# AgamChopra/TorchRegister

Measured on AMD Instinct MI355X. Metric: registration iterations/sec (3D 256^3 fp32, affine+NCC), higher is better.
Workload: dtype f32; 1 GPU; 3D 256^3 fp32 affine+NCC, 8 independent pairs per GPU (BASELINE.json configs[3] share of one GPU), ADAM on theta; pairs_per_gpu=8, pairs_total=8, loss=NCC(alpha=100), optimizer=adam, preconditioning=100 untimed iterations before the warm-up (clock settling); value_cold has none, parallelism=1 x independent shards, no collective

## Files before the change

torchregister_amd/csrc/affine.hip:

```cpp
#ifdef TRX_DEV
#include <cstdlib>
#endif
#include "trx_dev.h"

#include "trx_common.h"

namespace trx {

struct AffineGeom {
    int TX, TY, logTX, RPT, nxseg, nychunk, nblk;
};

static AffineGeom affine_geom(const trx_volumes &v, int target_blocks_total)
{
    AffineGeom g;
    int tx = 16, l = 4;
    while (tx < v.W && tx < TRX_BLOCK) { tx <<= 1; l++; }
    g.TX = tx; g.logTX = l; g.TY = TRX_BLOCK / tx;
    g.nxseg = (v.W + tx - 1) / tx;
    long rows = (long)v.D * v.H * g.nxseg * v.B;
    long rpt = rows / ((long)g.TY * target_blocks_total);
    if (rpt < 1) rpt = 1;
    if (rpt > 64) rpt = 64;
    g.RPT = (int)rpt;
    int rows_per_blk = g.TY * g.RPT;
    g.nychunk = (v.H + rows_per_blk - 1) / rows_per_blk;
    g.nblk = v.D * g.nychunk * g.nxseg;
    return g;
}

constexpr int np_full(int nd) { return 5 + 3 * nd * (nd + 1); }
constexpr int kRowsMask = 0xFFFFFF;
__host__ __device__ constexpr int rows_note(int rows, int body) { return rows > 0 ? (rows | (body << 24)) : 0; }
constexpr int kNpMse = 13;

template <int ND, int MODE>
__global__ __launch_bounds__(TRX_BLOCK) void affine_accum_kernel(trx_volumes vol, const float *__restrict__ theta,
                                                                 AffineGeom g, int channels, size_t chan_stride,
                                                                 float *__restrict__ partials)
{
    constexpr int NC = ND;
    constexpr int NQ = (MODE == 0) ? 3 : (MODE == 2 ? 1 : 0);
    constexpr int NP = (MODE == 0) ? np_full(ND) : (MODE == 1 ? 5 : ND * (ND + 1));
    const int b = blockIdx.y;
    int id = blockIdx.x;
    const int xs = id % g.nxseg; id /= g.nxseg;
    const int yc = id % g.nychunk;
    const int z = id / g.nychunk;
    const int tid = threadIdx.x;
    const int lx = tid & (g.TX - 1), ly = tid >> g.logTX;
    const int x = xs * g.TX + lx;
    const int D = vol.D, H = vol.H, W = vol.W;

    const float *__restrict__ th = theta + (size_t)b * TRX_PSTRIDE;
    const float *__restrict__ mov = vol.moving + (size_t)b * vol.moving_stride;
    const float *__restrict__ tgt = vol.target + (size_t)b * vol.target_stride;

    float A[NQ > 0 ? NQ : 1][NC], Bq[NQ > 0 ? NQ : 1][NC], m[5];
#pragma unroll
    for (int q = 0; q < (NQ > 0 ? NQ : 1); q++)
#pragma unroll
        for (int c = 0; c < NC; c++) A[q][c] = Bq[q][c] = 0.f;
#pragma unroll
    for (int i = 0; i < 5; i++) m[i] = 0.f;

    float xn = 0.f, zn = 0.f;
    if (x < W) {
        xn = base_coord(vol.xn, x, W);
        float bx, by, bz = 0.f, t_x1, t_y1, t_z1 = 0.f;
        if constexpr (ND == 3) {
            zn = base_coord(vol.zn, z, D);
            bx = fmaf(th[0], xn, fmaf(th[2], zn, th[3]));
            by = fmaf(th[4], xn, fmaf(th[6], zn, th[7]));
            bz = fmaf(th[8], xn, fmaf(th[10], zn, th[11]));
            t_x1 = th[1]; t_y1 = th[5]; t_z1 = th[9];
        } else {
            bx = fmaf(th[0], xn, th[2]);
            by = fmaf(th[3], xn, th[5]);
            t_x1 = th[1]; t_y1 = th[4];
        }
        const float fW = (float)W, fH = (float)H, fD = (float)D;
        const int y0 = yc * g.TY * g.RPT + ly;
        for (int j = 0; j < g.RPT; j++) {
            const int y = y0 + j * g.TY;
            if (y >= H) break;
            const float yn = base_coord(vol.yn, y, H);
            const float ix = unnorm<ND>(fmaf(t_x1, yn, bx), fW);
            const float iy = unnorm<ND>(fmaf(t_y1, yn, by), fH);
            const size_t vox = ((size_t)z * H + y) * W + x;
            float gq[NC];
            float w;
            if constexpr (MODE == 2) {
#pragma unroll
                for (int c = 0; c < NC; c++) gq[c] = 0.f;
                for (int ch = 0; ch < channels; ch++) {
                    const float go = tgt[ch * chan_stride + vox];
                    if constexpr (ND == 3) {
                        const float iz = unnorm<ND>(fmaf(t_z1, yn, bz), fD);
                        Samp3 s = sample3(mov + ch * chan_stride, D, H, W, ix, iy, iz);
                        gq[0] = fmaf(go, s.dx, gq[0]); gq[1] = fmaf(go, s.dy, gq[1]); gq[2] = fmaf(go, s.dz, gq[2]);
                    } else {
                        Samp2 s = sample2(mov + ch * chan_stride, H, W, ix, iy);
                        gq[0] = fmaf(go, s.dx, gq[0]); gq[1] = fmaf(go, s.dy, gq[1]);
                    }
                }
                w = 0.f;
            } else {
                if constexpr (ND == 3) {
                    const float iz = unnorm<ND>(fmaf(t_z1, yn, bz), fD);
                    Samp3 s = sample3(mov, D, H, W, ix, iy, iz);
                    w = s.v; gq[0] = s.dx; gq[1] = s.dy; gq[2] = s.dz;
                } else {
                    Samp2 s = sample2(mov, H, W, ix, iy);
                    w = s.v; gq[0] = s.dx; gq[1] = s.dy;
                }
            }
            if constexpr (MODE != 2) {
                const float yv = tgt[vox];
                m[0] += yv; m[1] += w;
                m[2] = fmaf(yv, yv, m[2]); m[3] = fmaf(w, w, m[3]); m[4] = fmaf(yv, w, m[4]);
                if constexpr (MODE == 0) {
#pragma unroll
                    for (int c = 0; c < NC; c++) {
                        const float u = yn * gq[c];
                        A[0][c] += gq[c];            Bq[0][c] += u;
                        A[1][c] = fmaf(yv, gq[c], A[1][c]); Bq[1][c] = fmaf(yv, u, Bq[1][c]);
                        A[2][c] = fmaf(w, gq[c], A[2][c]);  Bq[2][c] = fmaf(w, u, Bq[2][c]);
                    }
                }
            } else {
#pragma unroll
                for (int c = 0; c < NC; c++) { A[0][c] += gq[c]; Bq[0][c] = fmaf(yn, gq[c], Bq[0][c]); }
            }
        }
    }

    float vals[NP];
    int o = 0;
    if constexpr (MODE != 2) {
#pragma unroll
        for (int i = 0; i < 5; i++) vals[o++] = m[i];
    }
#pragma unroll
    for (int q = 0; q < NQ; q++)
#pragma unroll
        for (int c = 0; c < NC; c++) {
            vals[o++] = xn * A[q][c];
            vals[o++] = Bq[q][c];
            if constexpr (ND == 3) vals[o++] = zn * A[q][c];
            vals[o++] = A[q][c];
        }
    block_reduce_store<NP>(vals, partials + ((size_t)b * g.nblk + blockIdx.x) * NP);
}

template <int TX_, int TZ_, int THREADS_, int BW_, int BH_, int BD_, int PP_, int TY_ = 16>
struct TileCfg {
    static constexpr int TX = TX_, TY = TY_, TZ = TZ_, Threads = THREADS_;
    static constexpr int BW = BW_, BH = BH_, BD = BD_, PP = PP_;
    static constexpr int NH = Threads / (TX * TZ);
    static constexpr int Rows = TY / NH;
    static constexpr int Waves = Threads / 64;
    static constexpr int BW4 = BW / 4;
    static constexpr int PlaneSlots = BH * BW4;
    static constexpr int Pieces = (BD + PP - 1) / PP;
    static constexpr int PieceFloats = PP * BH * BW;
    static constexpr int BoxFloats = BW * BH * BD;
    static constexpr int ReduceScratch = Waves * 16 * 65 + Waves * 16;
    static constexpr int BoxAlloc = (BoxFloats > ReduceScratch) ? BoxFloats : ReduceScratch;
    static_assert(BW % 4 == 0 && PP * PlaneSlots <= Threads && (PP == 2 || PP == 4), "one DMA piece: at most one slot per thread");
};
using GeomA = TileCfg<32, 8, 512, 44, 23, TRX_GEOMA_BD, 2>;
#ifndef TRX_GEOMR_BH
#define TRX_GEOMR_BH 27
#define TRX_GEOMR_BD 26
#endif
using GeomR = TileCfg<16, 8, 512, 28, TRX_GEOMR_BH, TRX_GEOMR_BD, 2>;
using GeomD = TileCfg<32, 16, 512, 44, 23, 19, 2>;
using GeomRD = TileCfg<16, 16, 512, 28, TRX_GEOMR_BH, TRX_GEOMR_BD, 2>;

struct TileGeom {
    int ntx, nty, ntz, ntiles, blocks_per_pair, ysplit, tiles_per_seg;
};

template <class G = GeomA>
static TileGeom tile_geom(const trx_volumes &v)
{
    TileGeom t;
    t.ntx = (v.W + G::TX - 1) / G::TX; t.nty = (v.H + G::TY - 1) / G::TY; t.ntz = (v.D + G::TZ - 1) / G::TZ;
    t.ntiles = t.ntx * t.nty * t.ntz;
    const int ncol = t.ntx * t.ntz;
#ifdef TRX_DEV
    static const int target = [] { const char *e = getenv("TRX_TILE_TARGET_BLOCKS"); return e ? atoi(e) : 0; }();
#else
    constexpr int target = 0;
#endif
    const long cols = (long)v.B * ncol;
    int ys = 1;
    if (target > 0) {
        ys = (int)((target + cols - 1) / cols);
    } else if (cols * t.nty > 1024) {
        double best = 1e30;
        int last_tps = 0;
        const int cmax = cols > 512 ? (t.nty < 4 ? t.nty : 4) : t.nty;
        for (int c = 1; c <= cmax; c++) {
            const int tps = (t.nty + c - 1) / c, segs = (t.nty + tps - 1) / tps;
            if (tps == last_tps) continue;
            last_tps = tps;
            const long blocks = cols * segs, full = blocks / 512, rem = blocks % 512;
            double cost = (double)full * 1.6 * (tps + 1.5);
            if (rem > 0) cost += (rem <= 256 ? 1.0 : 1.6) * (tps + 1.5);
            if (cost < best - 1e-9) { best = cost; ys = c; }
        }
    } else if (cols <= 512) {
        ys = (int)((512 + cols - 1) / cols);
        const int cap = t.nty / 2 > 1 ? t.nty / 2 : 1;
        if (ys > cap && cols * cap >= 256) ys = cap;
    } else {
        double best = 1e30;
        for (int c = 1; c <= 4 && c <= t.nty; c++) {
            const int tps = (t.nty + c - 1) / c, segs = (t.nty + tps - 1) / tps;
            const double blocks = (double)cols * segs;
            const double rounds = (double)(((long)blocks + 511) / 512);
            const double waste = rounds * 512.0 / blocks * (1.0 + 1.5 / tps);
            if (waste < best - 1e-9) { best = waste; ys = c; }
        }
    }
    if (ys < 1) ys = 1;
    if (ys > t.nty) ys = t.nty;
    t.tiles_per_seg = (t.nty + ys - 1) / ys;
    t.ysplit = (t.nty + t.tiles_per_seg - 1) / t.tiles_per_seg;
    t.blocks_per_pair = ncol * t.ysplit;
    return t;
}

struct F1Acc {
    f2 AB[3][3], M01, M23;
    float M4;
};

template <int MODE>
__device__ __forceinline__ void f1_accumulate_pk(const Samp3 &sm, float yv, float yn, F1Acc &a)
{
    if constexpr (MODE == 2) {
        const float gq[3] = {sm.dx, sm.dy, sm.dz};
#pragma unroll
        for (int c = 0; c < 3; c++) {
            const f2 gu = {gq[c], yn * gq[c]};
            a.AB[0][c] = gu * yv + a.AB[0][c];
        }
        return;
    }
    if constexpr (MODE == 4) {
        const float d = sm.v - yv;
        a.M4 = fmaf(d, d, a.M4);
        const float gq[3] = {sm.dx, sm.dy, sm.dz};
#pragma unroll
        for (int c = 0; c < 3; c++) {
            const f2 gu = {gq[c], yn * gq[c]};
            a.AB[0][c] = gu * d + a.AB[0][c];
        }
        return;
    }
    const f2 yw = {yv, sm.v};
    a.M01 += yw;
    a.M23 = yw * yw + a.M23;
    a.M4 = fmaf(yv, sm.v, a.M4);
    if constexpr (MODE == 0) {
        const float gq[3] = {sm.dx, sm.dy, sm.dz};
#pragma unroll
        for (int c = 0; c < 3; c++) {
            const f2 gu = {gq[c], yn * gq[c]};
            a.AB[0][c] += gu;
            a.AB[1][c] = gu * yv + a.AB[1][c];
            a.AB[2][c] = gu * sm.v + a.AB[2][c];
        }
    }
}

constexpr int kTileThreads = GeomA::Threads;

__device__ __forceinline__ int trx_lane_id() { return (int)__builtin_amdgcn_mbcnt_hi(~0u, __builtin_amdgcn_mbcnt_lo(~0u, 0u)); }
__device__ __forceinline__ int trx_wave_index() { return __builtin_amdgcn_readfirstlane((int)threadIdx.x >> 6); }

template <int NV, int NW>
__device__ __forceinline__ void block_reduce_store_nw(const float (&vals)[NV], float *__restrict__ out, float *smem, int wave)
{
    constexpr int CH = 16;
    float(*red)[CH][65] = reinterpret_cast<float(*)[CH][65]>(smem);
    float(*wsum)[CH] = reinterpret_cast<float(*)[CH]>(smem + NW * CH * 65);
    const int lane = trx_lane_id(), tid = wave * 64 + lane;
#pragma unroll
    for (int c0 = 0; c0 < NV; c0 += CH) {
#pragma unroll
        for (int j = 0; j < CH; j++)
            if (c0 + j < NV) red[wave][j][lane] = vals[c0 + j];
        __syncthreads();
        if (lane < CH && c0 + lane < NV) {
            float s = 0.f;
#pragma unroll 16
            for (int i = 0; i < 64; i++) s += red[wave][lane][i];
            wsum[wave][lane] = s;
        }
        __syncthreads();
        if (tid < CH && c0 + tid < NV) {
            float s = 0.f;
#pragma unroll
            for (int w = 0; w < NW; w++) s += wsum[w][tid];
            out[c0 + tid] = s;
        }
        __syncthreads();
    }
}

__device__ __forceinline__ float uni(float v) { return __int_as_float(__builtin_amdgcn_readfirstlane(__float_as_int(v))); }
template <class T>
__device__ __forceinline__ T *uni_ptr(T *p)
{
    const unsigned long long v = (unsigned long long)p;
    const unsigned lo = __builtin_amdgcn_readfirstlane((unsigned)v), hi = __builtin_amdgcn_readfirstlane((unsigned)(v >> 32));
    return (T *)(((unsigned long long)hi << 32) | lo);
}
__device__ __forceinline__ float lane_bcast(float v, int lane) { return __int_as_float(__builtin_amdgcn_readlane(__float_as_int(v), lane)); }

#pragma clang diagnostic push
#pragma clang diagnostic ignored "-Winline-asm"
#pragma clang diagnostic ignored "-Wint-to-pointer-cast"
template <int MODE, class G, bool LTH = false>
__device__ __forceinline__ void tile_body(const trx_volumes &vol, const float *__restrict__ theta, const TileGeom &tg, int channels,
                                          float *__restrict__ partials, float *box, const int bx, const int by, const int rows_stride, const int wave_in)
{
    constexpr int kTX = G::TX, kTY = G::TY, kTZ = G::TZ, kBW = G::BW, kBH = G::BH, kBD = G::BD, kPP = G::PP;
    constexpr int kBufs = 1;
    constexpr int kNH = G::NH, kRows = G::Rows, kTileWaves = G::Waves, kBW4 = G::BW4, kPlaneSlots = G::PlaneSlots, kPieces = G::Pieces;
    constexpr int kPieceFloats = G::PieceFloats, kBoxFloats = G::BoxFloats;
    (void)kNH; (void)kBD; (void)kPlaneSlots;
    constexpr int NQ = (MODE == 0) ? 3 : ((MODE == 2 || MODE == 4) ? 1 : 0);
    constexpr int NP = (MODE == 0) ? np_full(3) : (MODE == 2 ? 12 : (MODE == 4 ? kNpMse : 5));
    constexpr bool kGrad = (MODE == 0) || (MODE == 2) || (MODE == 4);
    constexpr bool kPerChannel = (MODE == 2) || (MODE == 3);
    const int b = kPerChannel ? by / channels : by;
    const int ch = kPerChannel ? by - b * channels : 0;
    const int D = vol.D, H = vol.H, W = vol.W;
    const float *__restrict__ th = LTH ? theta : uni_ptr(theta + (size_t)b * TRX_PSTRIDE);
    const float *__restrict__ mov = uni_ptr(vol.moving + (size_t)b * vol.moving_stride + (size_t)ch * D * H * W);
    float *__restrict__ wout = uni_ptr(partials + (size_t)by * D * H * W);
    const float *__restrict__ tgt = (MODE == 3) ? wout : uni_ptr(vol.target + (size_t)b * vol.target_stride + (MODE == 2 ? (size_t)ch * D * H * W : 0));
    const float *__restrict__ xtab = uni_ptr(vol.xn), *__restrict__ ytab = uni_ptr(vol.yn), *__restrict__ ztab = uni_ptr(vol.zn);
    const int lane = trx_lane_id();
    const int wave = __builtin_amdgcn_readfirstlane(wave_in);
    const int tid = wave * 64 + lane;
    const int lx = tid & (kTX - 1), lz = (tid / kTX) & (kTZ - 1), lh = wave / (kTileWaves / kNH);
    const float fW = (float)W, fH = (float)H, fD = (float)D;
    const float hW = 0.5f * fW, hH = 0.5f * fH, hD = 0.5f * fD;
    auto thv = [&](int k) { return LTH ? uni(th[k]) : th[k]; };
    const float t00 = thv(0), t01 = thv(1), t02 = thv(2), t03 = thv(3);
    const float t10 = thv(4), t11 = thv(5), t12 = thv(6), t13 = thv(7);
    const float t20 = thv(8), t21 = thv(9), t22 = thv(10), t23 = thv(11);
    const float sx = uni(hW * t01), sy = uni(hH * (t11 - 1.0f)), sz = uni(hD * t21);

    const int ncol = tg.ntx * tg.ntz;
    const int yseg = bx / ncol, cb = bx - yseg * ncol;
    int col = cb;
    if ((ncol & 7) == 0) col = (cb & 7) * (ncol >> 3) + (cb >> 3);
    const int X0 = (col % tg.ntx) * kTX, Z0 = (col / tg.ntx) * kTZ;
    const int nx = min(kTX, W - X0), nz = min(kTZ, D - Z0);
    const bool act = (lx < nx) && (lz < nz);
    const int x = X0 + (act ? lx : 0), z = Z0 + (act ? lz : 0);
    const float xn = xtab[x], zn = ztab[z];
    const float base_x = unnorm<3>(xn, fW) + hW * fmaf(t00 - 1.0f, xn, fmaf(t02, zn, t03));
    const float base_y = hH * fmaf(t10, xn, fmaf(t12, zn, t13));
    const float base_z = unnorm<3>(zn, fD) + hD * fmaf(t20, xn, fmaf(t22 - 1.0f, zn, t23));

    float ext_lo[3], ext_hi[3];
    {
        const float ex[3] = {(float)(kTX - 1), (float)(kTY - 1), (float)(kTZ - 1)};
        const float slope[3][3] = {{t00, t01 * fW / fH, t02 * fW / fD}, {t10 * fH / fW, t11, t12 * fH / fD}, {t20 * fD / fW, t21 * fD / fH, t22}};
#pragma unroll
        for (int c = 0; c < 3; c++) {
            ext_lo[c] = ext_hi[c] = 0.f;
#pragma unroll
            for (int a = 0; a < 3; a++) {
                const float e = slope[c][a] * ex[a];
                ext_lo[c] += fminf(e, 0.f); ext_hi[c] += fmaxf(e, 0.f);
            }
            ext_lo[c] = uni(ext_lo[c]); ext_hi[c] = uni(ext_hi[c]);
        }
    }
    const float cxn = xtab[X0], czn = ztab[Z0];
    const float corner_x = uni(unnorm<3>(cxn, fW) + hW * fmaf(t00 - 1.0f, cxn, fmaf(t02, czn, t03)));
    const float corner_y = uni(hH * fmaf(t10, cxn, fmaf(t12, czn, t13)));
    const float corner_z = uni(unnorm<3>(czn, fD) + hD * fmaf(t20, cxn, fmaf(t22 - 1.0f, czn, t23)));

    auto slot_geom = [&](int ln, unsigned &rb0, int &d0) {
        const int q = wave * 64 + ln;
        const int pz = q / kPlaneSlots, r = q - pz * kPlaneSlots;
        const int dy = r / kBW4, dx4 = r - dy * kBW4;
        const bool valid = q < kPP * kPlaneSlots;
        rb0 = valid ? (unsigned)((pz * H + dy) * W + dx4 * 4) * 4u : 0u;
        d0 = valid ? ((pz << 16) | (dy << 8) | dx4) : (100 << 16);
    };
    const unsigned piece_stride = (unsigned)(kPP * H * W) * 4u;
    constexpr int kDShift = (kPP == 2) ? 17 : 18;
    auto fill_slot = [&](float *dst, int gz, int gy, int gx) {
        const bool rowin = ((unsigned)gz < (unsigned)D) && ((unsigned)gy < (unsigned)H);
        const float *row = mov + ((size_t)(rowin ? gz : 0) * H + (rowin ? gy : 0)) * W;
        float4 v;
        v.x = (rowin && (unsigned)(gx + 0) < (unsigned)W) ? row[gx + 0] : 0.f;
        v.y = (rowin && (unsigned)(gx + 1) < (unsigned)W) ? row[gx + 1] : 0.f;
        v.z = (rowin && (unsigned)(gx + 2) < (unsigned)W) ? row[gx + 2] : 0.f;
        v.w = (rowin && (unsigned)(gx + 3) < (unsigned)W) ? row[gx + 3] : 0.f;
        *reinterpret_cast<float4 *>(dst) = v;
    };
    static_assert(kPP == 2 || kPP == 4, "piece planes");

    F1Acc acc;
#pragma unroll
    for (int q = 0; q < 3; q++)
#pragma unroll
        for (int c = 0; c < 3; c++) acc.AB[q][c] = (f2)(0.f);
    acc.M01 = acc.M23 = (f2)(0.f);
    acc.M4 = 0.f;
    const int j0 = lh * kRows;
    const int toff = (z * H + j0) * W + x;

    const int ty_begin = yseg * tg.tiles_per_seg, ty_end = min((yseg + 1) * tg.tiles_per_seg, tg.nty);
    int g_ox = 0, g_oy = 0, g_oz = 0, g_pk = 0;
    auto lane_geometry = [&](int ty_first) {
        const int ty = min(ty_first + lane, tg.nty - 1);
        const float yn0 = ytab[ty * kTY], yid0 = unnorm<3>(yn0, fH);
        const float cx = fmaf(sx, yn0, corner_x), cy = yid0 + fmaf(sy, yn0, corner_y), cz = fmaf(sz, yn0, corner_z);
        const float slack = 0.05f;
        bool fits = (fabsf(cx) < 1.0e6f) && (fabsf(cy) < 1.0e6f) && (fabsf(cz) < 1.0e6f);
        int ox = 0, oy = 0, oz = 0, ex4 = 0, ey = 0, ez = 0;
        bool interior = false;
        if (fits) {
            const int lx0 = (int)floorf(cx + ext_lo[0] - slack), hx1 = (int)floorf(cx + ext_hi[0] + slack) + 1;
            oy = (int)floorf(cy + ext_lo[1] - slack); const int hy1 = (int)floorf(cy + ext_hi[1] + slack) + 1;
            oz = (int)floorf(cz + ext_lo[2] - slack); const int hz1 = (int)floorf(cz + ext_hi[2] + slack) + 1;
            ox = lx0 & ~3;
            ex4 = ((hx1 - ox) >> 2) + 1; ey = hy1 - oy + 1; ez = hz1 - oz + 1;
            fits = (ex4 <= kBW4) && (ey <= kBH) && (ez <= kBD);
            interior = (ox >= 0) && (oy >= 0) && (oz >= 0) && (ox + kBW <= W) && (oy + kBH <= H) && (oz + kBD <= D);
        }
        g_ox = ox; g_oy = oy; g_oz = oz;
        g_pk = fits ? ((ex4 - 1) | ((ey - 1) << 8) | ((ez - 1) << 16) | (1 << 24) | ((interior ? 1 : 0) << 25)) : 0;
    };
    int ty = ty_begin;
    {
        const unsigned toffb = (unsigned)toff * 4u;
        const unsigned lane7b = (unsigned)(lane & (kRows - 1)) * 4u;
        float sxv, syv, szv;
        asm("v_mov_b32 %0, %1" : "=v"(sxv) : "s"(sx));
        asm("v_mov_b32 %0, %1" : "=v"(syv) : "s"(sy));
        asm("v_mov_b32 %0, %1" : "=v"(szv) : "s"(sz));
        int ys_s, zs_s;
        asm("s_mov_b32 %0, %1" : "=s"(ys_s) : "i"(kBW * 4));
        asm("s_mov_b32 %0, %1" : "=s"(zs_s) : "i"(kBW * kBH * 4));
        const unsigned box_lds = (unsigned)(uintptr_t)box;
        unsigned rb0;
        {
            int d0;
            slot_geom(lane, rb0, d0);
        }
        constexpr bool kZMask = kPieces > 8;
        static_assert(!kZMask || (kPP == 2 && kBD <= 32), "plane-bit masks: pieces of two planes");
        constexpr int kNM = kZMask ? 1 : kPieces;
        unsigned long long m_ld[kNM];
#pragma unroll
        for (int k = 0; k < kNM; k++) m_ld[k] = 0;
        unsigned long long m_a0 = 0, m_a1 = 0;
        unsigned m_zb = 0;
        unsigned m_oob = 0;
        unsigned m_part = 0;
        int lim_blk;
        {
            const float slack2 = 0.1f;
            const int ex4m = (((int)floorf(ext_hi[0] - ext_lo[0] + slack2) + 5) >> 2) + 1;
            const int eym = (int)floorf(ext_hi[1] - ext_lo[1] + slack2) + 3, ezm = (int)floorf(ext_hi[2] - ext_lo[2] + slack2) + 3;
            lim_blk = __builtin_amdgcn_readfirstlane(((min(ezm, kBD) - 1) << 16) | ((min(eym, kBH) - 1) << 8) | (min(ex4m, kBW4) - 1));
        }
        int m_lim = -1, m_lo = -1, m_hi = -1, m_px = -2;
        TRX_TM_INIT();
        typedef const __attribute__((address_space(3))) f2u *lds_f2;
        while (ty < ty_end) {
          lane_geometry(ty);
          const int chunk = min(64, ty_end - ty);
          const bool xpart = ((W & 3) != 0) && (g_ox + 4 * ((lim_blk & 0xff) + 1) > W - (W & 3)) &&
                             (g_oy + ((lim_blk >> 8) & 0xff) >= H - 1) && (g_oz + (lim_blk >> 16) >= D - 1);
          const bool ok = (lane < chunk) && ((g_pk >> 24) & 1) && ((ty + lane + 1) * kTY <= H) && !xpart;
          const unsigned long long bad = ~__builtin_amdgcn_ballot_w64(ok);
          const int nf = bad ? __builtin_ctzll(bad) : 64;
          const char *dma_base = nullptr;
          unsigned dma_lds = 0;
          auto issue_box = [&](int g, int buf, bool spread) {
              const int ox = __builtin_amdgcn_readlane(g_ox, g), oy = __builtin_amdgcn_readlane(g_oy, g), oz = __builtin_amdgcn_readlane(g_oz, g);
              const int lim = lim_blk;
              const int loz = max(0, -oz), loy = max(0, -oy), lox = max(0, -(ox >> 2));
              const int hiz = min(lim >> 16, D - 1 - oz), hiy = min((lim >> 8) & 0xff, H - 1 - oy), hix = min(lim & 0xff, ((W - ox + 3) >> 2) - 1);
              const bool none = (hiz < loz) || (hiy < loy) || (hix < lox);
              const int lo = none ? 0x7f7f7f : ((loz << 16) | (loy << 8) | lox);
              const int hi = none ? 0 : ((hiz << 16) | (hiy << 8) | hix);
              const int part_x = ((W & 3) && !none && ((W - ox) >> 2) <= hix) ? ((W - ox) >> 2) : -1;
              if (lim != m_lim || lo != m_lo || hi != m_hi || part_x != m_px) {
                  m_lim = lim; m_lo = lo; m_hi = hi; m_px = part_x;
                  m_oob = 0;
                  m_part = 0;
                  int ln = lane;
                  asm volatile("" : "+v"(ln));
                  unsigned rbx;
                  int d0;
                  slot_geom(ln, rbx, d0);
#pragma unroll
                  for (int k = 0; k < kPieces; k++) {
                      const int d = d0 + (k << kDShift);
                      const bool need = (((lim - d) & 0x80808080) == 0);
                      const bool ld = need && (((hi - d) & 0x80808080) == 0) && (((d - lo) & 0x80808080) == 0);
                      if constexpr (!kZMask) m_ld[k] = __builtin_amdgcn_ballot_w64(ld);
                      if (need && !ld) m_oob |= 1u << k;
                      if (ld && (d & 0xff) == part_x) m_part |= 1u << k;
                  }
                  if constexpr (kZMask) {
                      const int dyx = d0 & 0xffff;
                      const bool xy = (((((lim & 0xffff) - dyx) | ((hi & 0xffff) - dyx) | (dyx - (lo & 0xffff))) & 0x8080) == 0);
                      m_a0 = __builtin_amdgcn_ballot_w64(xy && (d0 >> 16) == 0);
                      m_a1 = __builtin_amdgcn_ballot_w64(xy && (d0 >> 16) == 1);
                      m_zb = (unsigned)__builtin_amdgcn_readfirstlane((int)(none ? 0u : (((2u << hiz) - 1u) & ~((1u << loz) - 1u))));
                  }
              }
              dma_base = reinterpret_cast<const char *>(mov + (ptrdiff_t)((oz * H + oy) * W + ox));
              dma_lds = box_lds + (unsigned)buf * (kBoxFloats * 4u) + (unsigned)wave * 1024u;
              if (TRX_DBG_SKIP != 2 && !spread) {
                  const float *mbase = reinterpret_cast<const float *>(dma_base);
                  const unsigned lds0 = dma_lds;
                  unsigned long long sv;
                  unsigned m0s;
                  static_assert((kPieces >= 6 && kPieces <= 8) || (kPieces >= 9 && kPieces <= 13), "the DMA block below is written for 6, 7, 8 or 9..13 pieces");
#define TRX_DMA_SKIP "s_cbranch_execz 1f\n\t"
#define TRX_DMA_NEXT(K)                                  \
    "s_add_u32 s100, s100, %[vstr]\n\t"                  \
    "s_addc_u32 s101, s101, 0\n\t"                       \
    "s_add_u32 m0, m0, %[pstr]\n\t"                      \
    "s_mov_b64 exec, %[k" #K "]\n\t"                     \
    TRX_DMA_SKIP                                         \
    "global_load_lds_dwordx4 %[off], s[100:101]" TRX_BOX_POLICY "\n\t" \
    "1:\n\t"
#define TRX_DMA_HEAD                                     \
    "s_mov_b64 %[sv], exec\n\t"                          \
    "s_mov_b32 %[m0s], m0\n\t"                           \
    "s_mov_b64 s[100:101], %[base]\n\t"                  \
    "s_mov_b32 m0, %[lds]\n\t"                           \
    "s_mov_b64 exec, %[k0]\n\t"                          \
    TRX_DMA_SKIP                                         \
    "global_load_lds_dwordx4 %[off], s[100:101]" TRX_BOX_POLICY "\n\t"     \
    "1:\n\t"                                             \
    TRX_DMA_NEXT(1) TRX_DMA_NEXT(2) TRX_DMA_NEXT(3) TRX_DMA_NEXT(4) TRX_DMA_NEXT(5)
#define TRX_DMA_TAIL "s_mov_b64 exec, %[sv]\n\t" "s_mov_b32 m0, %[m0s]"
                  if constexpr (kZMask) {
                      static_assert(kPieces <= 13, "plane-bit DMA block: up to 13 pieces (the plane bits of pieces a shallower box lacks are never set)");
                      unsigned long long t0, t1;
#define TRX_DMA_ZSEL(B0, B1)                             \
    "s_bitcmp1_b32 %[zb], " #B0 "\n\t"                   \
    "s_cselect_b64 %[t0], %[a0], 0\n\t"                 \
    "s_bitcmp1_b32 %[zb], " #B1 "\n\t"                   \
    "s_cselect_b64 %[t1], %[a1], 0\n\t"                 \
    "s_or_b64 exec, %[t0], %[t1]\n\t"                   \
    "s_cbranch_execz 1f\n\t"                            \
    "global_load_lds_dwordx4 %[off], s[100:101]" TRX_BOX_POLICY "\n\t" \
    "1:\n\t"
#define TRX_DMA_ZNEXT(B0, B1)                            \
    "s_add_u32 s100, s100, %[vstr]\n\t"                 \
    "s_addc_u32 s101, s101, 0\n\t"                      \
    "s_add_u32 m0, m0, %[pstr]\n\t" TRX_DMA_ZSEL(B0, B1)
                      asm volatile("s_mov_b64 %[sv], exec\n\t"
                                   "s_mov_b32 %[m0s], m0\n\t"
                                   "s_mov_b64 s[100:101], %[base]\n\t"
                                   "s_mov_b32 m0, %[lds]\n\t" TRX_DMA_ZSEL(0, 1)
                                   TRX_DMA_ZNEXT(2, 3) TRX_DMA_ZNEXT(4, 5) TRX_DMA_ZNEXT(6, 7) TRX_DMA_ZNEXT(8, 9) TRX_DMA_ZNEXT(10, 11)
                                   TRX_DMA_ZNEXT(12, 13) TRX_DMA_ZNEXT(14, 15) TRX_DMA_ZNEXT(16, 17) TRX_DMA_ZNEXT(18, 19)
                                   TRX_DMA_ZNEXT(20, 21) TRX_DMA_ZNEXT(22, 23) TRX_DMA_ZNEXT(24, 25) TRX_DMA_TAIL
                                   : [sv] "=&s"(sv), [m0s] "=&s"(m0s), [t0] "=&s"(t0), [t1] "=&s"(t1)
                                   : [lds] "s"(lds0), [base] "s"(mbase), [pstr] "i"(kPieceFloats * 4), [vstr] "s"(piece_stride), [off] "v"(rb0),
                                     [a0] "s"(m_a0), [a1] "s"(m_a1), [zb] "s"(__builtin_amdgcn_readfirstlane((int)m_zb))
                                   : "memory", "scc", "s100", "s101");
#undef TRX_DMA_ZSEL
#undef TRX_DMA_ZNEXT
                  } else if constexpr (kPieces == 8) {
                      asm volatile(TRX_DMA_HEAD TRX_DMA_NEXT(6) TRX_DMA_NEXT(7) TRX_DMA_TAIL
                                   : [sv] "=&s"(sv), [m0s] "=&s"(m0s)
                                   : [lds] "s"(lds0), [base] "s"(mbase), [pstr] "i"(kPieceFloats * 4), [vstr] "s"(piece_stride), [off] "v"(rb0),
                                     [k0] "s"(m_ld[0]), [k1] "s"(m_ld[1]), [k2] "s"(m_ld[2]), [k3] "s"(m_ld[3]), [k4] "s"(m_ld[4]),
                                     [k5] "s"(m_ld[5]), [k6] "s"(m_ld[kPieces > 6 ? 6 : 0]), [k7] "s"(m_ld[kPieces - 1])
                                   : "memory", "scc", "s100", "s101");
                  } else if constexpr (kPieces == 7) {
                      asm volatile(TRX_DMA_HEAD TRX_DMA_NEXT(6) TRX_DMA_TAIL
                                   : [sv] "=&s"(sv), [m0s] "=&s"(m0s)
                                   : [lds] "s"(lds0), [base] "s"(mbase), [pstr] "i"(kPieceFloats * 4), [vstr] "s"(piece_stride), [off] "v"(rb0),
                                     [k0] "s"(m_ld[0]), [k1] "s"(m_ld[1]), [k2] "s"(m_ld[2]), [k3] "s"(m_ld[3]), [k4] "s"(m_ld[4]),
                                     [k5] "s"(m_ld[5]), [k6] "s"(m_ld[kPieces - 1])
                                   : "memory", "scc", "s100", "s101");
                  } else {
                      asm volatile(TRX_DMA_HEAD TRX_DMA_TAIL
                                   : [sv] "=&s"(sv), [m0s] "=&s"(m0s)
                                   : [lds] "s"(lds0), [base] "s"(mbase), [pstr] "i"(kPieceFloats * 4), [vstr] "s"(piece_stride), [off] "v"(rb0),
                                     [k0] "s"(m_ld[0]), [k1] "s"(m_ld[1]), [k2] "s"(m_ld[2]), [k3] "s"(m_ld[3]), [k4] "s"(m_ld[4]),
                                     [k5] "s"(m_ld[5])
                                   : "memory", "scc", "s100", "s101");
                  }
#undef TRX_DMA_NEXT
#undef TRX_DMA_SKIP
#undef TRX_DMA_HEAD
#undef TRX_DMA_TAIL
              }
              if (m_oob) {
                  float zero;
                  asm volatile("v_mov_b32 %0, 0" : "=v"(zero));
#pragma unroll
                  for (int k = 0; k < kPieces; k++)
                      if (m_oob & (1u << k))
                          *reinterpret_cast<float4 *>(box + buf * kBoxFloats + k * kPieceFloats + (wave * 64 + lane) * 4) = make_float4(zero, zero, zero, zero);
              }
          };
          auto zero_tails = [&](int buf) {
#pragma unroll
              for (int k = 0; k < kPieces; k++)
                  if (m_part & (1u << k)) {
                      float *sl = box + buf * kBoxFloats + k * kPieceFloats + (wave * 64 + lane) * 4;
                      for (int e = W & 3; e < 4; e++) sl[e] = 0.f;
                  }
          };
          auto issue_piece = [&](int k) {
              if (TRX_DBG_SKIP == 2) return;
              unsigned long long sv;
              unsigned m0s;
              asm volatile("s_mov_b64 %[sv], exec\n\t"
                           "s_mov_b32 %[m0s], m0\n\t"
                           "s_mov_b32 m0, %[lds]\n\t"
                           "s_mov_b64 exec, %[mk]\n\t"
                           "global_load_lds_dwordx4 %[off], %[base]\n\t"
                           "s_mov_b64 exec, %[sv]\n\t"
                           "s_mov_b32 m0, %[m0s]"
                           : [sv] "=&s"(sv), [m0s] "=&s"(m0s)
                           : [lds] "s"(dma_lds + (unsigned)k * (kPieceFloats * 4u)), [base] "s"(dma_base + (size_t)k * piece_stride), [off] "v"(rb0),
                             [mk] "s"(kZMask ? ((((m_zb >> (2 * k)) & 1u) ? m_a0 : 0ull) | (((m_zb >> (2 * k + 1)) & 1u) ? m_a1 : 0ull)) : m_ld[kZMask ? 0 : k])
                           : "memory");
          };
          auto gather_tile = [&](int g, int buf, float yn_l, float yid_l, float (&tv)[kRows], const float *tnext, bool dma_next) {
              const int Y0 = (ty + g) * kTY;
              const int ox = __builtin_amdgcn_readlane(g_ox, g), oy = __builtin_amdgcn_readlane(g_oy, g), oz = __builtin_amdgcn_readlane(g_oz, g);
              float yn_r[kRows], yid_r[kRows];
#pragma unroll
              for (int j = 0; j < kRows; j++) { yn_r[j] = lane_bcast(yn_l, j); yid_r[j] = lane_bcast(yid_l, j); }
              if (TRX_DBG_SKIP == 1) return;
              const int bpb = (int)box_lds + buf * (kBoxFloats * 4) - ((oz * kBH + oy) * kBW + ox) * 4;
              struct Fetch { f2 r00, r01, r10, r11; float fx, fy, fz; };
              auto fetch = [&](int j) -> Fetch {
                  const float yn = yn_r[j];
                  const float ix = fmaf(sxv, yn, base_x);
                  const float iy = yid_r[j] + fmaf(syv, yn, base_y);
                  const float iz = fmaf(szv, yn, base_z);
                  int a0, a1, a2, a3;
                  asm("v_lshl_add_u32 %0, %1, 2, %2" : "=v"(a0) : "v"(floor_to_int(ix)), "s"(bpb));
                  asm("v_mad_i32_i24 %0, %1, %2, %3" : "=v"(a1) : "v"(floor_to_int(iy)), "s"(ys_s), "v"(a0));
                  asm("v_mad_i32_i24 %0, %1, %2, %3" : "=v"(a2) : "v"(floor_to_int(iz)), "s"(zs_s), "v"(a1));
                  asm("v_add_u32 %0, %1, %2" : "=v"(a3) : "s"(zs_s), "v"(a2));
                  Fetch f;
                  f.r00 = *(lds_f2)(unsigned)a2; f.r01 = *(lds_f2)(unsigned)(a2 + kBW * 4);
                  f.r10 = *(lds_f2)(unsigned)a3; f.r11 = *(lds_f2)(unsigned)(a3 + kBW * 4);
                  f.fx = __builtin_amdgcn_fractf(ix); f.fy = __builtin_amdgcn_fractf(iy); f.fz = __builtin_amdgcn_fractf(iz);
                  return f;
              };
              Fetch cur = fetch(0);
#pragma unroll
              for (int j = 0; j < kRows; j++) {
                  Fetch nxt;
                  if (j + 1 < kRows) nxt = fetch(j + 1);
                  if (kBufs == 2 && j < kPieces && dma_next) issue_piece(j);
                  const Samp3 sm = lerp3_pairs<kGrad>(cur.r00, cur.r01, cur.r10, cur.r11, cur.fx, cur.fy, cur.fz);
                  if constexpr (MODE == 3) { if (act) wout[(size_t)Y0 * W + (unsigned)(toff + j * W)] = sm.v; }
                  else f1_accumulate_pk<MODE>(sm, tv[j], yn_r[j], acc);
                  if (kBufs == 2 && TRX_DBG_SKIP != 3 && MODE != 3)
                      asm volatile("global_load_dword %0, %1, %2" : "=v"(tv[j]) : "v"(toffb), "s"(tnext + (size_t)j * W));
                  if (j + 1 < kRows) cur = nxt;
              }
          };
          auto load_targets = [&](int g, float (&tv)[kRows]) {
              const float *trow = tgt + (size_t)(ty + g) * kTY * W;
#pragma unroll
              for (int j = 0; j < kRows; j++) {
                  if (TRX_DBG_SKIP == 3 || MODE == 3) tv[j] = 1.f;
                  else asm volatile("global_load_dword %0, %1, %2" TRX_TGT_POLICY : "=v"(tv[j]) : "v"(toffb), "s"(trow + (size_t)j * W) : "memory");
              }
          };
          float tv[kRows];
          if constexpr (kBufs == 1) {
            for (int gl = 0; gl < nf; gl++) {
              TRX_TM_STAMP(tm0);
              float yn_l;
              asm volatile("global_load_dword %0, %1, %2" : "=v"(yn_l) : "v"(lane7b), "s"(ytab + (ty + gl) * kTY + j0) : "memory");
              __builtin_amdgcn_s_setprio(TRX_STAGE_PRIO);
              load_targets(gl, tv);
              issue_box(gl, 0, false);
              __builtin_amdgcn_s_setprio(0);
              asm volatile("s_waitcnt vmcnt(0)" ::: "memory");
              if (m_part) zero_tails(0);
              {
#pragma unroll
                  for (int j = 0; j < kRows; j++) asm volatile("" : "+v"(tv[j]));
                  asm volatile("" : "+v"(yn_l));
              }
              const float yid_l = unnorm<3>(yn_l, fH);
              TRX_TM_STAMP(tm1);
              __syncthreads();
              TRX_TM_STAMP(tm2);
              gather_tile(gl, 0, yn_l, yid_l, tv, nullptr, false);
              TRX_TM_STAMP(tm3);
              __syncthreads();
              TRX_TM_TILE_DONE();
            }
          } else {
            if (nf > 0) {
                load_targets(0, tv);
                issue_box(0, 0, false);
            }
            for (int gl = 0; gl < nf; gl++) {
              TRX_TM_STAMP(tm0);
              float yn_l;
              asm volatile("global_load_dword %0, %1, %2" : "=v"(yn_l) : "v"(lane7b), "s"(ytab + (ty + gl) * kTY + j0) : "memory");
              asm volatile("s_waitcnt vmcnt(0)" ::: "memory");
              if (m_part) zero_tails(gl & 1);
              {
#pragma unroll
                  for (int j = 0; j < kRows; j++) asm volatile("" : "+v"(tv[j]));
                  asm volatile("" : "+v"(yn_l));
              }
              const float yid_l = unnorm<3>(yn_l, fH);
              TRX_TM_STAMP(tm1);
              __syncthreads();
              TRX_TM_STAMP(tm2);
              const int gn = (gl + 1 < nf) ? gl + 1 : gl;
              if (gl + 1 < nf) issue_box(gl + 1, (gl + 1) & 1, true);
              TRX_TM_STAMP(tm3);
              gather_tile(gl, gl & 1, yn_l, yid_l, tv, tgt + (size_t)(ty + gn) * kTY * W, gl + 1 < nf);
              TRX_TM_TILE_DONE();
            }
            asm volatile("s_waitcnt vmcnt(0)" ::: "memory");
#pragma unroll
            for (int j = 0; j < kRows; j++) asm volatile("" : "+v"(tv[j]));
            __syncthreads();
          }
          ty += nf;
          if (nf < chunk) break;
        }
        TRX_TM_STORE();
        if (!act) {
#pragma unroll
            for (int q = 0; q < 3; q++)
#pragma unroll
                for (int c = 0; c < 3; c++) acc.AB[q][c] = (f2)(0.f);
            acc.M01 = acc.M23 = (f2)(0.f);
            acc.M4 = 0.f;
        }
    }

    unsigned rb0;
    int d0;
    {
        int ln = lane;
        asm volatile("" : "+v"(ln));
        slot_geom(ln, rb0, d0);
    }
    int prev_lim = -1;
    unsigned needmask = 0;

    auto stage_box = [&](int pk, int ox, int oy, int oz) {
        const bool interior = (pk >> 25) & 1;
        const int lim = pk & 0xffffff;
        if (lim != prev_lim) {
            prev_lim = lim;
            needmask = 0;
#pragma unroll
            for (int k = 0; k < kPieces; k++)
                if (((lim - (d0 + (k << kDShift))) & 0x80808080) == 0) needmask |= 1u << k;
        }
        const int obase = (oz * H + oy) * W + ox;
        unsigned oob = 0;
        if (interior) {
            const char *__restrict__ mbase = reinterpret_cast<const char *>(mov + obase);
#pragma unroll
            for (int k = 0; k < kPieces; k++)
                if ((needmask & (1u << k)) && TRX_DBG_SKIP != 2)
                    __builtin_amdgcn_global_load_lds(reinterpret_cast<const float *>(mbase + (size_t)k * piece_stride + rb0),
                                                     box + k * kPieceFloats + wave * 256, 16, 0, 0);
        } else {
#pragma unroll
            for (int k = 0; k < kPieces; k++)
                if ((needmask & (1u << k)) && TRX_DBG_SKIP != 2) {
                    const int d = d0 + (k << kDShift);
                    const int gz = oz + (d >> 16), gy = oy + ((d >> 8) & 0xff), gx = ox + (d & 0xff) * 4;
                    const bool inb = ((unsigned)gz < (unsigned)D) && ((unsigned)gy < (unsigned)H) && (gx >= 0) && (gx + 4 <= W);
                    const unsigned idx = inb ? (unsigned)(obase + (int)((rb0 + k * piece_stride) >> 2)) : 0u;
                    if (!inb) oob |= 1u << k;
                    __builtin_amdgcn_global_load_lds(mov + idx, box + k * kPieceFloats + wave * 256, 16, 0, 0);
                }
        }
        __builtin_amdgcn_s_setprio(0);
        asm volatile("s_waitcnt vmcnt(0)" ::: "memory");
        if (oob) {
#pragma unroll
            for (int k = 0; k < kPieces; k++)
                if (oob & (1u << k)) {
                    const int d = d0 + (k << kDShift);
                    fill_slot(box + k * kPieceFloats + (wave * 64 + lane) * 4, oz + (d >> 16), oy + ((d >> 8) & 0xff), ox + (d & 0xff) * 4);
                }
        }
    };
    auto gather = [&](const float *bp, float yn, float yid) -> Samp3 {
        const float ix = fmaf(sx, yn, base_x);
        const float iy = yid + fmaf(sy, yn, base_y);
        const float iz = fmaf(sz, yn, base_z);
        const int a = __mul24(floor_to_int(iz), kBH * kBW) + __mul24(floor_to_int(iy), kBW) + floor_to_int(ix);
        const float *p = bp + a;
        const f2 r00 = *reinterpret_cast<const f2u *>(p), r01 = *reinterpret_cast<const f2u *>(p + kBW);
        const f2 r10 = *reinterpret_cast<const f2u *>(p + kBW * kBH), r11 = *reinterpret_cast<const f2u *>(p + kBW * kBH + kBW);
        return lerp3_pairs<kGrad>(r00, r01, r10, r11, __builtin_amdgcn_fractf(ix), __builtin_amdgcn_fractf(iy), __builtin_amdgcn_fractf(iz));
    };

    for (; ty < ty_end; ty++) {
        const int gl = (ty - ty_begin) & 63;
        if (gl == 0) lane_geometry(ty);
        const int Y0 = ty * kTY;
        const int ny = min(kTY, H - Y0);
        const float yn_l = ytab[Y0 + min(lane & (kTY - 1), ny - 1)];
        const float yid_l = unnorm<3>(yn_l, fH);
        const int pk = __builtin_amdgcn_readlane(g_pk, gl);
        const int ox = __builtin_amdgcn_readlane(g_ox, gl), oy = __builtin_amdgcn_readlane(g_oy, gl), oz = __builtin_amdgcn_readlane(g_oz, gl);
        const bool fits = (pk >> 24) & 1;
        const float *__restrict__ trow = tgt + (size_t)Y0 * W;

        if (fits) {
            __builtin_amdgcn_s_setprio(TRX_STAGE_PRIO);
            float tv[kRows];
#pragma unroll
            for (int j = 0; j < kRows; j++)
                tv[j] = (TRX_DBG_SKIP == 3 || MODE == 3) ? 1.f : trow[(unsigned)(toff + (min(j0 + j, ny - 1) - j0) * W)];
            stage_box(pk, ox, oy, oz);
            __syncthreads();
            float yn_r[kRows], yid_r[kRows];
#pragma unroll
            for (int j = 0; j < kRows; j++) { yn_r[j] = lane_bcast(yn_l, j0 + j); yid_r[j] = lane_bcast(yid_l, j0 + j); }
            if (act && TRX_DBG_SKIP != 1) {
                const float *bp = box - ((oz * kBH + oy) * kBW + ox);
#pragma unroll
                for (int j = 0; j < kRows; j++)
                    if (j0 + j < ny) {
                        const Samp3 sm = gather(bp, yn_r[j], yid_r[j]);
                        if constexpr (MODE == 3) wout[(size_t)Y0 * W + (unsigned)(toff + j * W)] = sm.v;
                        else f1_accumulate_pk<MODE>(sm, tv[j], yn_r[j], acc);
                    }
            }
            __syncthreads();
        } else if (act) {
            struct GFetch { f2 r00, r01, r10, r11; float fx, fy, fz, yn, yv; };
            auto gfetch = [&](int j) -> GFetch {
                GFetch g;
                g.yn = ytab[Y0 + j];
                const float ix = fmaf(sx, g.yn, base_x);
                const float iy = unnorm<3>(g.yn, fH) + fmaf(sy, g.yn, base_y);
                const float iz = fmaf(sz, g.yn, base_z);
                const float flx = floorf(ix), fly = floorf(iy), flz = floorf(iz);
                g.fx = ix - flx; g.fy = iy - fly; g.fz = iz - flz;
                const int x0 = (int)flx, y0 = (int)fly, z0 = (int)flz;
                const bool interior = ((unsigned)x0 < (unsigned)(W - 1)) & ((unsigned)y0 < (unsigned)(H - 1)) & ((unsigned)z0 < (unsigned)(D - 1));
                if (__all(interior)) {
                    const float *p = mov + ((size_t)z0 * H + y0) * W + x0, *q = p + (size_t)H * W;
                    g.r00 = *reinterpret_cast<const f2u *>(p); g.r01 = *reinterpret_cast<const f2u *>(p + W);
                    g.r10 = *reinterpret_cast<const f2u *>(q); g.r11 = *reinterpret_cast<const f2u *>(q + W);
                } else {
                    const int x1 = x0 + 1, y1 = y0 + 1, z1 = z0 + 1;
                    const bool bx0 = (unsigned)x0 < (unsigned)W, bx1 = (unsigned)x1 < (unsigned)W;
                    const bool by0 = (unsigned)y0 < (unsigned)H, by1 = (unsigned)y1 < (unsigned)H;
                    const bool bz0 = (unsigned)z0 < (unsigned)D, bz1 = (unsigned)z1 < (unsigned)D;
                    const int cx0 = min(max(x0, 0), W - 1), cx1 = min(max(x1, 0), W - 1);
                    const int cy0 = min(max(y0, 0), H - 1), cy1 = min(max(y1, 0), H - 1);
                    const int cz0 = min(max(z0, 0), D - 1), cz1 = min(max(z1, 0), D - 1);
                    const float *a00 = mov + ((size_t)cz0 * H + cy0) * W, *a01 = mov + ((size_t)cz0 * H + cy1) * W;
                    const float *a10 = mov + ((size_t)cz1 * H + cy0) * W, *a11 = mov + ((size_t)cz1 * H + cy1) * W;
                    g.r00 = f2{(bz0 & by0 & bx0) ? a00[cx0] : 0.f, (bz0 & by0 & bx1) ? a00[cx1] : 0.f};
                    g.r01 = f2{(bz0 & by1 & bx0) ? a01[cx0] : 0.f, (bz0 & by1 & bx1) ? a01[cx1] : 0.f};
                    g.r10 = f2{(bz1 & by0 & bx0) ? a10[cx0] : 0.f, (bz1 & by0 & bx1) ? a10[cx1] : 0.f};
                    g.r11 = f2{(bz1 & by1 & bx0) ? a11[cx0] : 0.f, (bz1 & by1 & bx1) ? a11[cx1] : 0.f};
                }
                g.yv = (MODE == 3) ? 0.f : trow[(unsigned)(toff + (j - j0) * W)];
                return g;
            };
            const int jend = min(j0 + kRows, ny);
            if (j0 < jend) {
                GFetch cur = gfetch(j0);
#pragma unroll 1
                for (int j = j0; j < jend; j++) {
                    GFetch nxt = cur;
                    if (j + 1 < jend) nxt = gfetch(j + 1);
                    const Samp3 sm = lerp3_pairs<kGrad>(cur.r00, cur.r01, cur.r10, cur.r11, cur.fx, cur.fy, cur.fz);
                    if constexpr (MODE == 3) wout[(size_t)Y0 * W + (unsigned)(toff + (j - j0) * W)] = sm.v;
                    else f1_accumulate_pk<MODE>(sm, cur.yv, cur.yn, acc);
                    cur = nxt;
                }
            }
        }
    }

    if constexpr (MODE == 3) return;
    float vals[NP];
    int o = 0;
    if constexpr (MODE == 4) {
        vals[0] = acc.M4;
        o = 1;
    } else if constexpr (MODE != 2) {
        vals[0] = acc.M01.x; vals[1] = acc.M01.y; vals[2] = acc.M23.x; vals[3] = acc.M23.y; vals[4] = acc.M4;
        o = 5;
    }
#pragma unroll
    for (int q = 0; q < NQ; q++)
#pragma unroll
        for (int c = 0; c < 3; c++) {
            const float a = acc.AB[q][c].x;
            vals[o++] = xn * a; vals[o++] = acc.AB[q][c].y; vals[o++] = zn * a; vals[o++] = a;
        }
    block_reduce_store_nw<NP, kTileWaves>(vals, partials + ((size_t)by * rows_stride + bx) * NP, box, wave);
}

template <int MODE>
__global__ __launch_bounds__(GeomA::Threads, TRX_TILE_MIN_WAVES) void affine_tile_kernel(trx_volumes vol, const float *__restrict__ theta,
                                                                                          TileGeom tg, int channels, float *__restrict__ partials)
{
    __shared__ __attribute__((aligned(16))) float box[GeomA::BoxAlloc + TRX_DEV_LDS_PAD];
    tile_body<MODE, GeomA>(vol, theta, tg, channels, partials, box, blockIdx.x, blockIdx.y, gridDim.x, trx_wave_index());
}

#pragma clang diagnostic pop
#include "affine_zstream.h"
#include "affine_eft.h"
#pragma clang diagnostic push
#pragma clang diagnostic ignored "-Winline-asm"
#pragma clang diagnostic ignored "-Wint-to-pointer-cast"

template <class G>
__device__ __forceinline__ bool dual_fits(const float *__restrict__ th, float fD, float fH, float fW)
{
    const float slope[3][3] = {{th[0], th[1] * fW / fH, th[2] * fW / fD}, {th[4] * fH / fW, th[5], th[6] * fH / fD}, {th[8] * fD / fW, th[9] * fD / fH, th[10]}};
    const float ex[3] = {(float)(G::TX - 1), (float)(G::TY - 1), (float)(G::TZ - 1)};
    float span[3];
#pragma unroll
    for (int c = 0; c < 3; c++) span[c] = fabsf(slope[c][0]) * ex[0] + fabsf(slope[c][1]) * ex[1] + fabsf(slope[c][2]) * ex[2];
    return (span[0] < 1.0e6f) && (span[1] < 1.0e6f) && (span[2] < 1.0e6f) &&
           ((((int)floorf(span[0] + 0.1f) + 5) >> 2) + 1 <= G::BW4) && ((int)floorf(span[1] + 0.1f) + 3 <= G::BH) &&
           ((int)floorf(span[2] + 0.1f) + 3 <= G::BD);
}
__device__ __forceinline__ int dual_choice(const float *__restrict__ th, float fD, float fH, float fW, bool with_deep, bool with_rd = false, int zs_planes = 0)
{
    if (zs_planes > 0 && zs_nsub<ZS64>(th, fD, fH, fW, zs_planes) > 0) return 4;
    if (with_deep && dual_fits<GeomD>(th, fD, fH, fW)) return 0;
    if (dual_fits<GeomA>(th, fD, fH, fW)) return 1;
    return (with_rd && dual_fits<GeomRD>(th, fD, fH, fW)) ? 3 : 2;
}

__device__ __forceinline__ bool eft_wants(int choice, const float *__restrict__ th, float fD, float fH, float fW)
{
    if (choice == 2) return true;
    if (choice != 3) return false;
    const float tilt = fabsf(th[8] * fD / fW) + fabsf(th[9] * fD / fH);
    const float zspan = (tilt + fabsf(th[10])) * (float)(ECfg::TZ - 1);
    if (zspan > 17.0f || tilt > 0.07f) return true;
    const float s = fmaxf(fabsf(th[1] * fW / fH), fabsf(th[4] * fH / fW));
    return s > 0.15f && s < 0.37f;
}

struct CarryKArgs {
    const float *prev_partials;
    const int *prev_rows_used;
    int prev_nblk;
    int mse_rows;
    const float *state_prev;
    float *state_next;
    double nvox;
    trx_loss_cfg lc;
    trx_opt_cfg oc;
    trx_affine_state st;
};
typedef const __attribute__((address_space(4))) CarryKArgs *CarryKPtr;
template <int MODE>
__device__ __forceinline__ void carry_prologue(CarryKPtr c, int b, bool designated, int D, int H, int W, float *scratch, float *s_th, int wave, int lane);

struct DualKArgs {
    trx_volumes vol;
    const float *theta;
    TileGeom tgA, tgR;
    int channels;
    float *partials;
    int zero_surplus;
    TileGeom tgD, tgRD;
    ZGeom zg;
    int *rows_used;
    int rows_stride;
    int eft;
    CarryKArgs carry;
};

template <int MODE, int WHICH = 0>
__global__ __launch_bounds__(512, TRX_DUAL_MIN_WAVES) void affine_tile_dual_kernel(trx_volumes vol_, const float *__restrict__ theta_, TileGeom tgA_,
                                                                                   TileGeom tgR_, int channels_, float *__restrict__ partials_,
                                                                                   int zero_surplus_ = 1, TileGeom tgD_ = TileGeom{}, TileGeom tgRD_ = TileGeom{},
                                                                                   ZGeom zg_ = ZGeom{}, int *__restrict__ rows_used_ = nullptr, int rows_stride_ = 0,
                                                                                   int eft_ = 0, CarryKArgs carry_ = CarryKArgs{})
{
    static_assert(GeomA::Threads == 512 && GeomR::Threads == 512 && GeomD::Threads == 512 && GeomRD::Threads == 512, "every geometry runs 512-thread blocks");
    static_assert(GeomRD::BoxAlloc <= GeomR::BoxAlloc, "GeomRD lives in GeomR's box");
    constexpr bool kCarry = WHICH == 6;
    static_assert(!kCarry || MODE == 0 || MODE == 4, "the carry form exists for the step kernels");
    constexpr bool kDeep = (WHICH == 0 || WHICH == 4) && (MODE == 0 || MODE == 4);
    constexpr bool kZs = kDeep && WHICH == 0;
    constexpr int kAllocAR = GeomA::BoxAlloc > GeomR::BoxAlloc ? GeomA::BoxAlloc : GeomR::BoxAlloc;
    constexpr int kAllocD = (kDeep && GeomD::BoxAlloc > kAllocAR) ? GeomD::BoxAlloc : kAllocAR;
    constexpr int kAlloc = (kZs && ZS64::Alloc > kAllocD) ? ZS64::Alloc : kAllocD;
    __shared__ __attribute__((aligned(16))) float box[kAlloc];
    constexpr bool kPerChannel = (MODE == 2) || (MODE == 3);
    constexpr int NP = (MODE == 0) ? np_full(3) : (MODE == 2 ? 12 : (MODE == 4 ? kNpMse : 5));
    typedef const __attribute__((address_space(4))) DualKArgs *KArgs;
    auto args = [&]() {
        KArgs p = (KArgs)__builtin_amdgcn_kernarg_segment_ptr();
        asm volatile("" : "+s"(p));
        return p;
    };
    typedef const __attribute__((address_space(4))) TileGeom *KTile;
    auto tile_of = [](KTile t) { return TileGeom{t->ntx, t->nty, t->ntz, t->ntiles, t->blocks_per_pair, t->ysplit, t->tiles_per_seg}; };
    float fD, fH, fW;
    bool with_d, with_rd;
    int zs_planes, rows_stride, nA, nR, nD, nRD, nZ;
    bool with_ef;
    const float *theta;
    {
        KArgs a = args();
        fD = (float)a->vol.D; fH = (float)a->vol.H; fW = (float)a->vol.W;
        nA = a->tgA.blocks_per_pair; nR = a->tgR.blocks_per_pair; nD = a->tgD.blocks_per_pair; nRD = a->tgRD.blocks_per_pair; nZ = a->zg.blocks_per_pair;
        with_d = kDeep && nD > 0; with_rd = kDeep && nRD > 0;
        zs_planes = kZs && nZ > 0 ? a->zg.planes_per_seg : 0;
        rows_stride = a->rows_stride;
        theta = a->theta;
        with_ef = kDeep && a->rows_used != nullptr && (a->eft != 0 || WHICH == 4);
        if constexpr (WHICH == 4) {
            const int *plan = a->rows_used + a->vol.B;
            if (__builtin_amdgcn_readfirstlane(*plan) == 0) return;
        }
    }
    auto blocks_of = [&](int choice) { return choice == 6 ? 0 : (choice == 7 ? nRD : (choice == 4 ? nZ : (choice == 0 ? nD : (choice == 3 ? nRD : (choice == 1 ? nA : nR))))); };
    const bool flat = kDeep && rows_stride > 0;
    const int wave_idx = trx_wave_index();
    const int lane = trx_lane_id();
    const int tid_ = wave_idx * 64 + lane;
    __shared__ int s_choice[64], s_pre[64];
    __shared__ float s_th[16];
    if constexpr (kCarry) {
        carry_prologue<MODE>(&args()->carry, (int)blockIdx.y, blockIdx.x == 0, args()->vol.D, args()->vol.H, args()->vol.W, box, s_th, wave_idx, lane);
        theta = s_th - (size_t)blockIdx.y * TRX_PSTRIDE;
    }
    int my_choice = 2, total = 1;
    if (flat) {
        KArgs a = args();
        const int B = a->vol.B;
        int *rows_used = a->rows_used;
        int cnt = 0, ch = 2;
        if (lane < B) ch = dual_choice(theta + (size_t)lane * TRX_PSTRIDE, fD, fH, fW, with_d, with_rd, zs_planes);
        if (with_ef && lane < B && rows_used[lane] < 0) ch = 6;
        if (lane < B) {
            cnt = blocks_of(ch);
            if (rows_used && blockIdx.x == 0 && wave_idx == 0 && ch != 6) rows_used[lane] = ch == 7 ? -rows_note(cnt, 7) : rows_note(cnt, 1 + ch);
        }
        int pre = cnt;
#pragma unroll
        for (int d = 1; d < 64; d <<= 1) {
            const int t = __shfl_up(pre, d, 64);
            if (lane >= d) pre += t;
        }
        total = __builtin_amdgcn_readlane(pre, 63);
        if (wave_idx == 0) { s_choice[lane] = ch; s_pre[lane] = pre; }
        __syncthreads();
    } else {
        KArgs a = args();
        const int channels = a->channels;
        const int b = kPerChannel ? blockIdx.y / channels : blockIdx.y;
        my_choice = __builtin_amdgcn_readfirstlane(dual_choice(theta + (size_t)b * TRX_PSTRIDE, fD, fH, fW, with_d, with_rd, zs_planes));
        if (with_ef && a->rows_used[b] < 0) my_choice = 6;
        const int mine = blocks_of(my_choice);
        int *rows_used = a->rows_used;
        if (rows_used && blockIdx.x == 0 && tid_ == 0 && my_choice != 6) rows_used[blockIdx.y] = rows_note(mine, 1 + my_choice);
        if ((int)blockIdx.x >= mine) {
            if (MODE != 3 && a->zero_surplus && tid_ < NP) a->partials[((size_t)blockIdx.y * gridDim.x + blockIdx.x) * NP + tid_] = 0.f;
            return;
        }
    }
    total = __builtin_amdgcn_readfirstlane(total);
    const int it0 = flat ? (int)blockIdx.x : 0, it_step = flat ? (int)gridDim.x : 1;
    for (int item = __builtin_amdgcn_readfirstlane(it0); item < total; item += it_step) {
        int choice, v, by, stride;
        if (flat) {
            const int pre = *(volatile int *)&s_pre[lane];
            const int it = (WHICH == 4 && (args()->vol.flags & TRX_FLAG_WALK_DOWN) && (total & 7) == 0) ? total - 8 - (item & ~7) + (item & 7) : item;
            const int pair = __builtin_amdgcn_readfirstlane(__builtin_popcountll(__builtin_amdgcn_ballot_w64(pre <= it)));
            const int off = pair > 0 ? __builtin_amdgcn_readlane(pre, pair - 1) : 0;
            choice = *(volatile int *)&s_choice[pair];
            v = __builtin_amdgcn_readfirstlane(it - off); by = pair; stride = rows_stride;
            if (item != it0) __syncthreads();
        } else {
            choice = __builtin_amdgcn_readfirstlane(my_choice); v = blockIdx.x; by = blockIdx.y; stride = gridDim.x;
        }
        choice = __builtin_amdgcn_readfirstlane(choice); v = __builtin_amdgcn_readfirstlane(v);
        by = __builtin_amdgcn_readfirstlane(by); stride = __builtin_amdgcn_readfirstlane(stride);
        KArgs a = args();
        const trx_volumes vol = {a->vol.moving, a->vol.target, a->vol.moving_stride, a->vol.target_stride, a->vol.ndim, a->vol.B, a->vol.D, a->vol.H, a->vol.W,
                                 a->vol.xn, a->vol.yn, a->vol.zn, a->vol.flags};
        float *partials = a->partials;
        const int channels = a->channels;
        if constexpr (kZs) {
            if (choice == 4) {
                const ZGeom zg = {a->zg.ntx, a->zg.nty, a->zg.nzseg, a->zg.planes_per_seg, a->zg.blocks_per_pair};
                zstream_body<MODE, ZS64>(vol, theta, zg, partials, box, v, by, stride, wave_idx,
                                         (int)((blockIdx.y * gridDim.x + blockIdx.x) * 2 >= gridDim.x * gridDim.y));
                continue;
            }
        }
        if constexpr (kDeep) {
            if (choice == 0) {
                const TileGeom t = tile_of(&a->tgD);
                tile_body<MODE, GeomD>(vol, theta, t, channels, partials, box, v, by, stride, wave_idx);
                continue;
            }
            if (choice == 3) {
                const TileGeom t = tile_of(&a->tgRD);
                tile_body<MODE, GeomRD>(vol, theta, t, channels, partials, box, v, by, stride, wave_idx);
                continue;
            }
        }
        if (choice != 1) {
            const TileGeom t = tile_of(&a->tgR);
            if constexpr (kCarry) tile_body<MODE, GeomR, true>(vol, s_th, t, channels, partials, box, v, by, stride, wave_idx);
            else tile_body<MODE, GeomR>(vol, theta, t, channels, partials, box, v, by, stride, wave_idx);
            continue;
        }
        const TileGeom t = tile_of(&a->tgA);
        if constexpr (kCarry) tile_body<MODE, GeomA, true>(vol, s_th, t, channels, partials, box, v, by, stride, wave_idx);
        else tile_body<MODE, GeomA>(vol, theta, t, channels, partials, box, v, by, stride, wave_idx);
    }
}

struct ZsOneKArgs {
    trx_volumes vol;
    const float *theta;
    ZGeom zg, zgf;
    float *partials;
    int *rows_used;
    int stride;
    TileGeom tgR;
};
template <int MODE, int FB>
__device__ __forceinline__ void zs_step_main(const trx_volumes &vol, const float *__restrict__ theta, const ZGeom &zg, const ZGeom &zgf, float *__restrict__ partials,
                                             int *__restrict__ rows_used, int stride, const int fb_blocks, float *ring)
{
    const int wave = trx_wave_index(), lane = trx_lane_id();
    const float fD = (float)vol.D, fH = (float)vol.H, fW = (float)vol.W;
    int which = 0;
    if (lane < vol.B) {
        if (zs_nsub<ZS64>(theta + (size_t)lane * TRX_PSTRIDE, fD, fH, fW, zg.planes_per_seg) > 0) which = 1;
        else if (zgf.blocks_per_pair > 0 && zs_nsub<ZSF>(theta + (size_t)lane * TRX_PSTRIDE, fD, fH, fW, zgf.planes_per_seg) > 0) which = 2;
        else if (FB) which = 3;
    }
    const unsigned long long take = __builtin_amdgcn_ballot_w64(which != 0), take1 = __builtin_amdgcn_ballot_w64(which == 1);
    const int mine = which == 1 ? zg.blocks_per_pair : (which == 2 ? zgf.blocks_per_pair : ((FB && which == 3) ? fb_blocks : 0));
    if (blockIdx.x == 0 && wave == 0) {
        if (lane < vol.B) rows_used[lane] = -rows_note(mine, which == 3 ? 3 : (which == 2 ? 8 : 6));
        if (lane == 0) {
            rows_used[vol.B] = vol.B - __builtin_popcountll(take);
            rows_used[vol.B + 1] = (int)(unsigned)take; rows_used[vol.B + 2] = (int)(unsigned)(take >> 32);
        }
        if (lane < 8) rows_used[vol.B + 3 + lane] = 0;
    }
    if (take == 0) return;
    int pre = mine;
#pragma unroll
    for (int d = 1; d < 64; d <<= 1) {
        const int t = __shfl_up(pre, d, 64);
        if (lane >= d) pre += t;
    }
    const int total = __builtin_amdgcn_readlane(pre, 63);
    const int second = (int)(blockIdx.x * 2 >= gridDim.x);
    if constexpr (FB != 0) {
        const int prew = (pre << 2) | which;
        for (int item = blockIdx.x; item < total; item += gridDim.x) {
            const int pair = __builtin_amdgcn_readfirstlane(__builtin_popcountll(__builtin_amdgcn_ballot_w64((prew >> 2) <= item)));
            const int off = pair > 0 ? (__builtin_amdgcn_readlane(prew, pair - 1) >> 2) : 0;
            const int w = __builtin_amdgcn_readlane(prew, pair) & 3;
            const int v = __builtin_amdgcn_readfirstlane(item - off);
            if (item != (int)blockIdx.x) __syncthreads();
            if (__builtin_expect(w == 3, 0)) {
                typedef const __attribute__((address_space(4))) ZsOneKArgs *KArgs;
                KArgs a = (KArgs)__builtin_amdgcn_kernarg_segment_ptr();
                asm volatile("" : "+s"(a));
                const TileGeom t = {a->tgR.ntx, a->tgR.nty, a->tgR.ntz, a->tgR.ntiles, a->tgR.blocks_per_pair, a->tgR.ysplit, a->tgR.tiles_per_seg};
                tile_body<MODE, GeomR>(vol, theta, t, 1, partials, ring, v, pair, stride, wave);
            } else if (w == 1) zstream_body<MODE, ZS64>(vol, theta, zg, partials, ring, v, pair, stride, wave, second);
            else zstream_body<MODE, ZSF>(vol, theta, zgf, partials, ring, v, pair, stride, wave, second);
        }
        return;
    }
    for (int item = blockIdx.x; item < total; item += gridDim.x) {
        const int pair = __builtin_amdgcn_readfirstlane(__builtin_popcountll(__builtin_amdgcn_ballot_w64(pre <= item)));
        const int off = pair > 0 ? __builtin_amdgcn_readlane(pre, pair - 1) : 0;
        const int v = __builtin_amdgcn_readfirstlane(item - off);
        if (item != (int)blockIdx.x) __syncthreads();
        if ((take1 >> pair) & 1ull) zstream_body<MODE, ZS64>(vol, theta, zg, partials, ring, v, pair, stride, wave, second);
        else zstream_body<MODE, ZSF>(vol, theta, zgf, partials, ring, v, pair, stride, wave, second);
    }
}

template <int MODE>
__global__ __launch_bounds__(ZS64::Threads, TRX_ZS_MIN_WAVES) void affine_zs_step_kernel(trx_volumes vol, const float *__restrict__ theta, ZGeom zg, ZGeom zgf, float *__restrict__ partials,
                                                                                         int *__restrict__ rows_used, int stride)
{
    constexpr int kAlloc = ZSF::Alloc > ZS64::Alloc ? ZSF::Alloc : ZS64::Alloc;
    __shared__ __attribute__((aligned(16))) float ring[kAlloc];
    zs_step_main<MODE, 0>(vol, theta, zg, zgf, partials, rows_used, stride, 0, ring);
}

template <int MODE>
__global__ __launch_bounds__(ZS64::Threads, TRX_ZS_MIN_WAVES) void affine_zs_one_kernel(trx_volumes vol, const float *__restrict__ theta, ZGeom zg, ZGeom zgf, float *__restrict__ partials,
                                                                                        int *__restrict__ rows_used, int stride, TileGeom tgR)
{
    constexpr int kAllocZ = ZSF::Alloc > ZS64::Alloc ? ZSF::Alloc : ZS64::Alloc;
    constexpr int kAlloc = GeomR::BoxAlloc > kAllocZ ? GeomR::BoxAlloc : kAllocZ;
    __shared__ __attribute__((aligned(16))) float ring[kAlloc];
    zs_step_main<MODE, 1>(vol, theta, zg, zgf, partials, rows_used, stride, tgR.blocks_per_pair, ring);
}

template <int MODE>
__global__ __launch_bounds__(ECfg::Threads, 4) void affine_eft_step_kernel(trx_volumes vol, const float *__restrict__ theta, TileGeom tg, float *__restrict__ partials,
                                                                           int *__restrict__ rows_used, int stride, int with_d, int with_rd, int zs_planes_)
{
    const bool zs_first = zs_planes_ < 0;
    const int zs_planes = zs_first ? 0 : zs_planes_;
    __shared__ __attribute__((aligned(16))) float lds[ECfg::Alloc];
    __shared__ int s_ef[64];
    const int wave = trx_wave_index(), lane = trx_lane_id();
    const float fD = (float)vol.D, fH = (float)vol.H, fW = (float)vol.W;
    if (stride < 0) {
        if ((int)blockIdx.x >= tg.blocks_per_pair) return;
        const int b = blockIdx.y;
        const float *th = theta + (size_t)b * TRX_PSTRIDE;
        bool take = __builtin_amdgcn_readfirstlane((int)eft_wants(dual_choice(th, fD, fH, fW, with_d != 0, with_rd != 0, zs_planes), th, fD, fH, fW)) &&
                    __builtin_amdgcn_readfirstlane((int)ef_candidate(th, fD, fH, fW));
        if (take) {
            const EfMap m = ef_map(th, fD, fH, fW);
            const EfDims d = ef_dims(m);
            int cnt = 0;
#pragma unroll
            for (int h = 0; h < (ECfg::NY * ECfg::NZ) / ECfg::Threads; h++) {
                const int r = wave * 64 + lane + h * ECfg::Threads, iy = r & (ECfg::NY - 1), iz = r >> 5;
                int wlo;
                if (iy < d.ny && iz < d.nz) cnt += ef_row_window(m, d.dy0 + iy, d.dz0 + iz, wlo);
            }
#pragma unroll
            for (int o = 32; o > 0; o >>= 1) cnt += __shfl_xor(cnt, o, 64);
            if (lane == 0) s_ef[wave] = cnt;
            __syncthreads();
            int g = 0;
#pragma unroll
            for (int w = 0; w < ECfg::Waves; w++) g += s_ef[w];
            g = __builtin_amdgcn_readfirstlane(g);
            take = d.ok && g > 0 && g <= ECfg::GCap;
            __syncthreads();
        }
        if (blockIdx.x == 0 && wave == 0 && lane == 0) rows_used[b] = take ? -rows_note(tg.blocks_per_pair, 7) : 0;
        if (!take) return;
    }
    const bool flat = stride >= 0;
#if TRX_EF_STAMP
    if (flat && wave == 0 && lane == 0) { for (int k = 1; k < 8; k++) trx_ef_blocks[blockIdx.x * 8 + k] = 0; trx_ef_blocks[blockIdx.x * 8] = __builtin_amdgcn_s_memrealtime(); }
#endif
    int pre = 0, total = 1;
    if (flat) {
    if (zs_first && __builtin_amdgcn_readfirstlane(rows_used[vol.B]) == 0) return;
    unsigned long long zs_mask = 0;
    if (zs_first) zs_mask = (unsigned long long)(unsigned)__builtin_amdgcn_readfirstlane(rows_used[vol.B + 1]) | ((unsigned long long)(unsigned)__builtin_amdgcn_readfirstlane(rows_used[vol.B + 2]) << 32);
    const bool free_l = lane < vol.B && !((zs_mask >> lane) & 1ull);
    const bool cand_l = free_l && eft_wants(dual_choice(theta + (size_t)lane * TRX_PSTRIDE, fD, fH, fW, with_d != 0, with_rd != 0, zs_planes),
                                                  theta + (size_t)lane * TRX_PSTRIDE, fD, fH, fW) &&
                        ef_candidate(theta + (size_t)lane * TRX_PSTRIDE, fD, fH, fW);
    const unsigned long long cand = __builtin_amdgcn_ballot_w64(cand_l);
    unsigned long long fit = 0;
    if (cand) {
        if (wave == 0) s_ef[lane] = 0;
        __syncthreads();
        unsigned long long rest = cand;
        for (int k = 0; rest; k++) {
            const int pb = __builtin_ctzll(rest);
            rest &= rest - 1;
            if ((k & (ECfg::Waves - 1)) != wave) continue;
            const EfMap m = ef_map(theta + (size_t)pb * TRX_PSTRIDE, fD, fH, fW);
            const EfDims d = ef_dims(m);
            const int g = ef_plan_granules_wave(m, d, lane);
            if (lane == 0) s_ef[pb] = (d.ok && g > 0 && g <= ECfg::GCap) ? 1 : 0;
        }
        __syncthreads();
        fit = __builtin_amdgcn_ballot_w64(s_ef[lane] != 0) & cand;
    }
    const int mine = ((fit >> lane) & 1ull) ? tg.blocks_per_pair : 0;
    if (blockIdx.x == 0 && wave == 0 && free_l) rows_used[lane] = -rows_note(mine, 7);
    if (fit == 0) return;
    pre = mine;
#pragma unroll
    for (int d = 1; d < 64; d <<= 1) {
        const int t = __shfl_up(pre, d, 64);
        if (lane >= d) pre += t;
    }
    total = __builtin_amdgcn_readlane(pre, 63);
    }
    total = __builtin_amdgcn_readfirstlane(total);
    const int rows_stride = __builtin_amdgcn_readfirstlane(flat ? stride : -stride);
    const bool tickets = flat && zs_first && (tg.blocks_per_pair & 7) == 0 && (gridDim.x & 7) == 0 && (total % tg.blocks_per_pair) == 0;
    const int it0 = flat ? (int)blockIdx.x : 0, it_step = flat ? (int)gridDim.x : 1;
    const int it_end = flat ? total : 1;
    EfPlanRegs pr;
    int planned = -1;
    int q = blockIdx.x & 7;
    const int qlen = total >> 3, per_pair_q = tg.blocks_per_pair >> 3;
    int qk = (int)blockIdx.x >> 3;
    for (int item = __builtin_amdgcn_readfirstlane(it0); tickets ? (qk < qlen) : (item < it_end); item += it_step) {
        int v = blockIdx.x, pair = blockIdx.y;
        if (flat) {
            if (tickets) {
                int ord = qk / per_pair_q;
                const int j = qk - ord * per_pair_q;
                if (vol.flags & TRX_FLAG_WALK_DOWN) ord = total / tg.blocks_per_pair - 1 - ord;
                pair = __builtin_popcountll(__builtin_amdgcn_ballot_w64(pre <= ord * tg.blocks_per_pair));
                v = q + 8 * j;
            } else {
                pair = __builtin_popcountll(__builtin_amdgcn_ballot_w64(pre <= item));
                const int off = pair > 0 ? __builtin_amdgcn_readlane(pre, pair - 1) : 0;
                v = (item - off + 104 * pair) % tg.blocks_per_pair;
            }
        }
        v = __builtin_amdgcn_readfirstlane(v); pair = __builtin_amdgcn_readfirstlane(pair);
        if (item != it0) __syncthreads();
        eft_body<MODE>(vol, theta, tg, partials, lds, v, pair, rows_stride, wave, pr, pair != planned);
        planned = pair;
#if TRX_EF_STAMP
        if (flat && wave == 0 && lane == 0) { trx_ef_blocks[blockIdx.x * 8 + 1 + min((item - it0) / it_step, 5)] = __builtin_amdgcn_s_memrealtime(); }
#endif
        if (tickets) {
            if (wave == 0 && lane == 0) {
                const int first = (int)gridDim.x >> 3;
                int nq = blockIdx.x & 7, k = qlen;
                for (int t = 0; t < 8 && k >= qlen; t++) {
                    nq = ((int)blockIdx.x + t) & 7;
                    k = __hip_atomic_fetch_add(rows_used + vol.B + 3 + nq, 1, __ATOMIC_RELAXED, __HIP_MEMORY_SCOPE_AGENT) + first;
                }
                s_ef[63] = k < qlen ? ((nq << 24) | k) : -1;
            }
            __syncthreads();
            const int nx = __builtin_amdgcn_readfirstlane(s_ef[63]);
            if (nx < 0) break;
            q = nx >> 24; qk = nx & 0xffffff;
        }
    }
}

template <int MODE>
static void launch_dual(dim3 grid, hipStream_t s, const trx_volumes &v, const float *theta, const TileGeom &ta, const TileGeom &tr, int channels, float *out,
                        int zero_surplus = 1, TileGeom td = TileGeom{}, TileGeom trd = TileGeom{}, ZGeom zg = ZGeom{}, int *rows_used = nullptr, int rows_stride = 0,
                        int eft = 0, const CarryKArgs *carry = nullptr, bool *carry_used = nullptr)
{
    if (td.blocks_per_pair == 0 && trd.blocks_per_pair == 0 && zg.blocks_per_pair == 0 && rows_stride == 0 && eft == 0) {
        if constexpr (MODE == 0 || MODE == 4) {
            if (carry != nullptr && rows_used != nullptr && zero_surplus == 0) {
                hipLaunchKernelGGL((affine_tile_dual_kernel<MODE, 6>), grid, dim3(512), 0, s, v, theta, ta, tr, channels, out, zero_surplus, td, trd, zg, rows_used, rows_stride, 0, *carry);
                *carry_used = true;
                return;
            }
        }
        hipLaunchKernelGGL((affine_tile_dual_kernel<MODE, 3>), grid, dim3(512), 0, s, v, theta, ta, tr, channels, out, zero_surplus, td, trd, zg, rows_used, rows_stride);
    }
    else
        hipLaunchKernelGGL((affine_tile_dual_kernel<MODE, 0>), grid, dim3(512), 0, s, v, theta, ta, tr, channels, out, zero_surplus, td, trd, zg, rows_used, rows_stride, eft);
}

#pragma clang diagnostic pop


__global__ void fill_tables_kernel(float *__restrict__ tab, int W, int H, int D)
{
    const int i = blockIdx.x * blockDim.x + threadIdx.x;
    if (i < W) tab[i] = (float)(2 * i + 1) / (float)W - 1.0f;
    if (i < H) tab[W + i] = (float)(2 * i + 1) / (float)H - 1.0f;
    if (i < D) tab[W + H + i] = (float)(2 * i + 1) / (float)D - 1.0f;
}

struct LossCoef {
    double total, mse, ncc, ssd, cy, cw, c0;
};

__device__ __forceinline__ LossCoef loss_from_moments(const double *S, double n, const trx_loss_cfg &lc)
{
    const double Sy = S[0], Sw = S[1], Syy = S[2], Sww = S[3], Syw = S[4];
    const double my = Sy / n, mw = Sw / n;
    const double Saa = Syy - Sy * my, Sbb = Sww - Sw * mw, Sab = Syw - Sy * mw;
    const double s = sqrt(Saa * Sbb + 1e-10);
    const double alpha = lc.ncc_alpha;
    const double sq = Syy - 2.0 * Syw + Sww;
    LossCoef r;
    r.mse = sq / n;
    r.ncc = alpha * (1.0 - Sab / s);
    r.ssd = (double)lc.ssd_alpha * sq;
    r.total = (double)lc.w_mse * r.mse + (double)lc.w_ncc * r.ncc + (double)lc.w_ssd * r.ssd;
    const double k1 = -alpha / s, k2 = alpha * Sab * Saa / (s * s * s);
    const double q = (double)lc.w_mse * 2.0 / n + (double)lc.w_ssd * (double)lc.ssd_alpha * 2.0;
    r.cy = (double)lc.w_ncc * k1 - q;
    r.cw = (double)lc.w_ncc * k2 + q;
    r.c0 = (double)lc.w_ncc * (-k1 * my - k2 * mw);
    return r;
}

template <int ND>
__device__ void theta_from_pose(const float *p, double *th)
{
    if constexpr (ND == 3) {
        double cps, sps;
        sincos((double)p[0], &sps, &cps);
        double cth, sth;
        sincos((double)p[1], &sth, &cth);
        double cph, sph;
        sincos((double)p[2], &sph, &cph);
        th[0] = cps * cth; th[1] = sph * sps * cth - cph * sth; th[2] = cph * sps * cth + sph * sth; th[3] = 0.25 * tanh((double)p[3]);
        th[4] = cps * sth; th[5] = sph * sps * sth + cph * cth; th[6] = cph * sps * sth - sph * cth; th[7] = 0.25 * tanh((double)p[4]);
        th[8] = -sps;      th[9] = sph * cps;                   th[10] = cph * cps;                  th[11] = 0.25 * tanh((double)p[5]);
    } else {
        double c, s;
        sincos((double)p[0], &s, &c);
        th[0] = c; th[1] = -s; th[2] = p[1];
        th[3] = s; th[4] = c;  th[5] = p[2];
    }
}

template <int ND>
__device__ void pose_vjp(const float *p, const double *g, double *dx)
{
    if constexpr (ND == 3) {
        double cps, sps;
        sincos((double)p[0], &sps, &cps);
        double cth, sth;
        sincos((double)p[1], &sth, &cth);
        double cph, sph;
        sincos((double)p[2], &sph, &cph);
        dx[0] = g[0] * (-sps * cth) + g[1] * (sph * cps * cth) + g[2] * (cph * cps * cth) + g[4] * (-sps * sth) +
                g[5] * (sph * cps * sth) + g[6] * (cph * cps * sth) + g[8] * (-cps) + g[9] * (-sph * sps) + g[10] * (-cph * sps);
        dx[1] = g[0] * (-cps * sth) + g[1] * (-sph * sps * sth - cph * cth) + g[2] * (-cph * sps * sth + sph * cth) +
                g[4] * (cps * cth) + g[5] * (sph * sps * cth - cph * sth) + g[6] * (cph * sps * cth + sph * sth);
        dx[2] = g[1] * (cph * sps * cth + sph * sth) + g[2] * (-sph * sps * cth + cph * sth) +
                g[5] * (cph * sps * sth - sph * cth) + g[6] * (-sph * sps * sth - cph * cth) + g[9] * (cph * cps) + g[10] * (-sph * cps);
        for (int i = 0; i < 3; i++) {
            const double t = tanh((double)p[3 + i]);
            dx[3 + i] = g[3 + 4 * i] * 0.25 * (1.0 - t * t);
        }
    } else {
        double c, s;
        sincos((double)p[0], &s, &c);
        dx[0] = g[0] * (-s) + g[1] * (-c) + g[3] * c + g[4] * (-s);
        dx[1] = g[2];
        dx[2] = g[5];
    }
}

#define TRX_FIN_THREADS 1024

template <int NP>
__device__ __forceinline__ void reduce_partials(const float *__restrict__ part, int nblk, double *S )
{
    __shared__ double acc[TRX_FIN_THREADS / 64][64];
    const int tid = threadIdx.x, k = tid & 63, grp = tid >> 6;
    constexpr int NG = TRX_FIN_THREADS / 64;
    double s = 0.0;
    if (k < NP) {
        for (int blk0 = grp; blk0 < nblk; blk0 += 16 * NG) {
            float a[16];
#pragma unroll
            for (int i = 0; i < 16; i++) {
                const int blk = blk0 + i * NG;
                const float v = part[(size_t)min(blk, nblk - 1) * NP + k];
                a[i] = (blk < nblk) ? v : 0.f;
            }
            s += ((((double)a[0] + (double)a[1]) + ((double)a[2] + (double)a[3])) + (((double)a[4] + (double)a[5]) + ((double)a[6] + (double)a[7]))) +
                 ((((double)a[8] + (double)a[9]) + ((double)a[10] + (double)a[11])) + (((double)a[12] + (double)a[13]) + ((double)a[14] + (double)a[15])));
        }
    }
    acc[grp][k] = s;
    __syncthreads();
    if (tid < 64) {
        double t = 0.0;
#pragma unroll
        for (int i = 0; i < NG; i++) t += acc[i][tid];
        S[tid] = t;
    }
    __syncthreads();
}

template <int ND>
struct FinRegs {
    int t;
    float best_prev, theta_old, p_old, m_old, v_old;
    float pose_old[(ND == 3) ? 6 : 3];
};
template <int ND>
__device__ __forceinline__ FinRegs<ND> fin_load(const float *param, const float *theta, const float *am, const float *av, const int *step, const float *best_loss,
                                                bool adam, bool rigid, int i)
{
    constexpr int NT = ND * (ND + 1), NPOSE = (ND == 3) ? 6 : 3;
    FinRegs<ND> r;
    const int ic = min(i, NT - 1);
    r.t = *step;
    r.best_prev = best_loss ? *best_loss : 0.f;
    r.theta_old = theta[ic]; r.p_old = param[ic];
    r.m_old = r.v_old = 0.f;
    if (adam) { r.m_old = am[ic]; r.v_old = av[ic]; }
#pragma unroll
    for (int k = 0; k < NPOSE; k++) r.pose_old[k] = rigid ? param[k] : 0.f;
    return r;
}
template <int ND>
__device__ __forceinline__ void fin_apply(const double *S, const FinRegs<ND> &r, int b, int i, double nvox, int D, int H, int W, const trx_loss_cfg &lc, const trx_opt_cfg &oc,
                                          const trx_affine_state &st, int mse_rows, float *param_out, float *theta_out, float *m_out, float *v_out, int *step_out, bool user,
                                          float *theta_lds, double *sh_dth, float *sh_pose)
{
    constexpr int NT = ND * (ND + 1);
    constexpr int NPOSE = (ND == 3) ? 6 : 3;
    const bool rigid = st.mode == TRX_PARAM_RIGID;
    const int np = rigid ? NPOSE : NT;
    const int ic = min(i, NT - 1);
    const int t = r.t;
    double bc1 = 1.0, rsbc2 = 1.0;
    if (oc.kind == TRX_OPT_ADAM) {
        bc1 = 1.0 - ipow((double)oc.beta1, t + 1);
        rsbc2 = 1.0 / sqrt(1.0 - ipow((double)oc.beta2, t + 1));
    }
    const double scale[3] = {0.5 * W, 0.5 * H, 0.5 * D};
    double dth_i, total;
    if (ND == 3 && mse_rows) {
        const double q = (double)lc.w_mse * 2.0 / nvox + (double)lc.w_ssd * (double)lc.ssd_alpha * 2.0;
        total = 0.5 * q * S[0];
        dth_i = scale[ic / (ND + 1)] * q * S[1 + ic];
    } else {
        const LossCoef L = loss_from_moments(S, nvox, lc);
        total = L.total;
        dth_i = scale[ic / (ND + 1)] * (L.c0 * S[5 + ic] + L.cy * S[5 + NT + ic] + L.cw * S[5 + 2 * NT + ic]);
    }
    const float lossf = (float)total;
    const bool is_best = (t == 0) || (lossf < r.best_prev);
    if (user) {
        if (is_best && i < NT) st.best_theta[(size_t)b * TRX_PSTRIDE + i] = r.theta_old;
        if (i == 0) {
            if (st.losses && t < st.losses_capacity) st.losses[(size_t)b * st.losses_capacity + t] = lossf;
            if (is_best) { st.best_loss[b] = lossf; st.best_idx[b] = t; }
        }
    }
    if (i == 0 && step_out) *step_out = t + 1;

    double g_i = dth_i;
    if (rigid) {
        if (i < NT) sh_dth[i] = dth_i;
        __builtin_amdgcn_wave_barrier();
        __threadfence_block();
        double dth[NT], g[NT];
#pragma unroll
        for (int k = 0; k < NT; k++) dth[k] = sh_dth[k];
        pose_vjp<ND>(r.pose_old, dth, g);
        g_i = 0.0;
#pragma unroll
        for (int k = 0; k < NPOSE; k++) g_i = (k == i) ? g[k] : g_i;
    }
    float p_new = r.p_old;
    if (i < np) {
        const float gf = (float)g_i;
        if (user && st.grad) st.grad[(size_t)b * TRX_PSTRIDE + i] = gf;
        if (oc.kind == TRX_OPT_ADAM) {
            const float mi = r.m_old + (gf - r.m_old) * (1.0f - oc.beta1);
            const float vi = oc.beta2 * r.v_old + (1.0f - oc.beta2) * gf * gf;
            if (m_out) { m_out[i] = mi; v_out[i] = vi; }
            const float denom = (float)(sqrt((double)vi) * rsbc2) + oc.eps;
            p_new = r.p_old - (float)((double)oc.lr / bc1) * (mi / denom);
        } else {
            p_new = r.p_old - oc.lr * gf;
        }
        if (param_out) param_out[i] = p_new;
    }
    float th_new = p_new;
    if (rigid) {
        if (i < NPOSE) sh_pose[i] = p_new;
        __builtin_amdgcn_wave_barrier();
        __threadfence_block();
        float pose_new[NPOSE];
#pragma unroll
        for (int k = 0; k < NPOSE; k++) pose_new[k] = sh_pose[k];
        double thd[NT];
        theta_from_pose<ND>(pose_new, thd);
        double th_i = 0.0;
#pragma unroll
        for (int k = 0; k < NT; k++) th_i = (k == i) ? thd[k] : th_i;
        th_new = (float)th_i;
    }
    if (i < NT) {
        if (theta_out) theta_out[i] = th_new;
        if (theta_lds) theta_lds[i] = th_new;
    }
}

constexpr int kCarryStride = 64;
constexpr int kCarryTheta = 0, kCarryParam = 12, kCarryM = 24, kCarryV = 36, kCarryStep = 48;

template <int ND>
__global__ __launch_bounds__(TRX_FIN_THREADS) void affine_finalize_kernel(const float *__restrict__ partials, int nblk,
                                                                          double nvox, int D, int H, int W,
                                                                          trx_loss_cfg lc, trx_opt_cfg oc,
                                                                          trx_affine_state st, const int *__restrict__ rows_used = nullptr, int mse_rows = 0,
                                                                          const float *__restrict__ state_in = nullptr)
{
    constexpr int NP = np_full(ND);
    constexpr int NT = ND * (ND + 1);
    constexpr int NPOSE = (ND == 3) ? 6 : 3;
    __shared__ double S[64];
    const int b = blockIdx.x;
    __shared__ double sh_dth[NT];
    __shared__ float sh_pose[NPOSE];
    const int i = threadIdx.x;
    const bool rigid = st.mode == TRX_PARAM_RIGID;
    float *param = st.param + (size_t)b * TRX_PSTRIDE;
    float *theta = st.theta + (size_t)b * TRX_PSTRIDE;
    FinRegs<ND> r;
    if (i < 64) {
        if (state_in) {
            const float *sb = state_in + (size_t)b * kCarryStride;
            r = fin_load<ND>(sb + kCarryParam, sb + kCarryTheta, sb + kCarryM, sb + kCarryV, reinterpret_cast<const int *>(sb + kCarryStep), st.best_loss + b,
                             oc.kind == TRX_OPT_ADAM, rigid, i);
        } else {
            r = fin_load<ND>(param, theta, st.adam_m ? st.adam_m + (size_t)b * TRX_PSTRIDE : nullptr, st.adam_v ? st.adam_v + (size_t)b * TRX_PSTRIDE : nullptr, st.step + b,
                             st.best_loss + b, oc.kind == TRX_OPT_ADAM, rigid, i);
        }
    }
    {
        int rows = nblk;
        if (rows_used) rows = min(abs(rows_used[b]) & kRowsMask, nblk);
        if (ND == 3 && mse_rows) reduce_partials<kNpMse>(partials + (size_t)b * nblk * kNpMse, rows, S);
        else reduce_partials<NP>(partials + (size_t)b * nblk * NP, rows, S);
    }
    if (i >= 64) return;
    fin_apply<ND>(S, r, b, i, nvox, D, H, W, lc, oc, st, mse_rows, param, theta, st.adam_m ? st.adam_m + (size_t)b * TRX_PSTRIDE : nullptr,
                  st.adam_v ? st.adam_v + (size_t)b * TRX_PSTRIDE : nullptr, st.step + b, true, nullptr, sh_dth, sh_pose);
}

template <int MODE>
__device__ __forceinline__ void carry_prologue(CarryKPtr c, int b, bool designated, int D, int H, int W, float *scratch, float *s_th, int wave, int lane)
{
    constexpr int NP = (MODE == 4) ? kNpMse : np_full(3);
    constexpr int NT = 12;
    const float *prev = c->prev_partials;
    const float *sp = c->state_prev;
    float *sn = c->state_next;
    const trx_affine_state st = {c->st.mode, c->st.param, c->st.theta, c->st.adam_m, c->st.adam_v, c->st.best_theta, c->st.best_loss, c->st.best_idx, c->st.losses,
                                 c->st.losses_capacity, c->st.step, c->st.grad};
    const trx_opt_cfg oc = {c->oc.kind, c->oc.lr, c->oc.beta1, c->oc.beta2, c->oc.eps};
    const bool adam = oc.kind == TRX_OPT_ADAM, rigid = st.mode == TRX_PARAM_RIGID;
    const float *src_theta = sp ? sp + (size_t)b * kCarryStride + kCarryTheta : st.theta + (size_t)b * TRX_PSTRIDE;
    const float *src_param = sp ? sp + (size_t)b * kCarryStride + kCarryParam : st.param + (size_t)b * TRX_PSTRIDE;
    const float *src_m = sp ? sp + (size_t)b * kCarryStride + kCarryM : (st.adam_m ? st.adam_m + (size_t)b * TRX_PSTRIDE : nullptr);
    const float *src_v = sp ? sp + (size_t)b * kCarryStride + kCarryV : (st.adam_v ? st.adam_v + (size_t)b * TRX_PSTRIDE : nullptr);
    const int *src_step = sp ? reinterpret_cast<const int *>(sp + (size_t)b * kCarryStride + kCarryStep) : st.step + b;
    float *nxt = (designated && sn) ? sn + (size_t)b * kCarryStride : nullptr;
    if (prev == nullptr) {
        if (wave == 0) {
            const int ic = min(lane, NT - 1);
            const float th = src_theta[ic], pa = src_param[ic];
            const float m0 = (adam && src_m) ? src_m[ic] : 0.f, v0 = (adam && src_v) ? src_v[ic] : 0.f;
            const int t = *src_step;
            if (lane < NT) {
                s_th[lane] = th;
                if (nxt) { nxt[kCarryTheta + lane] = th; nxt[kCarryParam + lane] = pa; nxt[kCarryM + lane] = m0; nxt[kCarryV + lane] = v0; }
            }
            if (lane == 0 && nxt) *reinterpret_cast<int *>(nxt + kCarryStep) = t;
        }
        __syncthreads();
        return;
    }
    double *acc = reinterpret_cast<double *>(scratch);
    double *S = acc + 8 * 64, *sh_dth = S + 64;
    float *sh_pose = reinterpret_cast<float *>(sh_dth + NT);
    FinRegs<3> r;
    if (wave == 0) r = fin_load<3>(src_param, src_theta, src_m, src_v, src_step, designated ? st.best_loss + b : nullptr, adam, rigid, lane);
    {
        const int nblk = c->prev_nblk;
        const int rows = min(abs(c->prev_rows_used[b]) & kRowsMask, nblk);
        const float *part = prev + (size_t)b * nblk * NP;
        double s = 0.0;
        if (lane < NP) {
            constexpr int NB = TRX_CARRY_BATCH;
            for (int r0 = wave; r0 < rows; r0 += NB * 8) {
                float a[NB];
#pragma unroll
                for (int i = 0; i < NB; i++) {
                    const int row = r0 + i * 8;
                    const float v = part[(size_t)min(row, rows - 1) * NP + lane];
                    a[i] = (row < rows) ? v : 0.f;
                }
                double d[NB];
#pragma unroll
                for (int i = 0; i < NB; i++) d[i] = (double)a[i];
#pragma unroll
                for (int w = 1; w < NB; w <<= 1)
#pragma unroll
                    for (int i = 0; i + w < NB; i += 2 * w) d[i] += d[i + w];
                s += d[0];
            }
        }
        acc[wave * 64 + lane] = s;
    }
    __syncthreads();
    if (wave == 0) {
        double t = 0.0;
#pragma unroll
        for (int w = 0; w < 8; w++) t += acc[w * 64 + lane];
        S[lane] = t;
    }
    __syncthreads();
    if (wave == 0) {
        const trx_loss_cfg lc = {c->lc.w_mse, c->lc.w_ncc, c->lc.ncc_alpha, c->lc.w_ssd, c->lc.ssd_alpha};
        fin_apply<3>(S, r, b, lane, c->nvox, D, H, W, lc, oc, st, c->mse_rows, nxt ? nxt + kCarryParam : nullptr, nxt ? nxt + kCarryTheta : nullptr,
                     nxt ? nxt + kCarryM : nullptr, nxt ? nxt + kCarryV : nullptr, nxt ? reinterpret_cast<int *>(nxt + kCarryStep) : nullptr, designated, s_th, sh_dth, sh_pose);
    }
    __syncthreads();
}

__global__ __launch_bounds__(TRX_FIN_THREADS) void affine_loss_finalize_kernel(const float *__restrict__ partials, int nblk,
                                                                               double nvox, trx_loss_cfg lc,
                                                                               float *__restrict__ terms)
{
    __shared__ double S[64];
    const int b = blockIdx.x;
    reduce_partials<5>(partials + (size_t)b * nblk * 5, nblk, S);
    if (threadIdx.x != 0) return;
    const LossCoef L = loss_from_moments(S, nvox, lc);
    terms[b * 4 + 0] = (float)L.total; terms[b * 4 + 1] = (float)L.mse;
    terms[b * 4 + 2] = (float)L.ncc;   terms[b * 4 + 3] = (float)L.ssd;
}

template <int ND>
__global__ __launch_bounds__(TRX_FIN_THREADS) void affine_bwd_finalize_kernel(const float *__restrict__ partials, int nblk,
                                                                              int D, int H, int W, float *__restrict__ dtheta)
{
    constexpr int NT = ND * (ND + 1);
    __shared__ double S[64];
    const int b = blockIdx.x;
    reduce_partials<NT>(partials + (size_t)b * nblk * NT, nblk, S);
    if (threadIdx.x >= NT) return;
    const double scale[3] = {0.5 * W, 0.5 * H, 0.5 * D};
    dtheta[(size_t)b * TRX_PSTRIDE + threadIdx.x] = (float)(scale[threadIdx.x / (ND + 1)] * S[threadIdx.x]);
}

template <int ND>
__global__ __launch_bounds__(TRX_BLOCK) void affine_warp_kernel(trx_volumes vol, const float *__restrict__ theta,
                                                                int channels, size_t chan_stride,
                                                                float *__restrict__ out)
{
    const int b = blockIdx.y;
    const int D = vol.D, H = vol.H, W = vol.W;
    const size_t nvox = (size_t)D * H * W;
    const float *__restrict__ th = theta + (size_t)b * TRX_PSTRIDE;
    const float *__restrict__ mov = vol.moving + (size_t)b * vol.moving_stride;
    float *__restrict__ o = out + (size_t)b * channels * nvox;
    const float fW = (float)W, fH = (float)H, fD = (float)D;
    for (VoxelWalk vw(blockIdx.x * TRX_BLOCK + threadIdx.x, gridDim.x * TRX_BLOCK, H, W); vw.i < nvox; vw.next(H, W)) {
        const size_t i = vw.i;
        const int x = vw.x, y = vw.y, z = vw.z;
        const float xn = base_coord(vol.xn, x, W), yn = base_coord(vol.yn, y, H);
        if constexpr (ND == 3) {
            const float zn = base_coord(vol.zn, z, D);
            const float ix = unnorm<3>(fmaf(th[1], yn, fmaf(th[0], xn, fmaf(th[2], zn, th[3]))), fW);
            const float iy = unnorm<3>(fmaf(th[5], yn, fmaf(th[4], xn, fmaf(th[6], zn, th[7]))), fH);
            const float iz = unnorm<3>(fmaf(th[9], yn, fmaf(th[8], xn, fmaf(th[10], zn, th[11]))), fD);
            for (int ch = 0; ch < channels; ch++) o[ch * nvox + i] = sample3(mov + ch * chan_stride, D, H, W, ix, iy, iz).v;
        } else {
            const float ix = unnorm<2>(fmaf(th[1], yn, fmaf(th[0], xn, th[2])), fW);
            const float iy = unnorm<2>(fmaf(th[4], yn, fmaf(th[3], xn, th[5])), fH);
            for (int ch = 0; ch < channels; ch++) o[ch * nvox + i] = sample2(mov + ch * chan_stride, H, W, ix, iy).v;
        }
    }
}

struct LatticeIdx {
    const int *iz, *iy, *ix;
    int nz, ny, nx;
};

template <int ND>
__device__ __forceinline__ void lattice_coords(const trx_volumes &vol, const float *__restrict__ th, int x, int y, int z, float &xn, float &yn,
                                               float &zn, float &ix, float &iy, float &iz)
{
    xn = base_coord(vol.xn, x, vol.W); yn = base_coord(vol.yn, y, vol.H); zn = 0.f; iz = 0.f;
    if constexpr (ND == 3) {
        zn = base_coord(vol.zn, z, vol.D);
        ix = unnorm<3>(fmaf(th[1], yn, fmaf(th[0], xn, fmaf(th[2], zn, th[3]))), (float)vol.W);
        iy = unnorm<3>(fmaf(th[5], yn, fmaf(th[4], xn, fmaf(th[6], zn, th[7]))), (float)vol.H);
        iz = unnorm<3>(fmaf(th[9], yn, fmaf(th[8], xn, fmaf(th[10], zn, th[11]))), (float)vol.D);
    } else {
        ix = unnorm<2>(fmaf(th[1], yn, fmaf(th[0], xn, th[2])), (float)vol.W);
        iy = unnorm<2>(fmaf(th[4], yn, fmaf(th[3], xn, th[5])), (float)vol.H);
    }
}

template <int ND, bool BWD>
__device__ __forceinline__ void lattice_pass(const trx_volumes &vol, const float *__restrict__ th, const float *__restrict__ mov, const LatticeIdx &L,
                                             const float *__restrict__ go, float *__restrict__ out, float (&acc)[ND * (ND + 1)], float &vmin, float &vmax)
{
    constexpr int U = 4;
    const unsigned n = (unsigned)L.nz * L.ny * L.nx;
    const unsigned stride = gridDim.x * TRX_BLOCK;
    for (unsigned i0 = blockIdx.x * TRX_BLOCK + threadIdx.x; i0 < n; i0 += U * stride) {
        unsigned idx[U];
        bool ok[U];
        int x[U], y[U], z[U];
        float g[U];
#pragma unroll
        for (int u = 0; u < U; u++) {
            const unsigned i = i0 + u * stride;
            ok[u] = i < n;
            idx[u] = ok[u] ? i : i0;
            const unsigned r = idx[u] / (unsigned)L.nx, kx = idx[u] - r * L.nx, kz = r / (unsigned)L.ny, ky = r - kz * L.ny;
            x[u] = L.ix[kx]; y[u] = L.iy[ky]; z[u] = (ND == 3) ? L.iz[kz] : 0;
            g[u] = BWD ? go[idx[u]] : 0.f;
        }
        float xn[U], yn[U], zn[U], ix[U], iy[U], iz[U];
#pragma unroll
        for (int u = 0; u < U; u++) lattice_coords<ND>(vol, th, x[u], y[u], z[u], xn[u], yn[u], zn[u], ix[u], iy[u], iz[u]);
        float v[U], gq[U][ND];
#pragma unroll
        for (int u = 0; u < U; u++) {
            if constexpr (ND == 3) {
                const Samp3 sm = sample3_padded(mov, vol.D, vol.H, vol.W, ix[u], iy[u], iz[u]);
                v[u] = sm.v; gq[u][0] = sm.dx; gq[u][1] = sm.dy; gq[u][2] = sm.dz;
            } else {
                const Samp2 sm = sample2(mov, vol.H, vol.W, ix[u], iy[u]);
                v[u] = sm.v; gq[u][0] = sm.dx; gq[u][1] = sm.dy;
            }
        }
#pragma unroll
        for (int u = 0; u < U; u++) {
            if constexpr (!BWD) {
                if (ok[u]) { out[idx[u]] = v[u]; vmin = fminf(vmin, v[u]); vmax = fmaxf(vmax, v[u]); }
            } else {
                const float w = ok[u] ? g[u] : 0.f;
#pragma unroll
                for (int c = 0; c < ND; c++) {
                    const float q = w * gq[u][c];
                    acc[c * (ND + 1) + 0] = fmaf(q, xn[u], acc[c * (ND + 1) + 0]);
                    acc[c * (ND + 1) + 1] = fmaf(q, yn[u], acc[c * (ND + 1) + 1]);
                    if constexpr (ND == 3) acc[c * (ND + 1) + 2] = fmaf(q, zn[u], acc[c * (ND + 1) + 2]);
                    acc[c * (ND + 1) + ND] += q;
                }
            }
        }
    }
}

template <int ND>
__global__ __launch_bounds__(TRX_BLOCK) void affine_warp_lattice_kernel(trx_volumes vol, const float *__restrict__ theta, LatticeIdx L,
                                                                        float *__restrict__ out, float *__restrict__ block_minmax)
{
    const int b = blockIdx.y;
    const size_t n = (size_t)L.nz * L.ny * L.nx;
    float acc[ND * (ND + 1)];
    float vmin = INFINITY, vmax = -INFINITY;
    lattice_pass<ND, false>(vol, theta + (size_t)b * TRX_PSTRIDE, vol.moving + (size_t)b * vol.moving_stride, L, nullptr, out + (size_t)b * n, acc, vmin, vmax);
    if (block_minmax) {
        __shared__ float red[2][TRX_WAVES];
#pragma unroll
        for (int m = 32; m >= 1; m >>= 1) { vmin = fminf(vmin, __shfl_xor(vmin, m, 64)); vmax = fmaxf(vmax, __shfl_xor(vmax, m, 64)); }
        if ((threadIdx.x & 63) == 0) { red[0][threadIdx.x >> 6] = vmin; red[1][threadIdx.x >> 6] = vmax; }
        __syncthreads();
        if (threadIdx.x == 0) {
#pragma unroll
            for (int w = 1; w < TRX_WAVES; w++) { vmin = fminf(vmin, red[0][w]); vmax = fmaxf(vmax, red[1][w]); }
            block_minmax[((size_t)b * gridDim.x + blockIdx.x) * 2 + 0] = vmin;
            block_minmax[((size_t)b * gridDim.x + blockIdx.x) * 2 + 1] = vmax;
        }
    }
}

__global__ __launch_bounds__(1024) void nmi_lines_kernel(const float *__restrict__ block_minmax, int nblk, const float *__restrict__ mm_target, int P, int bins,
                                                         float *__restrict__ xis, float *__restrict__ mm_out)
{
    __shared__ float red[2][16];
    const int b = blockIdx.x, tid = threadIdx.x;
    float vmin = INFINITY, vmax = -INFINITY;
    for (int i = tid; i < nblk; i += 1024) {
        vmin = fminf(vmin, block_minmax[((size_t)b * nblk + i) * 2 + 0]);
        vmax = fmaxf(vmax, block_minmax[((size_t)b * nblk + i) * 2 + 1]);
    }
#pragma unroll
    for (int m = 32; m >= 1; m >>= 1) { vmin = fminf(vmin, __shfl_xor(vmin, m, 64)); vmax = fmaxf(vmax, __shfl_xor(vmax, m, 64)); }
    if ((tid & 63) == 0) { red[0][tid >> 6] = vmin; red[1][tid >> 6] = vmax; }
    __syncthreads();
    vmin = red[0][0]; vmax = red[1][0];
#pragma unroll
    for (int w = 1; w < 16; w++) { vmin = fminf(vmin, red[0][w]); vmax = fmaxf(vmax, red[1][w]); }
    const float tlo = mm_target[b * 2 + 0], thi = mm_target[b * 2 + 1];
    const float lo2 = fminf(vmin, tlo), hi2 = fmaxf(vmax, thi);
    if (tid == 0 && mm_out) { mm_out[b * 2 + 0] = vmin; mm_out[b * 2 + 1] = vmax; }
    auto lerp = [](float start, float end, float w) { const float d = end - start; return (fabsf(w) < 0.5f) ? start + w * d : end - d * (1.0f - w); };
    for (int i = tid; i < P * 2 * bins; i += 1024) {
        const int p = i / (2 * bins), k = i - p * 2 * bins;
        const bool second = k >= bins;
        const float w = (float)(second ? k - bins : k) / (float)(bins - 1);
        xis[((size_t)b * P + p) * 2 * bins + k] = second ? lerp(hi2, lo2, w) : lerp(vmax, vmin, w);
    }
}

template <int ND>
__global__ __launch_bounds__(64) void nmi_loop_update_kernel(float *__restrict__ theta, float *__restrict__ pose, const float *__restrict__ g_a,
                                                             const float *__restrict__ g_b, float lr, const float *__restrict__ loss_terms, int n_terms,
                                                             const float *__restrict__ loss_b, float *__restrict__ hist_loss_t,
                                                             float *__restrict__ hist_theta_t, float *__restrict__ param_copy)
{
    constexpr int NT = ND * (ND + 1), NPOSE = (ND == 3) ? 6 : 3;
    const int i = threadIdx.x;
    if (i == 0) {
        float tot = 0.f;
        for (int k = 0; k < n_terms; k++) tot += loss_terms[k];
        if (loss_b) tot += *loss_b;
        *hist_loss_t = tot;
    }
    const float th_i = (i < TRX_PSTRIDE) ? theta[i] : 0.f;
    if (i < TRX_PSTRIDE) hist_theta_t[i] = th_i;
    float gi = 0.f;
    if (i < TRX_PSTRIDE) gi = g_a[i] + (g_b ? g_b[i] : 0.f);
    float th_new = th_i;
    if (pose) {
        float p[NPOSE];
        double g[NT], dx[NPOSE];
#pragma unroll
        for (int k = 0; k < NPOSE; k++) p[k] = pose[k];
#pragma unroll
        for (int k = 0; k < NT; k++) g[k] = (double)(g_a[k] + (g_b ? g_b[k] : 0.f));
        pose_vjp<ND>(p, g, dx);
#pragma unroll
        for (int k = 0; k < NPOSE; k++) p[k] = p[k] - lr * (float)dx[k];
        double th[NT];
        theta_from_pose<ND>(p, th);
        double v = 0.0, pv = 0.0;
#pragma unroll
        for (int k = 0; k < NT; k++) v = (k == i) ? th[k] : v;
#pragma unroll
        for (int k = 0; k < NPOSE; k++) pv = (k == i) ? (double)p[k] : pv;
        if (i < NT) th_new = (float)v;
        __syncthreads();
        if (i < NPOSE) pose[i] = (float)pv;
    } else if (i < NT) {
        th_new = th_i - lr * gi;
    }
    if (i < TRX_PSTRIDE) { theta[i] = th_new; if (param_copy) param_copy[i] = th_new; }
}

template <int ND>
__global__ __launch_bounds__(TRX_BLOCK) void affine_lattice_bwd_kernel(trx_volumes vol, const float *__restrict__ theta, LatticeIdx L,
                                                                       const float *__restrict__ grad_out, float *__restrict__ partials)
{
    constexpr int NT = ND * (ND + 1);
    const int b = blockIdx.y;
    const size_t n = (size_t)L.nz * L.ny * L.nx;
    float acc[NT];
#pragma unroll
    for (int t = 0; t < NT; t++) acc[t] = 0.f;
    float vmin = 0.f, vmax = 0.f;
    lattice_pass<ND, true>(vol, theta + (size_t)b * TRX_PSTRIDE, vol.moving + (size_t)b * vol.moving_stride, L, grad_out + (size_t)b * n, nullptr, acc, vmin, vmax);
    block_reduce_store<NT>(acc, partials + ((size_t)b * gridDim.x + blockIdx.x) * NT);
}

template <int ND>
__global__ __launch_bounds__(64) void theta_chain_kernel(const float *__restrict__ pose, const float *__restrict__ dtheta, float *__restrict__ theta_out,
                                                         float *__restrict__ dpose_out)
{
    constexpr int NT = ND * (ND + 1), NPOSE = (ND == 3) ? 6 : 3;
    const int b = blockIdx.x, i = threadIdx.x;
    float p[NPOSE];
#pragma unroll
    for (int k = 0; k < NPOSE; k++) p[k] = pose[(size_t)b * TRX_PSTRIDE + k];
    if (theta_out) {
        double th[NT];
        theta_from_pose<ND>(p, th);
        double v = 0.0;
#pragma unroll
        for (int k = 0; k < NT; k++) v = (k == i) ? th[k] : v;
        if (i < NT) theta_out[(size_t)b * TRX_PSTRIDE + i] = (float)v;
    }
    if (dtheta && dpose_out) {
        double g[NT], dx[NPOSE];
#pragma unroll
        for (int k = 0; k < NT; k++) g[k] = (double)dtheta[(size_t)b * TRX_PSTRIDE + k];
        pose_vjp<ND>(p, g, dx);
        double v = 0.0;
#pragma unroll
        for (int k = 0; k < NPOSE; k++) v = (k == i) ? dx[k] : v;
        if (i < NPOSE) dpose_out[(size_t)b * TRX_PSTRIDE + i] = (float)v;
    }
}

static int check_vol(const trx_volumes *v, bool need_target)
{
    if (!v || !v->moving || (need_target && !v->target)) return TRX_ERR_ARG;
    if (v->ndim != 2 && v->ndim != 3) return TRX_ERR_NDIM;
    if (v->B < 1 || v->D < 1 || v->H < 1 || v->W < 1) return TRX_ERR_ARG;
    if (v->ndim == 2 && v->D != 1) return TRX_ERR_NDIM;
    if (v->B > 65535) return TRX_ERR_ARG;
    if ((size_t)v->D * v->H * v->W >= ((size_t)1 << 31)) return TRX_ERR_ARG;
    return TRX_OK;
}

constexpr int kTargetBlocks = 2048;

}

using namespace trx;

static bool use_dual(const trx_volumes *vol)
{
    return !(vol->flags & TRX_FLAG_SINGLE_GEOM);
}

static int persistent_blocks()
{
    int dev = 0, cus = 0;
    if (hipGetDevice(&dev) != hipSuccess || hipDeviceGetAttribute(&cus, hipDeviceAttributeMultiprocessorCount, dev) != hipSuccess || cus <= 0)
        return TRX_PERSISTENT_BLOCKS;
    return 2 * cus;
}

static ZGeom zs_launch_geom(const trx_volumes &v)
{
    ZGeom none = ZGeom{};
    if ((v.flags & TRX_FLAG_NO_ZSTREAM) || !zs_shape_ok<ZS64>(v)) return none;
    const ZGeom g = zs_geom<ZS64>(v);
    if (v.flags & TRX_FLAG_ZSTREAM) return g;
    const long zb = (long)g.blocks_per_pair * v.B;
    if (zb < TRX_ZS_MIN_BLOCKS || g.planes_per_seg < TRX_ZS_MIN_PLANES) return none;
    const int slots = persistent_blocks();
    if (zb > slots / 2 && zb < slots && (long)tile_geom<GeomA>(v).blocks_per_pair * v.B <= slots) return none;
    return g;
}

static size_t tile_rows_per_pair(const trx_volumes &v)
{
    size_t n = (size_t)tile_geom<GeomA>(v).blocks_per_pair;
    const size_t r = (size_t)tile_geom<GeomR>(v).blocks_per_pair;
    const size_t d = (size_t)tile_geom<GeomD>(v).blocks_per_pair, rd = (size_t)tile_geom<GeomRD>(v).blocks_per_pair;
    size_t z = zs_shape_ok<ZS64>(v) ? (size_t)zs_geom<ZS64>(v).blocks_per_pair : 0;
    if (zs_shape_ok<ZSF>(v) && (size_t)zs_geom<ZSF>(v).blocks_per_pair > z) z = (size_t)zs_geom<ZSF>(v).blocks_per_pair;
    if (r > n) n = r;
    if (d > n) n = d;
    if (rd > n) n = rd;
    if (z > n) n = z;
    return n;
}

struct AffineWs {
    size_t rows, off_tab, off_rows_used, off_part2, off_rows_used2, off_carry, bytes;
};
static AffineWs affine_ws(const trx_volumes &v)
{
    AffineWs w;
    AffineGeom g = affine_geom(v, kTargetBlocks);
    w.rows = (size_t)g.nblk;
    if (v.ndim == 3) {
        const size_t t = tile_rows_per_pair(v);
        if (t > w.rows) w.rows = t;
    }
    w.off_tab = ((size_t)v.B * w.rows * np_full(3) * sizeof(float) + 255) & ~(size_t)255;
    w.off_rows_used = w.off_tab + (((size_t)(v.W + v.H + v.D) * sizeof(float) + 255) & ~(size_t)255);
    const size_t notes = ((size_t)(v.B + 11) * sizeof(int) + 255) & ~(size_t)255;
    w.off_part2 = w.off_rows_used + notes;
    w.off_rows_used2 = w.off_part2 + (v.ndim == 3 ? w.off_tab : 0);
    w.off_carry = w.off_rows_used2 + (v.ndim == 3 ? notes : 0);
    w.bytes = w.off_carry + (v.ndim == 3 ? (((size_t)2 * v.B * kCarryStride * sizeof(float) + 255) & ~(size_t)255) : 0);
    return w;
}

extern "C" size_t trx_affine_workspace_bytes(const trx_volumes *vol)
{
    if (check_vol(vol, false) != TRX_OK) return 0;
    return affine_ws(*vol).bytes;
}

extern "C" size_t trx_affine_workspace_rows_offset(const trx_volumes *vol)
{
    if (check_vol(vol, false) != TRX_OK) return 0;
    return affine_ws(*vol).off_rows_used;
}

extern "C" int trx_affine_near_identity(const trx_volumes *vol, const float *theta_host)
{
    if (check_vol(vol, false) != TRX_OK || !theta_host || vol->ndim != 3) return 0;
    const ZGeom zg = zs_launch_geom(*vol);
    if (zg.blocks_per_pair == 0) return 0;
    const bool flat_ok = zs_shape_ok<ZSF>(*vol) && !(vol->flags & TRX_FLAG_NO_ZS_FLAT);
    const ZGeom zgf = flat_ok ? zs_geom<ZSF>(*vol) : ZGeom{};
    const float fD = (float)vol->D, fH = (float)vol->H, fW = (float)vol->W;
    for (int b = 0; b < vol->B; b++) {
        const float *th = theta_host + (size_t)b * TRX_PSTRIDE;
        if (zs_nsub<ZS64>(th, fD, fH, fW, zg.planes_per_seg) > 0) continue;
        if (flat_ok && zs_nsub<ZSF>(th, fD, fH, fW, zgf.planes_per_seg) > 0) continue;
        return 0;
    }
    return 1;
}

static bool use_tile_path(const trx_volumes *vol)
{
    if (vol->ndim != 3) return false;
    return !(vol->flags & TRX_FLAG_GATHER_PATH);
}

struct CarryLaunch {
    int parity;
    CarryKArgs args;
    bool used;
    float *partials_out;
};
template <int MODE>
static int launch_f1(const trx_volumes *vol, const float *theta, float *partials, int *nblk, hipStream_t s, bool dual, const int **rows_used = nullptr, CarryLaunch *cl = nullptr);

template <int MODE>
static int launch_accum(const trx_volumes *vol, const float *theta, const AffineGeom &g, int channels, size_t chan_stride,
                        float *partials, hipStream_t s)
{
    dim3 grid(g.nblk, vol->B), block(TRX_BLOCK);
    if (vol->ndim == 3)
        hipLaunchKernelGGL((affine_accum_kernel<3, MODE>), grid, block, 0, s, *vol, theta, g, channels, chan_stride, partials);
    else
        hipLaunchKernelGGL((affine_accum_kernel<2, MODE>), grid, block, 0, s, *vol, theta, g, channels, chan_stride, partials);
    TRX_CHECK_LAUNCH();
    return TRX_OK;
}

template <int MODE>
static int launch_f1(const trx_volumes *vol, const float *theta, float *partials, int *nblk, hipStream_t s, bool dual, const int **rows_used, CarryLaunch *cl)
{
    if (rows_used) *rows_used = nullptr;
    if (cl) cl->used = false;
    if (use_tile_path(vol)) {
        TileGeom t = tile_geom(*vol);
        trx_volumes v = *vol;
        const AffineWs ws = affine_ws(*vol);
        float *const ws_base = partials;
        const bool odd = cl != nullptr && cl->parity != 0;
        if (odd) partials = (float *)((char *)ws_base + ws.off_part2);
        if (cl) cl->partials_out = partials;
        if (!v.xn || !v.yn || !v.zn) {
            float *tab = (float *)((char *)ws_base + ws.off_tab);
            const int n = max(v.W, max(v.H, v.D));
            hipLaunchKernelGGL(fill_tables_kernel, dim3((n + 255) / 256), dim3(256), 0, s, tab, v.W, v.H, v.D);
            TRX_CHECK_LAUNCH();
            v.xn = tab; v.yn = tab + v.W; v.zn = tab + v.W + v.H;
        }
        if (dual && use_dual(vol)) {
            const TileGeom ta = tile_geom<GeomA>(*vol), tr = tile_geom<GeomR>(*vol);
            const int gx = ta.blocks_per_pair > tr.blocks_per_pair ? ta.blocks_per_pair : tr.blocks_per_pair;
            const bool aware = rows_used != nullptr;
            const bool step_kernel = aware && (MODE == 0 || MODE == 4);
            TileGeom td = TileGeom{};
            if (step_kernel) {
                const TileGeom cand = tile_geom<GeomD>(*vol);
                const long blocks_d = (long)cand.blocks_per_pair * vol->B;
                const long slots_d = persistent_blocks();
                const long rem_d = blocks_d % slots_d;
                const bool small_ok = blocks_d >= slots_d && cand.tiles_per_seg >= 4 && (rem_d == 0 || rem_d >= slots_d * 5 / 8);
                if (blocks_d >= 2 * slots_d || small_ok || (vol->flags & TRX_FLAG_DEEP_TILE)) td = cand;
            }
            TileGeom trd = TileGeom{};
            if (step_kernel && !(vol->flags & TRX_FLAG_NO_ROT_DEEP_TILE)) {
                const TileGeom cand = tile_geom<GeomRD>(*vol);
                if ((cand.ntiles >= 128 && (long)cand.ntiles * vol->B >= 2l * persistent_blocks()) || (vol->flags & TRX_FLAG_DEEP_TILE)) trd = cand;
            }
            ZGeom zg = ZGeom{};
            if (step_kernel) zg = zs_launch_geom(*vol);
            int gxx = gx;
            if (td.blocks_per_pair > gxx) gxx = td.blocks_per_pair;
            if (trd.blocks_per_pair > gxx) gxx = trd.blocks_per_pair;
            if (zg.blocks_per_pair > gxx) gxx = zg.blocks_per_pair;
            if (zg.blocks_per_pair > 0 && zs_shape_ok<ZSF>(*vol) && zs_geom<ZSF>(*vol).blocks_per_pair > gxx) gxx = zs_geom<ZSF>(*vol).blocks_per_pair;
            int *ru = aware ? (int *)((char *)ws_base + (odd ? ws.off_rows_used2 : ws.off_rows_used)) : nullptr;
            const int slots = persistent_blocks();
            const bool flat = step_kernel && vol->B <= 64 && (long)gxx * vol->B >= 2 * slots;
            const TileGeom tef = tile_geom<GeomRD>(*vol);
            const bool eft_sizes = (long)vol->H * vol->W * 4 < (1l << 24) && (size_t)vol->D * vol->H * vol->W < ((size_t)1 << 29);
            const int eft = (step_kernel && ru && tef.tiles_per_seg <= 64 && eft_sizes && !(vol->flags & TRX_FLAG_NO_EFT) &&
                             (flat || (vol->flags & TRX_FLAG_EFT))) ? tef.blocks_per_pair : 0;
            if (eft && tef.blocks_per_pair > gxx) gxx = tef.blocks_per_pair;
            const bool zs_first = flat && zg.blocks_per_pair > 0 && ru != nullptr && !(vol->flags & TRX_FLAG_ZS_FUSED);
            if constexpr (MODE == 0 || MODE == 4) {
                if (zs_first) {
                    const ZGeom zgf = (zs_shape_ok<ZSF>(*vol) && !(vol->flags & TRX_FLAG_NO_ZS_FLAT)) ? zs_geom<ZSF>(*vol) : ZGeom{};
                    if (vol->flags & TRX_FLAG_ONE_KERNEL) {
                        hipLaunchKernelGGL((affine_zs_one_kernel<MODE>), dim3(slots, 1), dim3(ZS64::Threads), 0, s, v, theta, zg, zgf, partials, ru, gxx, tr);
                        TRX_CHECK_LAUNCH();
                        *nblk = gxx;
                        *rows_used = ru;
                        return TRX_OK;
                    }
                    hipLaunchKernelGGL((affine_zs_step_kernel<MODE>), dim3(slots, 1), dim3(ZS64::Threads), 0, s, v, theta, zg, zgf, partials, ru, gxx);
                    TRX_CHECK_LAUNCH();
                }
                if (eft) {
                    const int wd = td.blocks_per_pair > 0, wrd = trd.blocks_per_pair > 0, zp = zs_first ? -1 : (zg.blocks_per_pair > 0 ? zg.planes_per_seg : 0);
                    if (flat) hipLaunchKernelGGL((affine_eft_step_kernel<MODE>), dim3(slots, 1), dim3(ECfg::Threads), 0, s, v, theta, tef, partials, ru, gxx, wd, wrd, zp);
                    else hipLaunchKernelGGL((affine_eft_step_kernel<MODE>), dim3(tef.blocks_per_pair, vol->B), dim3(ECfg::Threads), 0, s, v, theta, tef, partials, ru, -gxx, wd, wrd, zp);
                    TRX_CHECK_LAUNCH();
                }
            }
            if (zs_first) hipLaunchKernelGGL((affine_tile_dual_kernel<MODE, 4>), dim3(slots, 1), dim3(512), 0, s, v, theta, ta, tr, 1, partials, 0, td, trd, zg, ru, gxx, eft);
            else if (flat) launch_dual<MODE>(dim3(slots, 1), s, v, theta, ta, tr, 1, partials, 0, td, trd, zg, ru, gxx, eft);
            else launch_dual<MODE>(dim3(gxx, vol->B), s, v, theta, ta, tr, 1, partials, aware ? 0 : 1, td, trd, zg, ru, 0, eft, cl ? &cl->args : nullptr, cl ? &cl->used : nullptr);
            TRX_CHECK_LAUNCH();
            *nblk = gxx;
            if (aware) *rows_used = ru;
            return TRX_OK;
        }
        hipLaunchKernelGGL((affine_tile_kernel<MODE>), dim3(t.blocks_per_pair, vol->B), dim3(kTileThreads), 0, s, v, theta, t, 1, partials);
        TRX_CHECK_LAUNCH();
        *nblk = t.blocks_per_pair;
        return TRX_OK;
    }
    if constexpr (MODE == 4) {
        return TRX_ERR_ARG;
    } else {
        AffineGeom g = affine_geom(*vol, kTargetBlocks);
        *nblk = g.nblk;
        return launch_accum<MODE>(vol, theta, g, 1, 0, partials, s);
    }
}

static int launch_finalize(const trx_volumes *vol, const trx_loss_cfg *loss, const trx_opt_cfg *opt, const trx_affine_state *st, const float *partials, int nblk,
                           const int *rows_used, bool mse_only, const float *state_in, hipStream_t s);

extern "C" int trx_affine_step(const trx_volumes *vol, const trx_loss_cfg *loss, const trx_opt_cfg *opt,
                               const trx_affine_state *st, void *workspace, size_t workspace_bytes, void *stream)
{
    int rc = check_vol(vol, true);
    if (rc) return rc;
    if (!loss || !opt || !st || !workspace) return TRX_ERR_ARG;
    if (!st->param || !st->theta || !st->best_theta || !st->best_loss || !st->best_idx || !st->step) return TRX_ERR_ARG;
    if (opt->kind != TRX_OPT_SGD && opt->kind != TRX_OPT_ADAM) return TRX_ERR_ARG;
    if (opt->kind == TRX_OPT_ADAM && (!st->adam_m || !st->adam_v)) return TRX_ERR_ARG;
    if (st->mode != TRX_PARAM_AFFINE && st->mode != TRX_PARAM_RIGID) return TRX_ERR_ARG;
    if (workspace_bytes < trx_affine_workspace_bytes(vol)) return TRX_ERR_WORKSPACE;
    hipStream_t s = (hipStream_t)stream;
    float *partials = (float *)workspace;
    int nblk = 0;
    const int *rows_used = nullptr;
    const bool mse_only = (loss->w_ncc == 0.f) && use_tile_path(vol);
    rc = mse_only ? launch_f1<4>(vol, st->theta, partials, &nblk, s, true, &rows_used) : launch_f1<0>(vol, st->theta, partials, &nblk, s, true, &rows_used);
    if (rc) return rc;
    return launch_finalize(vol, loss, opt, st, partials, nblk, rows_used, mse_only, nullptr, s);
}

extern "C" int trx_affine_accumulate(const trx_volumes *vol, const float *theta, void *workspace, size_t workspace_bytes, void *stream)
{
    int rc = check_vol(vol, true);
    if (rc) return rc;
    if (!theta || !workspace) return TRX_ERR_ARG;
    if (workspace_bytes < trx_affine_workspace_bytes(vol)) return TRX_ERR_WORKSPACE;
    int nblk = 0;
    const int *rows_used = nullptr;
    return launch_f1<0>(vol, theta, (float *)workspace, &nblk, (hipStream_t)stream, true, &rows_used);
}

static int launch_finalize(const trx_volumes *vol, const trx_loss_cfg *loss, const trx_opt_cfg *opt, const trx_affine_state *st, const float *partials, int nblk,
                           const int *rows_used, bool mse_only, const float *state_in, hipStream_t s)
{
    const double nvox = (double)vol->D * vol->H * vol->W;
    if (vol->ndim == 3)
        hipLaunchKernelGGL((affine_finalize_kernel<3>), dim3(vol->B), dim3(TRX_FIN_THREADS), 0, s, partials, nblk, nvox,
                           vol->D, vol->H, vol->W, *loss, *opt, *st, rows_used, mse_only ? 1 : 0, state_in);
    else
        hipLaunchKernelGGL((affine_finalize_kernel<2>), dim3(vol->B), dim3(TRX_FIN_THREADS), 0, s, partials, nblk, nvox,
                           vol->D, vol->H, vol->W, *loss, *opt, *st);
    TRX_CHECK_LAUNCH();
    return TRX_OK;
}

extern "C" int trx_affine_run(const trx_volumes *vol, const trx_loss_cfg *loss, const trx_opt_cfg *opt,
                              const trx_affine_state *st, int iters, void *workspace, size_t workspace_bytes, void *stream)
{
    if (iters < 0 || !st) return TRX_ERR_ARG;
    if (st->losses && iters > st->losses_capacity) return TRX_ERR_CAPACITY;
    if (!vol) return TRX_ERR_ARG;
    trx_volumes v = *vol;
    int first = 0;
    if (iters >= 2 && !(vol->flags & TRX_FLAG_NO_CARRY) && check_vol(vol, true) == TRX_OK && vol->ndim == 3 && use_tile_path(vol) && loss && opt && workspace &&
        st->param && st->theta && st->best_theta && st->best_loss && st->best_idx && st->step && (opt->kind == TRX_OPT_SGD || (opt->kind == TRX_OPT_ADAM && st->adam_m && st->adam_v)) &&
        (st->mode == TRX_PARAM_AFFINE || st->mode == TRX_PARAM_RIGID) && workspace_bytes >= trx_affine_workspace_bytes(vol)) {
        hipStream_t s = (hipStream_t)stream;
        const AffineWs ws = affine_ws(*vol);
        const bool mse_only = loss->w_ncc == 0.f;
        float *const base = (float *)workspace;
        float *const carry_buf = (float *)((char *)workspace + ws.off_carry);
        const float *prev_partials = nullptr;
        const int *prev_notes = nullptr;
        int prev_nblk = 0;
        for (int k = 0; k < iters; k++) {
            CarryLaunch cl;
            cl.parity = (iters - 1 - k) & 1;
            cl.used = false;
            cl.partials_out = nullptr;
            cl.args = CarryKArgs{prev_partials, prev_notes, prev_nblk, mse_only ? 1 : 0, k > 0 ? carry_buf + (size_t)(cl.parity ^ 1) * vol->B * kCarryStride : nullptr,
                                 carry_buf + (size_t)cl.parity * vol->B * kCarryStride, (double)vol->D * vol->H * vol->W, *loss, *opt, *st};
            v.flags = vol->flags;
            if ((k & 1) && !(vol->flags & TRX_FLAG_NO_PINGPONG)) v.flags ^= TRX_FLAG_WALK_DOWN;
            int nblk = 0;
            const int *notes = nullptr;
            int rc = mse_only ? launch_f1<4>(&v, st->theta, base, &nblk, s, true, &notes, &cl) : launch_f1<0>(&v, st->theta, base, &nblk, s, true, &notes, &cl);
            if (rc) return rc;
            if (!cl.used) {
                rc = launch_finalize(vol, loss, opt, st, cl.partials_out, nblk, notes, mse_only, nullptr, s);
                if (rc) return rc;
                first = 1;
                prev_partials = nullptr;
                break;
            }
            prev_partials = cl.partials_out; prev_notes = notes; prev_nblk = nblk;
        }
        if (prev_partials != nullptr)
            return launch_finalize(vol, loss, opt, st, prev_partials, prev_nblk, prev_notes, mse_only, carry_buf, s);
    }
    for (int i = first; i < iters; i++) {
        v.flags = vol->flags;
        if ((i & 1) && !(vol->flags & TRX_FLAG_NO_PINGPONG)) v.flags ^= TRX_FLAG_WALK_DOWN;
        int rc = trx_affine_step(&v, loss, opt, st, workspace, workspace_bytes, stream);
        if (rc) return rc;
    }
    return TRX_OK;
}

extern "C" int trx_affine_loss(const trx_volumes *vol, const trx_loss_cfg *loss, const float *theta, float *terms,
                               void *workspace, size_t workspace_bytes, void *stream)
{
    int rc = check_vol(vol, true);
    if (rc) return rc;
    if (!loss || !theta || !terms || !workspace) return TRX_ERR_ARG;
    if (workspace_bytes < trx_affine_workspace_bytes(vol)) return TRX_ERR_WORKSPACE;
    hipStream_t s = (hipStream_t)stream;
    float *partials = (float *)workspace;
    int nblk = 0;
    rc = launch_f1<1>(vol, theta, partials, &nblk, s, true);
    if (rc) return rc;
    const double nvox = (double)vol->D * vol->H * vol->W;
    hipLaunchKernelGGL(affine_loss_finalize_kernel, dim3(vol->B), dim3(TRX_FIN_THREADS), 0, s, partials, nblk, nvox, *loss, terms);
    TRX_CHECK_LAUNCH();
    return TRX_OK;
}

extern "C" int trx_affine_warp(const trx_volumes *vol, const float *theta, int channels, float *out, void *stream)
{
    int rc = check_vol(vol, false);
    if (rc) return rc;
    if (!theta || !out || channels < 1) return TRX_ERR_ARG;
    if ((long)vol->B * channels > 65535) return TRX_ERR_ARG;
    hipStream_t s = (hipStream_t)stream;
    const size_t nvox = (size_t)vol->D * vol->H * vol->W;
    if (use_tile_path(vol) && vol->xn && vol->yn && vol->zn) {
        trx_volumes v = *vol;
        v.B = vol->B * channels;
        TileGeom t = tile_geom(v);
        if (use_dual(vol)) {
            const TileGeom ta = tile_geom<GeomA>(v), tr = tile_geom<GeomR>(v);
            v.B = vol->B;
            const int gx = ta.blocks_per_pair > tr.blocks_per_pair ? ta.blocks_per_pair : tr.blocks_per_pair;
            launch_dual<3>(dim3(gx, vol->B * channels), s, v, theta, ta, tr, channels, out);
            TRX_CHECK_LAUNCH();
            return TRX_OK;
        }
        v.B = vol->B;
        hipLaunchKernelGGL((affine_tile_kernel<3>), dim3(t.blocks_per_pair, vol->B * channels), dim3(kTileThreads), 0, s, v, theta, t, channels, out);
        TRX_CHECK_LAUNCH();
        return TRX_OK;
    }
    size_t nb = (nvox + TRX_BLOCK - 1) / TRX_BLOCK;
    if (nb > 8192) nb = 8192;
    dim3 grid((unsigned)nb, vol->B), block(TRX_BLOCK);
    if (vol->ndim == 3)
        hipLaunchKernelGGL((affine_warp_kernel<3>), grid, block, 0, s, *vol, theta, channels, nvox, out);
    else
        hipLaunchKernelGGL((affine_warp_kernel<2>), grid, block, 0, s, *vol, theta, channels, nvox, out);
    TRX_CHECK_LAUNCH();
    return TRX_OK;
}

extern "C" int trx_affine_warp_backward(const trx_volumes *vol, const float *theta, int channels, const float *grad_out,
                                        float *dtheta, void *workspace, size_t workspace_bytes, void *stream)
{
    int rc = check_vol(vol, false);
    if (rc) return rc;
    if (!theta || !grad_out || !dtheta || !workspace || channels < 1) return TRX_ERR_ARG;
    if (workspace_bytes < trx_affine_workspace_bytes(vol)) return TRX_ERR_WORKSPACE;
    hipStream_t s = (hipStream_t)stream;
    AffineGeom g = affine_geom(*vol, kTargetBlocks);
    float *partials = (float *)workspace;
    const size_t nvox = (size_t)vol->D * vol->H * vol->W;
    trx_volumes v = *vol;
    v.target = grad_out;
    v.target_stride = (size_t)channels * nvox;
    if (use_tile_path(vol) && vol->xn && vol->yn && vol->zn && channels == 1) {
        TileGeom t = tile_geom(*vol);
        int rows = t.blocks_per_pair;
        if (use_dual(vol)) {
            const TileGeom ta = tile_geom<GeomA>(*vol), tr = tile_geom<GeomR>(*vol);
            rows = ta.blocks_per_pair > tr.blocks_per_pair ? ta.blocks_per_pair : tr.blocks_per_pair;
            launch_dual<2>(dim3(rows, vol->B), s, v, theta, ta, tr, 1, partials);
        } else {
            hipLaunchKernelGGL((affine_tile_kernel<2>), dim3(t.blocks_per_pair, vol->B), dim3(kTileThreads), 0, s, v, theta, t, 1, partials);
        }
        TRX_CHECK_LAUNCH();
        hipLaunchKernelGGL((affine_bwd_finalize_kernel<3>), dim3(vol->B), dim3(TRX_FIN_THREADS), 0, s, partials, rows, vol->D, vol->H,
                           vol->W, dtheta);
        TRX_CHECK_LAUNCH();
        return TRX_OK;
    }
    rc = launch_accum<2>(&v, theta, g, channels, nvox, partials, s);
    if (rc) return rc;
    if (vol->ndim == 3)
        hipLaunchKernelGGL((affine_bwd_finalize_kernel<3>), dim3(vol->B), dim3(TRX_FIN_THREADS), 0, s, partials, g.nblk, vol->D, vol->H, vol->W, dtheta);
    else
        hipLaunchKernelGGL((affine_bwd_finalize_kernel<2>), dim3(vol->B), dim3(TRX_FIN_THREADS), 0, s, partials, g.nblk, vol->D, vol->H, vol->W, dtheta);
    TRX_CHECK_LAUNCH();
    return TRX_OK;
}

static int check_lattice(const trx_volumes *vol, const int *iz, int nz, const int *iy, int ny, const int *ix, int nx)
{
    if (!iy || !ix || ny < 1 || nx < 1) return TRX_ERR_ARG;
    if (vol->ndim == 3 ? (!iz || nz < 1) : (nz != 1)) return TRX_ERR_ARG;
    if ((double)nz * ny * nx >= 2147483648.0) return TRX_ERR_ARG;
    return TRX_OK;
}

static int lattice_blocks(size_t n)
{
    size_t nb = (n + (size_t)TRX_BLOCK * 4 - 1) / ((size_t)TRX_BLOCK * 4);
    return (int)(nb < 1 ? 1 : (nb > 1024 ? 1024 : nb));
}

static unsigned lattice_fwd_blocks(size_t n)
{
    size_t nb = (n + (size_t)TRX_BLOCK * 4 - 1) / ((size_t)TRX_BLOCK * 4);
    return (unsigned)(nb > 8192 ? 8192 : nb);
}

static int launch_lattice_fwd(const trx_volumes *vol, const float *theta, const LatticeIdx &L, float *out, float *block_minmax, hipStream_t s)
{
    dim3 grid(lattice_fwd_blocks((size_t)L.nz * L.ny * L.nx), vol->B), block(TRX_BLOCK);
    if (vol->ndim == 3) hipLaunchKernelGGL((affine_warp_lattice_kernel<3>), grid, block, 0, s, *vol, theta, L, out, block_minmax);
    else hipLaunchKernelGGL((affine_warp_lattice_kernel<2>), grid, block, 0, s, *vol, theta, L, out, block_minmax);
    TRX_CHECK_LAUNCH();
    return TRX_OK;
}

extern "C" int trx_affine_warp_lattice(const trx_volumes *vol, const float *theta, const int *iz, int nz, const int *iy, int ny, const int *ix,
                                       int nx, float *out, void *stream)
{
    int rc = check_vol(vol, false);
    if (rc) return rc;
    if (!theta || !out) return TRX_ERR_ARG;
    if ((rc = check_lattice(vol, iz, nz, iy, ny, ix, nx)) != TRX_OK) return rc;
    const LatticeIdx L = {iz, iy, ix, nz, ny, nx};
    return launch_lattice_fwd(vol, theta, L, out, nullptr, (hipStream_t)stream);
}

extern "C" int trx_nmi_lattice_lines(const trx_volumes *vol, const float *theta, const int *iz, int nz, const int *iy, int ny, const int *ix, int nx,
                                     float *out, const float *minmax_target, int patches, int bins, float *xis, float *minmax_warped, void *workspace,
                                     size_t workspace_bytes, void *stream)
{
    int rc = check_vol(vol, false);
    if (rc) return rc;
    if (!theta || !out || !minmax_target || !xis || !workspace || patches < 1 || bins < 2 || bins > 1024) return TRX_ERR_ARG;
    if ((rc = check_lattice(vol, iz, nz, iy, ny, ix, nx)) != TRX_OK) return rc;
    const LatticeIdx L = {iz, iy, ix, nz, ny, nx};
    const unsigned nblk = lattice_fwd_blocks((size_t)nz * ny * nx);
    if (workspace_bytes < (size_t)vol->B * nblk * 2 * sizeof(float)) return TRX_ERR_WORKSPACE;
    hipStream_t s = (hipStream_t)stream;
    if ((rc = launch_lattice_fwd(vol, theta, L, out, (float *)workspace, s)) != TRX_OK) return rc;
    hipLaunchKernelGGL(nmi_lines_kernel, dim3(vol->B), dim3(1024), 0, s, (const float *)workspace, (int)nblk, minmax_target, patches, bins, xis, minmax_warped);
    TRX_CHECK_LAUNCH();
    return TRX_OK;
}

extern "C" int trx_nmi_loop_update(int ndim, float *theta, float *pose, const float *grad_a, const float *grad_b, float lr, const float *loss_terms,
                                   int n_terms, const float *loss_b, float *hist_loss_t, float *hist_theta_t, float *param_copy, void *stream)
{
    if ((ndim != 2 && ndim != 3)) return TRX_ERR_NDIM;
    if (!theta || !grad_a || !loss_terms || n_terms < 1 || !hist_loss_t || !hist_theta_t) return TRX_ERR_ARG;
    hipStream_t s = (hipStream_t)stream;
    if (ndim == 3) hipLaunchKernelGGL((nmi_loop_update_kernel<3>), dim3(1), dim3(64), 0, s, theta, pose, grad_a, grad_b, lr, loss_terms, n_terms, loss_b,
                                      hist_loss_t, hist_theta_t, param_copy);
    else hipLaunchKernelGGL((nmi_loop_update_kernel<2>), dim3(1), dim3(64), 0, s, theta, pose, grad_a, grad_b, lr, loss_terms, n_terms, loss_b, hist_loss_t,
                            hist_theta_t, param_copy);
    TRX_CHECK_LAUNCH();
    return TRX_OK;
}

extern "C" int trx_affine_warp_lattice_backward(const trx_volumes *vol, const float *theta, const int *iz, int nz, const int *iy, int ny,
                                                const int *ix, int nx, const float *grad_out, float *dtheta, void *workspace,
                                                size_t workspace_bytes, void *stream)
{
    int rc = check_vol(vol, false);
    if (rc) return rc;
    if (!theta || !grad_out || !dtheta || !workspace) return TRX_ERR_ARG;
    if ((rc = check_lattice(vol, iz, nz, iy, ny, ix, nx)) != TRX_OK) return rc;
    const int nblk = lattice_blocks((size_t)nz * ny * nx);
    if (workspace_bytes < trx_affine_workspace_bytes(vol) || workspace_bytes < (size_t)vol->B * nblk * 12 * sizeof(float)) return TRX_ERR_WORKSPACE;
    hipStream_t s = (hipStream_t)stream;
    float *partials = (float *)workspace;
    const LatticeIdx L = {iz, iy, ix, nz, ny, nx};
    dim3 grid((unsigned)nblk, vol->B), block(TRX_BLOCK);
    if (vol->ndim == 3) {
        hipLaunchKernelGGL((affine_lattice_bwd_kernel<3>), grid, block, 0, s, *vol, theta, L, grad_out, partials);
        TRX_CHECK_LAUNCH();
        hipLaunchKernelGGL((affine_bwd_finalize_kernel<3>), dim3(vol->B), dim3(TRX_FIN_THREADS), 0, s, partials, nblk, vol->D, vol->H, vol->W, dtheta);
    } else {
        hipLaunchKernelGGL((affine_lattice_bwd_kernel<2>), grid, block, 0, s, *vol, theta, L, grad_out, partials);
        TRX_CHECK_LAUNCH();
        hipLaunchKernelGGL((affine_bwd_finalize_kernel<2>), dim3(vol->B), dim3(TRX_FIN_THREADS), 0, s, partials, nblk, vol->D, vol->H, vol->W, dtheta);
    }
    TRX_CHECK_LAUNCH();
    return TRX_OK;
}

extern "C" int trx_theta_chain(const float *pose, const float *dtheta, int ndim, int B, float *theta_out, float *dpose_out, void *stream)
{
    if (!pose || B < 1 || (!theta_out && !(dtheta && dpose_out))) return TRX_ERR_ARG;
    if (ndim != 2 && ndim != 3) return TRX_ERR_NDIM;
    hipStream_t s = (hipStream_t)stream;
    if (ndim == 3) hipLaunchKernelGGL((theta_chain_kernel<3>), dim3(B), dim3(64), 0, s, pose, dtheta, theta_out, dpose_out);
    else hipLaunchKernelGGL((theta_chain_kernel<2>), dim3(B), dim3(64), 0, s, pose, dtheta, theta_out, dpose_out);
    TRX_CHECK_LAUNCH();
    return TRX_OK;
}
```

torchregister_amd/csrc/affine_eft.h:

```cpp

#ifndef TRX_EF_DBG
#define TRX_EF_DBG 0
#endif
#ifndef TRX_EF_STAMP
#define TRX_EF_STAMP 0
#endif
#if TRX_EF_STAMP
__device__ unsigned long long trx_ef_stamps2[1024 * 8 * 8];
#define TRX_EF_ST2(k) do { if (trx_lane_id() == 0) trx_ef_stamps2[((size_t)((by * rows_stride + bx) & 1023) * 8 + wave) * 8 + (k)] = __builtin_amdgcn_s_memtime() - ef_t0; } while (0)
__device__ unsigned long long trx_ef_blocks[1024 * 8];
__device__ unsigned long long trx_ef_stamps[1024 * 8 * 8];
#endif
#if !TRX_EF_STAMP
#define TRX_EF_ST2(k) do { } while (0)
#endif
#ifndef TRX_EF_EPS
#define TRX_EF_EPS 0.05f
#endif

struct ECfg {
    static constexpr int TX = 16, TY = 16, TZ = 16, Threads = 512, Waves = 8, NH = 2, Rows = 8;
    static constexpr int K = 5;
    static constexpr int NY = 32, NZ = 32;
    static constexpr int TP = 40;
    static constexpr int GCap = 2304;
    static constexpr int BufFloats = GCap * 4, TabInts = TP * NZ;
    static constexpr int ReduceScratch = Waves * 16 * 65 + Waves * 16;
    static constexpr int OrgInts = 64 * 8;
    static constexpr int Alloc = 2 * BufFloats + TabInts + OrgInts;
    static_assert(Alloc >= ReduceScratch && K * Threads >= GCap && NY * NZ == 2 * Threads && TabInts + 2 * Waves <= BufFloats, "geometry");
};

struct EfMap {
    float A[3][3], N[3][3], ext_lo[3], ext_hi[3];
    bool ok;
};
__device__ __forceinline__ EfMap ef_map(const float *__restrict__ th, float fD, float fH, float fW)
{
    EfMap m;
    const float A[3][3] = {{th[0], th[1] * fW / fH, th[2] * fW / fD}, {th[4] * fH / fW, th[5], th[6] * fH / fD}, {th[8] * fD / fW, th[9] * fD / fH, th[10]}};
    const float c00 = A[1][1] * A[2][2] - A[1][2] * A[2][1], c01 = A[1][2] * A[2][0] - A[1][0] * A[2][2], c02 = A[1][0] * A[2][1] - A[1][1] * A[2][0];
    const float det = A[0][0] * c00 + A[0][1] * c01 + A[0][2] * c02;
    float amax = 0.f;
#pragma unroll
    for (int c = 0; c < 3; c++)
#pragma unroll
        for (int a = 0; a < 3; a++) { m.A[c][a] = A[c][a]; amax = fmaxf(amax, fabsf(A[c][a])); }
    m.ok = (fabsf(det) > 0.05f) && (amax < 4.0f);
    const float r = 1.0f / det;
    m.N[0][0] = c00 * r; m.N[0][1] = (A[0][2] * A[2][1] - A[0][1] * A[2][2]) * r; m.N[0][2] = (A[0][1] * A[1][2] - A[0][2] * A[1][1]) * r;
    m.N[1][0] = c01 * r; m.N[1][1] = (A[0][0] * A[2][2] - A[0][2] * A[2][0]) * r; m.N[1][2] = (A[0][2] * A[1][0] - A[0][0] * A[1][2]) * r;
    m.N[2][0] = c02 * r; m.N[2][1] = (A[0][1] * A[2][0] - A[0][0] * A[2][1]) * r; m.N[2][2] = (A[0][0] * A[1][1] - A[0][1] * A[1][0]) * r;
    const float ex = (float)(ECfg::TX - 1);
#pragma unroll
    for (int c = 0; c < 3; c++) {
        m.ext_lo[c] = m.ext_hi[c] = 0.f;
#pragma unroll
        for (int a = 0; a < 3; a++) { const float e = A[c][a] * ex; m.ext_lo[c] += fminf(e, 0.f); m.ext_hi[c] += fmaxf(e, 0.f); }
    }
    return m;
}
struct EfDims {
    int dy0, dz0, ny, nz, xmin, xmax;
    bool ok;
};
__device__ __forceinline__ EfDims ef_dims(const EfMap &m)
{
    EfDims d;
    const float e = TRX_EF_EPS;
    d.dy0 = (int)floorf(m.ext_lo[1] - e); d.ny = (int)floorf(m.ext_hi[1] + e) + 3 - d.dy0;
    d.dz0 = (int)floorf(m.ext_lo[2] - e); d.nz = (int)floorf(m.ext_hi[2] + e) + 3 - d.dz0;
    d.xmin = (int)floorf(m.ext_lo[0] - 2.f * e); d.xmax = (int)floorf(m.ext_hi[0] + 2.f * e) + 2;
    d.ok = m.ok && d.ny <= ECfg::NY && d.nz <= ECfg::NZ && d.ny > 0 && d.nz > 0 && (d.xmax - d.xmin) < 120;
    return d;
}
__device__ __forceinline__ int ef_row_window(const EfMap &m, int dy, int dz, int &wlo)
{
    const float e = TRX_EF_EPS, hw = 1.5f + e, yc = (float)dy - 0.5f, zc = (float)dz - 0.5f, ex = (float)(ECfg::TX - 1);
    float lo = m.ext_lo[0] - e, hi = m.ext_hi[0] + e;
    bool feasible = true;
#pragma unroll
    for (int a = 0; a < 3; a++) {
        const float gc = m.N[a][1] * yc + m.N[a][2] * zc, gh = (fabsf(m.N[a][1]) + fabsf(m.N[a][2])) * hw;
        const float l = -gc - gh, h = ex - gc + gh, n = m.N[a][0];
        if (fabsf(n) < 1.0e-6f) {
            feasible = feasible && (l <= 1.0e-3f) && (h >= -1.0e-3f);
        } else {
            const float r = 1.0f / n;
            const float a0 = l * r, a1 = h * r;
            lo = fmaxf(lo, fminf(a0, a1)); hi = fminf(hi, fmaxf(a0, a1));
        }
    }
    if (!feasible || !(lo <= hi)) { wlo = 0; return 0; }
    wlo = (int)floorf(lo - e);
    const int whi = (int)floorf(hi + e) + 2;
    return (whi - wlo + 4) >> 2;
}

__device__ __forceinline__ int ef_plan_granules_wave(const EfMap &m, const EfDims &d, int lane)
{
    int cnt = 0;
    for (int h = 0; h < (ECfg::NY * ECfg::NZ) / 64; h++) {
        const int r = lane + h * 64, iy = r & (ECfg::NY - 1), iz = r >> 5;
        int wlo;
        if (iy < d.ny && iz < d.nz) cnt += ef_row_window(m, d.dy0 + iy, d.dz0 + iz, wlo);
    }
#pragma unroll
    for (int o = 32; o > 0; o >>= 1) cnt += __shfl_xor(cnt, o, 64);
    return __builtin_amdgcn_readfirstlane(cnt);
}
__device__ __forceinline__ bool ef_candidate(const float *__restrict__ th, float fD, float fH, float fW)
{
    const EfMap m = ef_map(th, fD, fH, fW);
    return ef_dims(m).ok;
}

typedef float f4 __attribute__((ext_vector_type(4)));
typedef int i2u __attribute__((ext_vector_type(2), aligned(4)));

#pragma clang diagnostic push
#pragma clang diagnostic ignored "-Winline-asm"
#pragma clang diagnostic ignored "-Wint-to-pointer-cast"
__device__ __forceinline__ int wave_scan_incl(int v)
{
    v += __builtin_amdgcn_update_dpp(0, v, 0x111, 0xf, 0xf, false);
    v += __builtin_amdgcn_update_dpp(0, v, 0x112, 0xf, 0xf, false);
    v += __builtin_amdgcn_update_dpp(0, v, 0x114, 0xf, 0xf, false);
    v += __builtin_amdgcn_update_dpp(0, v, 0x118, 0xf, 0xf, false);
    v += __builtin_amdgcn_update_dpp(0, v, 0x142, 0xa, 0xf, false);
    v += __builtin_amdgcn_update_dpp(0, v, 0x143, 0xc, 0xf, false);
    return v;
}

struct EfPlanRegs {
    int G, ok;
    int geo[ECfg::K];
    unsigned goff[ECfg::K];
};
template <int MODE>
__device__ __forceinline__ void eft_body(const trx_volumes &vol, const float *__restrict__ theta, const TileGeom &tg, float *__restrict__ partials,
                                         float *lds, const int bx, const int by, const int rows_stride, const int wave_in, EfPlanRegs &pr, const bool replan)
{
    static_assert(MODE == 0 || MODE == 1 || MODE == 4, "step kernels and the moments pass");
    using C = ECfg;
    constexpr int NQ = (MODE == 0) ? 3 : (MODE == 4 ? 1 : 0);
    constexpr int NP = (MODE == 0) ? np_full(3) : (MODE == 4 ? kNpMse : 5);
    constexpr bool kGrad = MODE != 1;
    constexpr int kRows = C::Rows, K = C::K;
    const int b = by;
    const int D = vol.D, H = vol.H, W = vol.W;
    const float *__restrict__ th = uni_ptr(theta + (size_t)b * TRX_PSTRIDE);
    const float *__restrict__ mov = uni_ptr(vol.moving + (size_t)b * vol.moving_stride);
    const float *__restrict__ tgt = uni_ptr(vol.target + (size_t)b * vol.target_stride);
    const float *__restrict__ xtab = uni_ptr(vol.xn), *__restrict__ ytab = uni_ptr(vol.yn), *__restrict__ ztab = uni_ptr(vol.zn);
    const int lane = trx_lane_id();
    const int wave = __builtin_amdgcn_readfirstlane(wave_in);
    const int tid = wave * 64 + lane;
    const int lx = tid & (C::TX - 1), lz = (tid / C::TX) & (C::TZ - 1), lh = wave / (C::Waves / C::NH);
    const float fW = (float)W, fH = (float)H, fD = (float)D;
    const float hW = 0.5f * fW, hH = 0.5f * fH, hD = 0.5f * fD;
    const float t00 = th[0], t01 = th[1], t02 = th[2], t03 = th[3];
    const float t10 = th[4], t11 = th[5], t12 = th[6], t13 = th[7];
    const float t20 = th[8], t21 = th[9], t22 = th[10], t23 = th[11];
    const float sx = uni(hW * t01), sy = uni(hH * (t11 - 1.0f)), sz = uni(hD * t21);

    const int ncol = tg.ntx * tg.ntz;
    const int yseg = bx / ncol, cb = bx - yseg * ncol;
    int col = cb;
    if ((ncol & 7) == 0) col = (cb & 7) * (ncol >> 3) + (cb >> 3);
    const int colx = col % tg.ntx, colz = col / tg.ntx;
    const int X0 = colx * C::TX, Z0 = colz * C::TZ;
    const int nx = min(C::TX, W - X0), nz = min(C::TZ, D - Z0);
    const bool act = (lx < nx) && (lz < nz);
    const int x = X0 + (act ? lx : 0), z = Z0 + (act ? lz : 0);
    const float xn = xtab[x], zn = ztab[z];
    const float base_x = unnorm<3>(xn, fW) + hW * fmaf(t00 - 1.0f, xn, fmaf(t02, zn, t03));
    const float base_y = hH * fmaf(t10, xn, fmaf(t12, zn, t13));
    const float base_z = unnorm<3>(zn, fD) + hD * fmaf(t20, xn, fmaf(t22 - 1.0f, zn, t23));
    const float cxn = xtab[X0], czn = ztab[Z0];
    const float corner_x = uni(unnorm<3>(cxn, fW) + hW * fmaf(t00 - 1.0f, cxn, fmaf(t02, czn, t03)));
    const float corner_y = uni(hH * fmaf(t10, cxn, fmaf(t12, czn, t13)));
    const float corner_z = uni(unnorm<3>(czn, fD) + hD * fmaf(t20, cxn, fmaf(t22 - 1.0f, czn, t23)));
    const int ty_begin = yseg * tg.tiles_per_seg, ty_end = min((yseg + 1) * tg.tiles_per_seg, tg.nty);

    const EfMap mp = ef_map(th, fD, fH, fW);
    const EfDims dm = ef_dims(mp);
    int *ilds = reinterpret_cast<int *>(lds);
    int *tab = ilds + 2 * C::BufFloats;
    int *desc = ilds + C::BufFloats;
    int *wtot = ilds;
    const unsigned lds0 = (unsigned)(uintptr_t)lds;
#if TRX_EF_STAMP
    unsigned long long ef_stamp[6] = {0, 0, 0, 0, 0, 0}, ef_issue[2] = {0, 0};
    const unsigned long long ef_t0 = __builtin_amdgcn_s_memtime();
#endif
    int w4_s, hw4_s;
    asm("s_mov_b32 %0, %1" : "=s"(w4_s) : "s"(W * 4));
    asm("s_mov_b32 %0, %1" : "=s"(hw4_s) : "s"(H * W * 4));
    int *org = ilds + 2 * C::BufFloats + C::TabInts;
    auto lane_origins = [&](int ty_first) {
        if (wave != 0) return;
        const int ty = min(ty_first + lane, tg.nty - 1);
        const float yn0 = ytab[ty * C::TY], yid0 = unnorm<3>(yn0, fH);
        const float cx = fmaf(sx, yn0, corner_x), cy = yid0 + fmaf(sy, yn0, corner_y), cz = fmaf(sz, yn0, corner_z);
        const bool sane = (fabsf(cx) < 1.0e6f) && (fabsf(cy) < 1.0e6f) && (fabsf(cz) < 1.0e6f);
        const int rx = sane ? (int)floorf(cx) : -100000, ry = sane ? (int)floorf(cy) : -100000, rz = sane ? (int)floorf(cz) : -100000;
        const int x0 = rx + dm.xmin, y0 = ry + dm.dy0, z0 = rz + dm.dz0;
        const bool interior = (x0 >= 0) && (rx + dm.xmax + 3 < W) && (y0 >= 0) && (y0 + dm.ny <= H) && (z0 >= 0) && (z0 + dm.nz <= D);
        const bool outside = (rx + dm.xmax < 0) || (x0 >= W) || (y0 + dm.ny <= 0) || (y0 >= H) || (z0 + dm.nz <= 0) || (z0 >= D);
        int4 v;
        v.x = rx; v.y = ry; v.z = rz;
        v.w = outside ? 0 : (int)((((long long)z0 * H + y0) * W + x0) * 4);
        *reinterpret_cast<int4 *>(org + lane * 8) = v;
        org[lane * 8 + 4] = (interior ? 1 : 0) | (outside ? 2 : 0);
    };
    if (dm.ok) lane_origins(ty_begin);
    if (replan) {
    int cnt_r[2], wlo_r[2], pre_r[2];
#pragma unroll
    for (int h = 0; h < 2; h++) {
        const int r = tid + h * C::Threads, iy = r & (C::NY - 1), iz = r >> 5;
        cnt_r[h] = 0; wlo_r[h] = 0;
        if (dm.ok && iy < dm.ny && iz < dm.nz) cnt_r[h] = ef_row_window(mp, dm.dy0 + iy, dm.dz0 + iz, wlo_r[h]);
        const int p = wave_scan_incl(cnt_r[h]);
        pre_r[h] = p;
        if (lane == 63) wtot[h * C::Waves + wave] = p;
    }
    TRX_EF_ST2(0);
    __syncthreads();
    TRX_EF_ST2(1);
    int G = 0;
    {
        int before[2] = {0, 0};
#pragma unroll
        for (int c = 0; c < 2 * C::Waves; c++) {
            const int t = wtot[c];
            if (c < wave) before[0] += t;
            if (c < C::Waves + wave) before[1] += t;
            G += t;
        }
        pre_r[0] += before[0] - cnt_r[0];
        pre_r[1] += before[1] - cnt_r[1];
    }
    G = __builtin_amdgcn_readfirstlane(G);
    const bool plan_ok = dm.ok && G <= C::GCap && G > 0;
    __syncthreads();
    TRX_EF_ST2(2);
    if (plan_ok) {
#pragma unroll
        for (int h = 0; h < 2; h++) {
            const int r = tid + h * C::Threads, iy = r & (C::NY - 1), iz = r >> 5;
            tab[iz * C::TP + iy] = (pre_r[h] * 4 - wlo_r[h]) * 4;
            for (int k = 0; k < cnt_r[h]; k++) desc[pre_r[h] + k] = (iz << 20) | (iy << 12) | ((wlo_r[h] + 4 * k - dm.xmin) << 2);
        }
    }
    __syncthreads();
    TRX_EF_ST2(3);
#pragma unroll
    for (int k = 0; k < K; k++) {
        const int g = tid + k * C::Threads;
        pr.geo[k] = (plan_ok && g < G) ? desc[g] : 0;
    }
    auto goff_of = [&](int pk) -> unsigned {
        unsigned t0, t1, t2;
        asm("v_and_b32 %0, 0xffc, %1" : "=v"(t0) : "v"(pk));
        asm("v_bfe_u32 %0, %1, 12, 8" : "=v"(t1) : "v"(pk));
        asm("v_mad_u32_u24 %0, %1, %2, %3" : "=v"(t2) : "v"(t1), "s"(w4_s), "v"(t0));
        asm("v_lshrrev_b32 %0, 20, %1" : "=v"(t1) : "v"(pk));
        asm("v_mad_u32_u24 %0, %1, %2, %3" : "=v"(t0) : "v"(t1), "s"(hw4_s), "v"(t2));
        return t0;
    };
#pragma unroll
    for (int k = 0; k < K; k++) pr.goff[k] = goff_of(pr.geo[k]);
    pr.G = G; pr.ok = plan_ok ? 1 : 0;
    __syncthreads();
    TRX_EF_ST2(4);
    }
    const int G = __builtin_amdgcn_readfirstlane(pr.G);
    const bool plan_ok = __builtin_amdgcn_readfirstlane(pr.ok) != 0;
    const int (&geo)[K] = pr.geo;
    const unsigned (&goff)[K] = pr.goff;
#if TRX_EF_STAMP
    ef_stamp[3] = __builtin_amdgcn_s_memtime() - ef_t0;
#endif

    F1Acc acc;
#pragma unroll
    for (int q = 0; q < 3; q++)
#pragma unroll
        for (int c = 0; c < 3; c++) acc.AB[q][c] = (f2)(0.f);
    acc.M01 = acc.M23 = (f2)(0.f);
    acc.M4 = 0.f;
    const int j0 = lh * kRows;
    const unsigned toffb = (unsigned)((z * H + j0) * W + x) * 4u;
    const unsigned lane7b = (unsigned)(lane & (kRows - 1)) * 4u;

    if (plan_ok) {
        typedef const __attribute__((address_space(3))) f2u *lds_f2;
        typedef const __attribute__((address_space(3))) i2u *lds_i2;
        struct TileOrg { int rx, ry, rz; bool interior, outside; const char *base; int dP; };
        auto tile_org = [&](int ty) -> TileOrg {
            const int g = (ty - ty_begin) & 63;
            const int4 v = *reinterpret_cast<const int4 *>(org + g * 8);
            const int fl = org[g * 8 + 4];
            TileOrg o;
            o.rx = __builtin_amdgcn_readfirstlane(v.x); o.ry = __builtin_amdgcn_readfirstlane(v.y); o.rz = __builtin_amdgcn_readfirstlane(v.z);
            o.dP = __builtin_amdgcn_readfirstlane(v.w);
            const int f = __builtin_amdgcn_readfirstlane(fl);
            o.interior = f & 1; o.outside = (f >> 1) & 1;
            o.base = reinterpret_cast<const char *>(mov) + (o.interior ? (long long)o.dP : 0ll);
            return o;
        };
        auto issue_tile = [&](const TileOrg &o, int buf) {
            const char *bs = uni_ptr(o.base);
#pragma unroll
            for (int k = 0; k < K; k++) {
                int pk = geo[k], tt = tid;
                asm volatile("" : "+v"(pk), "+v"(tt));
                const int g = tt + k * C::Threads;
                unsigned off = goff[k];
                bool fetch = g < G;
                if (!o.interior) {
                    const int gz = o.rz + dm.dz0 + (pk >> 20), gy = o.ry + dm.dy0 + ((pk >> 12) & 0xff), gx = o.rx + dm.xmin + ((pk & 0xfff) >> 2);
                    const bool rowin = ((unsigned)gz < (unsigned)D) && ((unsigned)gy < (unsigned)H);
                    const bool full = rowin && (gx >= 0) && (gx + 3 < W);
                    const bool part = rowin && !full && (gx + 3 >= 0) && (gx < W);
                    off = (unsigned)((int)off + o.dP);
                    if (fetch && !full) {
                        f4 v = (f4)(0.f);
                        if (part) {
                            const float *row = mov + ((size_t)gz * H + gy) * W;
                            v.x = ((unsigned)(gx + 0) < (unsigned)W) ? row[gx + 0] : 0.f;
                            v.y = ((unsigned)(gx + 1) < (unsigned)W) ? row[gx + 1] : 0.f;
                            v.z = ((unsigned)(gx + 2) < (unsigned)W) ? row[gx + 2] : 0.f;
                            v.w = ((unsigned)(gx + 3) < (unsigned)W) ? row[gx + 3] : 0.f;
                        }
                        *reinterpret_cast<f4 *>(lds + buf * C::BufFloats + g * 4) = v;
                    }
                    fetch = fetch && full;
                }
                if (TRX_EF_DBG & 1) continue;
                const unsigned long long mk = __builtin_amdgcn_ballot_w64(fetch);
                const unsigned ldsa = lds0 + (unsigned)(buf * C::BufFloats * 4) + (unsigned)((wave * 64 + k * C::Threads) * 16);
                unsigned long long sv;
                unsigned m0s;
                asm volatile("s_mov_b64 %[sv], exec\n\t"
                             "s_mov_b32 %[m0s], m0\n\t"
                             "s_mov_b32 m0, %[l0]\n\t"
                             "s_mov_b64 exec, %[k0]\n\t"
                             "s_cbranch_execz 1f\n\t"
                             "global_load_lds_dwordx4 %[o0], %[b0]" TRX_EF_DMA_POLICY "\n\t"
                             "1:\n\t"
                             "s_mov_b64 exec, %[sv]\n\t"
                             "s_mov_b32 m0, %[m0s]"
                             : [sv] "=&s"(sv), [m0s] "=&s"(m0s)
                             : [l0] "s"(ldsa), [b0] "s"(bs), [o0] "v"(off), [k0] "s"(mk)
                             : "memory");
            }
        };
        auto issue_yn = [&](int ty, float &yn_l) {
            const unsigned yoff = (unsigned)min(ty * C::TY + j0 + (int)(lane7b >> 2), H - 1) * 4u;
            asm volatile("global_load_dword %0, %1, %2" : "=v"(yn_l) : "v"(yoff), "s"(ytab) : "memory");
        };
        auto issue_target = [&](int ty, int j, float &tvj) {
            const int Y0 = ty * C::TY;
            const float *trow = tgt + (size_t)min(Y0 + j, H - 1 - j0) * W;
            if (TRX_EF_DBG & 2) { tvj = 1.f; return; }
            asm volatile("global_load_dword %0, %1, %2" TRX_TGT_POLICY : "=v"(tvj) : "v"(toffb), "s"(trow) : "memory");
        };
        const float dyn_s = uni(H > 1 ? ytab[1] - ytab[0] : 0.f);
        const float dpx_s = uni(sx * dyn_s), dpy_s = uni((hH + sy) * dyn_s), dpz_s = uni(sz * dyn_s);
        const unsigned long long dxy2 = sgpr_pair(dpx_s, dpy_s);
        auto gather_rows = [&](int ty, const TileOrg &o, int buf, float yn_l, float (&tv)[kRows], int ja, int jb, bool more) {
            if (TRX_EF_DBG & 4) {
                if (more) for (int j = ja; j < jb; j++) issue_target(ty + 1, j, tv[j]);
                return;
            }
            const int Y0 = ty * C::TY, ny = min(C::TY, H - Y0);
            const float px_l = sx * yn_l, py_l = unnorm<3>(yn_l, fH) + sy * yn_l, pz_l = sz * yn_l;
            const float bxt = base_x - (float)o.rx, byt = base_y - (float)(o.ry + dm.dy0), bzt = base_z - (float)(o.rz + dm.dz0);
            const int tab_s = (int)lds0 + 2 * C::BufFloats * 4;
            int tp_s, bufb_s;
            asm("s_mov_b32 %0, %1" : "=s"(tp_s) : "i"(C::TP));
            asm("s_mov_b32 %0, %1" : "=s"(bufb_s) : "s"((int)lds0 + buf * C::BufFloats * 4));
            struct S1 { int e00, e01, e10, e11, xi; float fx, fy, fz; };
            struct S2 { f2 r00, r01, r10, r11; float fx, fy, fz; };
            const float ixr = bxt + lane_bcast(px_l, ja), iyr = byt + lane_bcast(py_l, ja);
            float izr = bzt + lane_bcast(pz_l, ja);
            float ynr = lane_bcast(yn_l, ja);
            f2 xyr = {ixr, iyr};
            auto stage1 = [&]() -> S1 {
                const float ix = xyr.x, iy = xyr.y, iz = izr;
                asm("v_pk_add_f32 %0, %1, %2" : "=v"(xyr) : "v"(xyr), "s"(dxy2));
                izr += dpz_s;
                int t, ta;
                asm("v_mad_u32_u24 %0, %1, %2, %3" : "=v"(t) : "v"(floor_to_int(iz)), "s"(tp_s), "v"(floor_to_int(iy)));
                asm("v_lshl_add_u32 %0, %1, 2, %2" : "=v"(ta) : "v"(t), "s"(tab_s));
                S1 s;
                const i2u ea = *(lds_i2)(unsigned)ta, eb = *(lds_i2)(unsigned)(ta + C::TP * 4);
                s.e00 = ea.x; s.e01 = ea.y; s.e10 = eb.x; s.e11 = eb.y;
                asm("v_lshl_add_u32 %0, %1, 2, %2" : "=v"(s.xi) : "v"(floor_to_int(ix)), "s"(bufb_s));
                s.fx = __builtin_amdgcn_fractf(ix); s.fy = __builtin_amdgcn_fractf(iy); s.fz = __builtin_amdgcn_fractf(iz);
                return s;
            };
            auto stage2 = [&](const S1 &s) -> S2 {
                int a00, a01, a10, a11;
                asm("v_add_u32 %0, %1, %2" : "=v"(a00) : "v"(s.xi), "v"(s.e00));
                asm("v_add_u32 %0, %1, %2" : "=v"(a01) : "v"(s.xi), "v"(s.e01));
                asm("v_add_u32 %0, %1, %2" : "=v"(a10) : "v"(s.xi), "v"(s.e10));
                asm("v_add_u32 %0, %1, %2" : "=v"(a11) : "v"(s.xi), "v"(s.e11));
                S2 f;
                f.r00 = *(lds_f2)(unsigned)a00; f.r01 = *(lds_f2)(unsigned)a01;
                f.r10 = *(lds_f2)(unsigned)a10; f.r11 = *(lds_f2)(unsigned)a11;
                f.fx = s.fx; f.fy = s.fy; f.fz = s.fz;
                return f;
            };
            const int je = min(jb, ny - j0);
            auto consume = [&](const S2 &f, int j) {
                const Samp3 sm = lerp3_pairs<kGrad>(f.r00, f.r01, f.r10, f.r11, f.fx, f.fy, f.fz);
                if (j < je) f1_accumulate_pk<MODE>(sm, tv[j], ynr, acc);
                ynr += dyn_s;
                if (more) issue_target(ty + 1, j, tv[j]);
            };
            static_assert(kRows / 2 == 4, "four rows per call");
            S2 fa = stage2(stage1());
            S2 fb = stage2(stage1());
            consume(fa, ja);
            fa = stage2(stage1());
            consume(fb, ja + 1);
            fb = stage2(stage1());
            consume(fa, ja + 2);
            consume(fb, ja + 3);
        };

        __syncthreads();
        TRX_EF_ST2(5);
        int t0 = ty_begin, t1 = ty_end;
        if (ty_end - ty_begin <= 64) {
            const int fl = org[min(lane, ty_end - ty_begin - 1) * 8 + 4];
            const unsigned long long valid = (ty_end - ty_begin) == 64 ? ~0ull : ((1ull << (ty_end - ty_begin)) - 1ull);
            const unsigned long long in = ~__builtin_amdgcn_ballot_w64((fl >> 1) & 1) & valid;
            if (in == 0) t0 = t1 = ty_end;
            else { t0 = ty_begin + __builtin_ctzll(in); t1 = ty_begin + 64 - __builtin_clzll(in); }
        } else {
            while (t0 < ty_end && tile_org(t0).outside) t0++;
            while (t1 > t0 && tile_org(t1 - 1).outside) t1--;
        }
        t0 = __builtin_amdgcn_readfirstlane(t0); t1 = __builtin_amdgcn_readfirstlane(t1);
        auto target_only = [&](int ta, int tb) {
            for (int ty = ta; ty < tb; ty++) {
                const int Y0 = ty * C::TY, nrow = min(C::TY, H - Y0) - j0;
                float yv[kRows];
#pragma unroll
                for (int j = 0; j < kRows; j++) yv[j] = tgt[(size_t)(z * H + min(Y0 + j0 + j, H - 1)) * W + x];
#pragma unroll
                for (int j = 0; j < kRows; j++) {
                    if (j < nrow) {
                        if constexpr (MODE == 4) acc.M4 = fmaf(yv[j], yv[j], acc.M4);
                        else { acc.M01.x += yv[j]; acc.M23.x = fmaf(yv[j], yv[j], acc.M23.x); }
                    }
                }
            }
        };
        float tvA[kRows], tvB[kRows], ynA = 0.f, ynB = 0.f;
#pragma unroll
        for (int j = 0; j < kRows; j++) tvA[j] = tvB[j] = 0.f;
        TileOrg cur = tile_org(min(t0, ty_end - 1));
        if (t0 < t1) {
            issue_yn(t0, ynA);
#pragma unroll
            for (int j = 0; j < kRows; j++) issue_target(t0, j, tvA[j]);
            issue_tile(cur, 0);
            TRX_EF_ST2(7);
        }
        target_only(ty_begin, t0);
        TRX_EF_ST2(6);
        if (t0 < t1) {
            asm volatile("s_waitcnt vmcnt(0)" ::: "memory");
#pragma unroll
            for (int j = 0; j < kRows; j++) asm volatile("" : "+v"(tvA[j]));
            asm volatile("" : "+v"(ynA));
        }
        __syncthreads();
#if TRX_EF_STAMP
        const unsigned long long ef_first = __builtin_amdgcn_s_memtime() - ef_t0;
#endif
        auto tile_step = [&](int ty, int par, float (&use)[kRows], float &yn_use, float (&load)[kRows], float &yn_load) {
#if TRX_EF_STAMP
            const unsigned long long es0 = __builtin_amdgcn_s_memtime();
#endif
            const bool more = ty + 1 < t1;
            TileOrg nxt = cur;
            if (more) {
                if (((ty + 1 - ty_begin) & 63) == 0) {
                    __syncthreads();
                    lane_origins(ty + 1);
                    __syncthreads();
                }
                nxt = tile_org(ty + 1);
#if TRX_EF_STAMP
                const unsigned long long ei0 = __builtin_amdgcn_s_memtime();
#endif
                issue_yn(ty + 1, yn_load);
#pragma unroll
                for (int j = 0; j < kRows; j++) issue_target(ty + 1, j, load[j]);
#if TRX_EF_STAMP
                const unsigned long long ei1 = __builtin_amdgcn_s_memtime();
                ef_issue[0] += ei0 - es0; ef_issue[1] += ei1 - ei0;
#endif
                issue_tile(nxt, par ^ 1);
            }
#if TRX_EF_STAMP
            const unsigned long long es1 = __builtin_amdgcn_s_memtime();
#endif
            gather_rows(ty, cur, par, yn_use, use, 0, kRows / 2, false);
            gather_rows(ty, cur, par, yn_use, use, kRows / 2, kRows, false);
#if TRX_EF_STAMP
            const unsigned long long es2 = __builtin_amdgcn_s_memtime();
#endif
            if (more) {
                asm volatile("s_waitcnt vmcnt(0)" ::: "memory");
#pragma unroll
                for (int j = 0; j < kRows; j++) asm volatile("" : "+v"(load[j]));
                asm volatile("" : "+v"(yn_load));
            }
            cur = nxt;
            __syncthreads();
#if TRX_EF_STAMP
            const unsigned long long es3 = __builtin_amdgcn_s_memtime();
            ef_stamp[0] += es1 - es0; ef_stamp[1] += es2 - es1; ef_stamp[2] += es3 - es2; ef_stamp[5] += 1;
#endif
        };
        {
            int ty = t0;
            while (ty < t1) {
                tile_step(ty, 0, tvA, ynA, tvB, ynB);
                ty++;
                if (ty >= t1) break;
                tile_step(ty, 1, tvB, ynB, tvA, ynA);
                ty++;
            }
        }
#if TRX_EF_STAMP
        const unsigned long long ef_walk = __builtin_amdgcn_s_memtime() - ef_t0;
#endif
        target_only(t1, ty_end);
#if TRX_EF_STAMP
        ef_stamp[4] = __builtin_amdgcn_s_memtime() - ef_t0;
        if (trx_lane_id() == 0) {
            unsigned long long *o = trx_ef_stamps + ((size_t)((by * rows_stride + bx) & 1023) * 8 + wave) * 8;
            o[6] = ef_first; o[7] = ef_walk;
        }
#endif
    } else {
        for (int ty = ty_begin; ty < ty_end; ty++) {
            const int Y0 = ty * C::TY, ny = min(C::TY, H - Y0);
            for (int j = j0; j < min(j0 + kRows, ny); j++) {
                const float yn = ytab[Y0 + j];
                const float ix = fmaf(sx, yn, base_x), iy = unnorm<3>(yn, fH) + fmaf(sy, yn, base_y), iz = fmaf(sz, yn, base_z);
                const Samp3 sm = sample3_padded(mov, D, H, W, ix, iy, iz);
                const float yv = tgt[(size_t)(z * H + Y0 + j) * W + x];
                f1_accumulate_pk<MODE>(sm, yv, yn, acc);
            }
        }
        __syncthreads();
    }
    if (!act) {
#pragma unroll
        for (int q = 0; q < 3; q++)
#pragma unroll
            for (int c = 0; c < 3; c++) acc.AB[q][c] = (f2)(0.f);
        acc.M01 = acc.M23 = (f2)(0.f);
        acc.M4 = 0.f;
    }
    float vals[NP];
    int o = 0;
    if constexpr (MODE == 4) {
        vals[0] = acc.M4;
        o = 1;
    } else {
        vals[0] = acc.M01.x; vals[1] = acc.M01.y; vals[2] = acc.M23.x; vals[3] = acc.M23.y; vals[4] = acc.M4;
        o = 5;
    }
    {
        int tt = tid;
        asm volatile("" : "+v"(tt));
        const int lx2 = tt & (C::TX - 1), lz2 = (tt / C::TX) & (C::TZ - 1);
        const int xx = X0 + ((lx2 < nx && lz2 < nz) ? lx2 : 0), zz = Z0 + ((lx2 < nx && lz2 < nz) ? lz2 : 0);
        const float xn_e = xtab[xx], zn_e = ztab[zz];
#pragma unroll
        for (int q = 0; q < NQ; q++)
#pragma unroll
            for (int c = 0; c < 3; c++) {
                const float a = acc.AB[q][c].x;
                vals[o++] = xn_e * a; vals[o++] = acc.AB[q][c].y; vals[o++] = zn_e * a; vals[o++] = a;
            }
    }
    block_reduce_store_nw<NP, C::Waves>(vals, partials + ((size_t)by * rows_stride + bx) * NP, lds, wave);
#if TRX_EF_STAMP
    if (trx_lane_id() == 0) {
        unsigned hwid, xcc;
        asm volatile("s_getreg_b32 %0, hwreg(HW_REG_HW_ID)" : "=s"(hwid));
        asm volatile("s_getreg_b32 %0, hwreg(HW_REG_XCC_ID)" : "=s"(xcc));
        unsigned long long *o = trx_ef_stamps + ((size_t)((by * rows_stride + bx) & 1023) * 8 + wave) * 8;
        for (int k = 0; k < 4; k++) o[k] = ef_stamp[k];
        o[0] |= ef_issue[0] << 32; o[1] |= ef_issue[1] << 32;
        o[4] = (ef_stamp[4] & 0xffffffffull) | ((__builtin_amdgcn_s_memtime() - ef_t0) << 32);
        o[5] = ef_stamp[5] | ((unsigned long long)(hwid & 0xffff) << 16) | ((unsigned long long)(xcc & 0xf) << 32);
    }
#endif
}

template <int MODE>
__global__ __launch_bounds__(ECfg::Threads, 4) void affine_eft_kernel(trx_volumes vol, const float *__restrict__ theta, TileGeom tg, float *__restrict__ partials)
{
    __shared__ __attribute__((aligned(16))) float lds[ECfg::Alloc];
    if ((int)blockIdx.x >= tg.blocks_per_pair) return;
    EfPlanRegs pr;
    eft_body<MODE>(vol, theta, tg, partials, lds, blockIdx.x, blockIdx.y, gridDim.x, trx_wave_index(), pr, true);
}
#pragma clang diagnostic pop
```

Measured before the change: 27090 pair-iterations/s.

## Precompute EFT row plans once per step in finalize and reuse in step kernels

```diff
diff --git a/torchregister_amd/csrc/affine.hip b/torchregister_amd/csrc/affine.hip
--- a/torchregister_amd/csrc/affine.hip
+++ b/torchregister_amd/csrc/affine.hip
@@ -1048,7 +1048,7 @@
         theta = a->theta;
         with_ef = kDeep && a->rows_used != nullptr && (a->eft != 0 || WHICH == 4);
         if constexpr (WHICH == 4) {
-            const int *plan = a->rows_used + a->vol.B;
+            const int *plan = a->rows_used + a->vol.B + (a->eft != 0 ? 11 : 0);
             if (__builtin_amdgcn_readfirstlane(*plan) == 0) return;
         }
     }
@@ -1240,43 +1240,37 @@
     zs_step_main<MODE, 1>(vol, theta, zg, zgf, partials, rows_used, stride, tgR.blocks_per_pair, ring);
 }
 
+struct EfOffer {
+    int *plans;
+    int with_d, with_rd, zs_planes;
+};
+__device__ __forceinline__ void ef_publish_pair(const float *th, int D, int H, int W, const EfOffer &eo, int b, int *s_tot, int tid)
+{
+    const float fD = (float)D, fH = (float)H, fW = (float)W;
+    const bool wanted = eft_wants(dual_choice(th, fD, fH, fW, eo.with_d != 0, eo.with_rd != 0, eo.zs_planes), th, fD, fH, fW);
+    ef_publish_plan(th, fD, fH, fW, wanted, eo.plans + (size_t)b * EfPlan::Ints, s_tot, tid);
+}
+__global__ __launch_bounds__(EfPlan::Threads) void affine_eft_plan_kernel(const float *__restrict__ theta, int D, int H, int W, EfOffer eo)
+{
+    __shared__ int s_tot[EfPlan::Threads / 64];
+    __shared__ float s_th[TRX_PSTRIDE];
+    if (threadIdx.x < TRX_PSTRIDE) s_th[threadIdx.x] = theta[(size_t)blockIdx.x * TRX_PSTRIDE + threadIdx.x];
+    __syncthreads();
+    ef_publish_pair(s_th, D, H, W, eo, blockIdx.x, s_tot, threadIdx.x);
+}
+
 template <int MODE>
 __global__ __launch_bounds__(ECfg::Threads, 4) void affine_eft_step_kernel(trx_volumes vol, const float *__restrict__ theta, TileGeom tg, float *__restrict__ partials,
-                                                                           int *__restrict__ rows_used, int stride, int with_d, int with_rd, int zs_planes_)
-{
-    const bool zs_first = zs_planes_ < 0;
-    const int zs_planes = zs_first ? 0 : zs_planes_;
+                                                                           int *__restrict__ rows_used, int stride, int zs_first_, const int *__restrict__ plans)
+{
+    const bool zs_first = zs_first_ != 0;
     __shared__ __attribute__((aligned(16))) float lds[ECfg::Alloc];
     __shared__ int s_ef[64];
     const int wave = trx_wave_index(), lane = trx_lane_id();
-    const float fD = (float)vol.D, fH = (float)vol.H, fW = (float)vol.W;
     if (stride < 0) {
         if ((int)blockIdx.x >= tg.blocks_per_pair) return;
         const int b = blockIdx.y;
-        const float *th = theta + (size_t)b * TRX_PSTRIDE;
-        bool take = __builtin_amdgcn_readfirstlane((int)eft_wants(dual_choice(th, fD, fH, fW, with_d != 0, with_rd != 0, zs_planes), th, fD, fH, fW)) &&
-                    __builtin_amdgcn_readfirstlane((int)ef_candidate(th, fD, fH, fW));
-        if (take) {
-            const EfMap m = ef_map(th, fD, fH, fW);
-            const EfDims d = ef_dims(m);
-            int cnt = 0;
-#pragma unroll
-            for (int h = 0; h < (ECfg::NY * ECfg::NZ) / ECfg::Threads; h++) {
-                const int r = wave * 64 + lane + h * ECfg::Threads, iy = r & (ECfg::NY - 1), iz = r >> 5;
-                int wlo;
-                if (iy < d.ny && iz < d.nz) cnt += ef_row_window(m, d.dy0 + iy, d.dz0 + iz, wlo);
-            }
-#pragma unroll
-            for (int o = 32; o > 0; o >>= 1) cnt += __shfl_xor(cnt, o, 64);
-            if (lane == 0) s_ef[wave] = cnt;
-            __syncthreads();
-            int g = 0;
-#pragma unroll
-            for (int w = 0; w < ECfg::Waves; w++) g += s_ef[w];
-            g = __builtin_amdgcn_readfirstlane(g);
-            take = d.ok && g > 0 && g <= ECfg::GCap;
-            __syncthreads();
-        }
+        const bool take = __builtin_amdgcn_readfirstlane(plans[(size_t)b * EfPlan::Ints + EfPlan::Ok]) != 0;
         if (blockIdx.x == 0 && wave == 0 && lane == 0) rows_used[b] = take ? -rows_note(tg.blocks_per_pair, 7) : 0;
         if (!take) return;
     }
@@ -1286,33 +1280,21 @@
 #endif
     int pre = 0, total = 1;
     if (flat) {
-    if (zs_first && __builtin_amdgcn_readfirstlane(rows_used[vol.B]) == 0) return;
+    const int left = zs_first ? __builtin_amdgcn_readfirstlane(rows_used[vol.B]) : vol.B;
+    if (left == 0) {
+        if (blockIdx.x == 0 && wave == 0 && lane == 0) rows_used[vol.B + 11] = 0;
+        return;
+    }
     unsigned long long zs_mask = 0;
     if (zs_first) zs_mask = (unsigned long long)(unsigned)__builtin_amdgcn_readfirstlane(rows_used[vol.B + 1]) | ((unsigned long long)(unsigned)__builtin_amdgcn_readfirstlane(rows_used[vol.B + 2]) << 32);
     const bool free_l = lane < vol.B && !((zs_mask >> lane) & 1ull);
-    const bool cand_l = free_l && eft_wants(dual_choice(theta + (size_t)lane * TRX_PSTRIDE, fD, fH, fW, with_d != 0, with_rd != 0, zs_planes),
-                                                  theta + (size_t)lane * TRX_PSTRIDE, fD, fH, fW) &&
-                        ef_candidate(theta + (size_t)lane * TRX_PSTRIDE, fD, fH, fW);
-    const unsigned long long cand = __builtin_amdgcn_ballot_w64(cand_l);
-    unsigned long long fit = 0;
-    if (cand) {
-        if (wave == 0) s_ef[lane] = 0;
-        __syncthreads();
-        unsigned long long rest = cand;
-        for (int k = 0; rest; k++) {
-            const int pb = __builtin_ctzll(rest);
-            rest &= rest - 1;
-            if ((k & (ECfg::Waves - 1)) != wave) continue;
-            const EfMap m = ef_map(theta + (size_t)pb * TRX_PSTRIDE, fD, fH, fW);
-            const EfDims d = ef_dims(m);
-            const int g = ef_plan_granules_wave(m, d, lane);
-            if (lane == 0) s_ef[pb] = (d.ok && g > 0 && g <= ECfg::GCap) ? 1 : 0;
-        }
-        __syncthreads();
-        fit = __builtin_amdgcn_ballot_w64(s_ef[lane] != 0) & cand;
-    }
+    const int ok_l = free_l ? plans[(size_t)lane * EfPlan::Ints + EfPlan::Ok] : 0;
+    const unsigned long long fit = __builtin_amdgcn_ballot_w64(ok_l != 0);
     const int mine = ((fit >> lane) & 1ull) ? tg.blocks_per_pair : 0;
-    if (blockIdx.x == 0 && wave == 0 && free_l) rows_used[lane] = -rows_note(mine, 7);
+    if (blockIdx.x == 0 && wave == 0) {
+        if (free_l) rows_used[lane] = -rows_note(mine, 7);
+        if (lane == 0) rows_used[vol.B + 11] = left - __builtin_popcountll(fit);
+    }
     if (fit == 0) return;
     pre = mine;
 #pragma unroll
@@ -1349,7 +1331,7 @@
         }
         v = __builtin_amdgcn_readfirstlane(v); pair = __builtin_amdgcn_readfirstlane(pair);
         if (item != it0) __syncthreads();
-        eft_body<MODE>(vol, theta, tg, partials, lds, v, pair, rows_stride, wave, pr, pair != planned);
+        eft_body<MODE>(vol, theta, tg, partials, lds, v, pair, rows_stride, wave, pr, pair != planned, plans);
         planned = pair;
 #if TRX_EF_STAMP
         if (flat && wave == 0 && lane == 0) { trx_ef_blocks[blockIdx.x * 8 + 1 + min((item - it0) / it_step, 5)] = __builtin_amdgcn_s_memrealtime(); }
@@ -1627,7 +1609,7 @@
                                                                           double nvox, int D, int H, int W,
                                                                           trx_loss_cfg lc, trx_opt_cfg oc,
                                                                           trx_affine_state st, const int *__restrict__ rows_used = nullptr, int mse_rows = 0,
-                                                                          const float *__restrict__ state_in = nullptr)
+                                                                          const float *__restrict__ state_in = nullptr, EfOffer eo = EfOffer{})
 {
     constexpr int NP = np_full(ND);
     constexpr int NT = ND * (ND + 1);
@@ -1657,9 +1639,19 @@
         if (ND == 3 && mse_rows) reduce_partials<kNpMse>(partials + (size_t)b * nblk * kNpMse, rows, S);
         else reduce_partials<NP>(partials + (size_t)b * nblk * NP, rows, S);
     }
-    if (i >= 64) return;
-    fin_apply<ND>(S, r, b, i, nvox, D, H, W, lc, oc, st, mse_rows, param, theta, st.adam_m ? st.adam_m + (size_t)b * TRX_PSTRIDE : nullptr,
-                  st.adam_v ? st.adam_v + (size_t)b * TRX_PSTRIDE : nullptr, st.step + b, true, nullptr, sh_dth, sh_pose);
+    __shared__ float sh_theta[TRX_PSTRIDE];
+    __shared__ int sh_tot[TRX_FIN_THREADS / 64];
+    const bool publish = ND == 3 && eo.plans != nullptr;
+    if (i < 64)
+        fin_apply<ND>(S, r, b, i, nvox, D, H, W, lc, oc, st, mse_rows, param, theta, st.adam_m ? st.adam_m + (size_t)b * TRX_PSTRIDE : nullptr,
+                      st.adam_v ? st.adam_v + (size_t)b * TRX_PSTRIDE : nullptr, st.step + b, true, publish ? sh_theta : nullptr, sh_dth, sh_pose);
+    if constexpr (ND == 3) {
+        static_assert(TRX_FIN_THREADS == EfPlan::Threads, "one row of the plan per thread");
+        if (publish) {
+            __syncthreads();
+            ef_publish_pair(sh_theta, D, H, W, eo, b, sh_tot, i);
+        }
+    }
 }
 
 template <int MODE>
@@ -2074,7 +2066,7 @@
 }
 
 struct AffineWs {
-    size_t rows, off_tab, off_rows_used, off_part2, off_rows_used2, off_carry, bytes;
+    size_t rows, off_tab, off_rows_used, off_part2, off_rows_used2, off_carry, off_plans, bytes;
 };
 static AffineWs affine_ws(const trx_volumes &v)
 {
@@ -2087,11 +2079,13 @@
     }
     w.off_tab = ((size_t)v.B * w.rows * np_full(3) * sizeof(float) + 255) & ~(size_t)255;
     w.off_rows_used = w.off_tab + (((size_t)(v.W + v.H + v.D) * sizeof(float) + 255) & ~(size_t)255);
-    const size_t notes = ((size_t)(v.B + 11) * sizeof(int) + 255) & ~(size_t)255;
+    const size_t notes = ((size_t)(v.B + 12) * sizeof(int) + 255) & ~(size_t)255;
     w.off_part2 = w.off_rows_used + notes;
     w.off_rows_used2 = w.off_part2 + (v.ndim == 3 ? w.off_tab : 0);
     w.off_carry = w.off_rows_used2 + (v.ndim == 3 ? notes : 0);
-    w.bytes = w.off_carry + (v.ndim == 3 ? (((size_t)2 * v.B * kCarryStride * sizeof(float) + 255) & ~(size_t)255) : 0);
+    w.off_plans = w.off_carry + (v.ndim == 3 ? (((size_t)2 * v.B * kCarryStride * sizeof(float) + 255) & ~(size_t)255) : 0);
+    const bool plans = v.ndim == 3 && (v.B <= 64 || (v.flags & TRX_FLAG_EFT));
+    w.bytes = w.off_plans + (plans ? (size_t)v.B * EfPlan::Ints * sizeof(int) : 0);
     return w;
 }
 
@@ -2137,7 +2131,8 @@
     float *partials_out;
 };
 template <int MODE>
-static int launch_f1(const trx_volumes *vol, const float *theta, float *partials, int *nblk, hipStream_t s, bool dual, const int **rows_used = nullptr, CarryLaunch *cl = nullptr);
+static int launch_f1(const trx_volumes *vol, const float *theta, float *partials, int *nblk, hipStream_t s, bool dual, const int **rows_used = nullptr, CarryLaunch *cl = nullptr,
+                     EfOffer *offer = nullptr, bool plans_ready = false);
 
 template <int MODE>
 static int launch_accum(const trx_volumes *vol, const float *theta, const AffineGeom &g, int channels, size_t chan_stride,
@@ -2153,8 +2148,10 @@
 }
 
 template <int MODE>
-static int launch_f1(const trx_volumes *vol, const float *theta, float *partials, int *nblk, hipStream_t s, bool dual, const int **rows_used, CarryLaunch *cl)
-{
+static int launch_f1(const trx_volumes *vol, const float *theta, float *partials, int *nblk, hipStream_t s, bool dual, const int **rows_used, CarryLaunch *cl,
+                     EfOffer *offer, bool plans_ready)
+{
+    if (offer) *offer = EfOffer{};
     if (rows_used) *rows_used = nullptr;
     if (cl) cl->used = false;
     if (use_tile_path(vol)) {
@@ -2203,7 +2200,7 @@
             const bool flat = step_kernel && vol->B <= 64 && (long)gxx * vol->B >= 2 * slots;
             const TileGeom tef = tile_geom<GeomRD>(*vol);
             const bool eft_sizes = (long)vol->H * vol->W * 4 < (1l << 24) && (size_t)vol->D * vol->H * vol->W < ((size_t)1 << 29);
-            const int eft = (step_kernel && ru && tef.tiles_per_seg <= 64 && eft_sizes && !(vol->flags & TRX_FLAG_NO_EFT) &&
+            const int eft = (step_kernel && ru && tef.tiles_per_seg <= 64 && eft_sizes && !(vol->flags & TRX_FLAG_NO_EFT) && ws.bytes > ws.off_plans &&
                              (flat || (vol->flags & TRX_FLAG_EFT))) ? tef.blocks_per_pair : 0;
             if (eft && tef.blocks_per_pair > gxx) gxx = tef.blocks_per_pair;
             const bool zs_first = flat && zg.blocks_per_pair > 0 && ru != nullptr && !(vol->flags & TRX_FLAG_ZS_FUSED);
@@ -2221,9 +2218,14 @@
                     TRX_CHECK_LAUNCH();
                 }
                 if (eft) {
-                    const int wd = td.blocks_per_pair > 0, wrd = trd.blocks_per_pair > 0, zp = zs_first ? -1 : (zg.blocks_per_pair > 0 ? zg.planes_per_seg : 0);
-                    if (flat) hipLaunchKernelGGL((affine_eft_step_kernel<MODE>), dim3(slots, 1), dim3(ECfg::Threads), 0, s, v, theta, tef, partials, ru, gxx, wd, wrd, zp);
-                    else hipLaunchKernelGGL((affine_eft_step_kernel<MODE>), dim3(tef.blocks_per_pair, vol->B), dim3(ECfg::Threads), 0, s, v, theta, tef, partials, ru, -gxx, wd, wrd, zp);
+                    const EfOffer eo = {(int *)((char *)ws_base + ws.off_plans), td.blocks_per_pair > 0, trd.blocks_per_pair > 0, (!zs_first && zg.blocks_per_pair > 0) ? zg.planes_per_seg : 0};
+                    if (offer) *offer = eo;
+                    if (!plans_ready) {
+                        hipLaunchKernelGGL(affine_eft_plan_kernel, dim3(vol->B), dim3(EfPlan::Threads), 0, s, theta, vol->D, vol->H, vol->W, eo);
+                        TRX_CHECK_LAUNCH();
+                    }
+                    if (flat) hipLaunchKernelGGL((affine_eft_step_kernel<MODE>), dim3(slots, 1), dim3(ECfg::Threads), 0, s, v, theta, tef, partials, ru, gxx, zs_first ? 1 : 0, eo.plans);
+                    else hipLaunchKernelGGL((affine_eft_step_kernel<MODE>), dim3(tef.blocks_per_pair, vol->B), dim3(ECfg::Threads), 0, s, v, theta, tef, partials, ru, -gxx, 0, eo.plans);
                     TRX_CHECK_LAUNCH();
                 }
             }
@@ -2250,10 +2252,17 @@
 }
 
 static int launch_finalize(const trx_volumes *vol, const trx_loss_cfg *loss, const trx_opt_cfg *opt, const trx_affine_state *st, const float *partials, int nblk,
-                           const int *rows_used, bool mse_only, const float *state_in, hipStream_t s);
-
+                           const int *rows_used, bool mse_only, const float *state_in, hipStream_t s, const EfOffer &eo = EfOffer{});
+
+static int affine_step(const trx_volumes *vol, const trx_loss_cfg *loss, const trx_opt_cfg *opt,
+                       const trx_affine_state *st, void *workspace, size_t workspace_bytes, void *stream, bool plans_ready);
 extern "C" int trx_affine_step(const trx_volumes *vol, const trx_loss_cfg *loss, const trx_opt_cfg *opt,
                                const trx_affine_state *st, void *workspace, size_t workspace_bytes, void *stream)
+{
+    return affine_step(vol, loss, opt, st, workspace, workspace_bytes, stream, false);
+}
+static int affine_step(const trx_volumes *vol, const trx_loss_cfg *loss, const trx_opt_cfg *opt,
+                       const trx_affine_state *st, void *workspace, size_t workspace_bytes, void *stream, bool plans_ready)
 {
     int rc = check_vol(vol, true);
     if (rc) return rc;
@@ -2268,9 +2277,11 @@
     int nblk = 0;
     const int *rows_used = nullptr;
     const bool mse_only = (loss->w_ncc == 0.f) && use_tile_path(vol);
-    rc = mse_only ? launch_f1<4>(vol, st->theta, partials, &nblk, s, true, &rows_used) : launch_f1<0>(vol, st->theta, partials, &nblk, s, true, &rows_used);
+    EfOffer eo;
+    rc = mse_only ? launch_f1<4>(vol, st->theta, partials, &nblk, s, true, &rows_used, nullptr, &eo, plans_ready)
+                  : launch_f1<0>(vol, st->theta, partials, &nblk, s, true, &rows_used, nullptr, &eo, plans_ready);
     if (rc) return rc;
-    return launch_finalize(vol, loss, opt, st, partials, nblk, rows_used, mse_only, nullptr, s);
+    return launch_finalize(vol, loss, opt, st, partials, nblk, rows_used, mse_only, nullptr, s, eo);
 }
 
 extern "C" int trx_affine_accumulate(const trx_volumes *vol, const float *theta, void *workspace, size_t workspace_bytes, void *stream)
@@ -2285,12 +2296,12 @@
 }
 
 static int launch_finalize(const trx_volumes *vol, const trx_loss_cfg *loss, const trx_opt_cfg *opt, const trx_affine_state *st, const float *partials, int nblk,
-                           const int *rows_used, bool mse_only, const float *state_in, hipStream_t s)
+                           const int *rows_used, bool mse_only, const float *state_in, hipStream_t s, const EfOffer &eo)
 {
     const double nvox = (double)vol->D * vol->H * vol->W;
     if (vol->ndim == 3)
         hipLaunchKernelGGL((affine_finalize_kernel<3>), dim3(vol->B), dim3(TRX_FIN_THREADS), 0, s, partials, nblk, nvox,
-                           vol->D, vol->H, vol->W, *loss, *opt, *st, rows_used, mse_only ? 1 : 0, state_in);
+                           vol->D, vol->H, vol->W, *loss, *opt, *st, rows_used, mse_only ? 1 : 0, state_in, eo);
     else
         hipLaunchKernelGGL((affine_finalize_kernel<2>), dim3(vol->B), dim3(TRX_FIN_THREADS), 0, s, partials, nblk, nvox,
                            vol->D, vol->H, vol->W, *loss, *opt, *st);
@@ -2328,10 +2339,11 @@
             if ((k & 1) && !(vol->flags & TRX_FLAG_NO_PINGPONG)) v.flags ^= TRX_FLAG_WALK_DOWN;
             int nblk = 0;
             const int *notes = nullptr;
-            int rc = mse_only ? launch_f1<4>(&v, st->theta, base, &nblk, s, true, &notes, &cl) : launch_f1<0>(&v, st->theta, base, &nblk, s, true, &notes, &cl);
+            EfOffer eo;
+            int rc = mse_only ? launch_f1<4>(&v, st->theta, base, &nblk, s, true, &notes, &cl, &eo) : launch_f1<0>(&v, st->theta, base, &nblk, s, true, &notes, &cl, &eo);
             if (rc) return rc;
             if (!cl.used) {
-                rc = launch_finalize(vol, loss, opt, st, cl.partials_out, nblk, notes, mse_only, nullptr, s);
+                rc = launch_finalize(vol, loss, opt, st, cl.partials_out, nblk, notes, mse_only, nullptr, s, eo);
                 if (rc) return rc;
                 first = 1;
                 prev_partials = nullptr;
@@ -2345,7 +2357,7 @@
     for (int i = first; i < iters; i++) {
         v.flags = vol->flags;
         if ((i & 1) && !(vol->flags & TRX_FLAG_NO_PINGPONG)) v.flags ^= TRX_FLAG_WALK_DOWN;
-        int rc = trx_affine_step(&v, loss, opt, st, workspace, workspace_bytes, stream);
+        int rc = affine_step(&v, loss, opt, st, workspace, workspace_bytes, stream, i > 0);
         if (rc) return rc;
     }
     return TRX_OK;
diff --git a/torchregister_amd/csrc/affine_eft.h b/torchregister_amd/csrc/affine_eft.h
--- a/torchregister_amd/csrc/affine_eft.h
+++ b/torchregister_amd/csrc/affine_eft.h
@@ -97,24 +97,6 @@
     return (whi - wlo + 4) >> 2;
 }
 
-__device__ __forceinline__ int ef_plan_granules_wave(const EfMap &m, const EfDims &d, int lane)
-{
-    int cnt = 0;
-    for (int h = 0; h < (ECfg::NY * ECfg::NZ) / 64; h++) {
-        const int r = lane + h * 64, iy = r & (ECfg::NY - 1), iz = r >> 5;
-        int wlo;
-        if (iy < d.ny && iz < d.nz) cnt += ef_row_window(m, d.dy0 + iy, d.dz0 + iz, wlo);
-    }
-#pragma unroll
-    for (int o = 32; o > 0; o >>= 1) cnt += __shfl_xor(cnt, o, 64);
-    return __builtin_amdgcn_readfirstlane(cnt);
-}
-__device__ __forceinline__ bool ef_candidate(const float *__restrict__ th, float fD, float fH, float fW)
-{
-    const EfMap m = ef_map(th, fD, fH, fW);
-    return ef_dims(m).ok;
-}
-
 typedef float f4 __attribute__((ext_vector_type(4)));
 typedef int i2u __attribute__((ext_vector_type(2), aligned(4)));
 
@@ -132,6 +114,42 @@
     return v;
 }
 
+struct EfPlan {
+    static constexpr int Ok = 0, G = 1, Theta = 4, Tab = 16, Desc = Tab + ECfg::TabInts;
+    static constexpr int Ints = ((Desc + ECfg::GCap + 63) / 64) * 64;
+    static constexpr int Threads = ECfg::NY * ECfg::NZ;
+    static_assert((Tab * 4) % 16 == 0 && (Desc * 4) % 16 == 0 && ECfg::TabInts % 4 == 0, "the table is copied in 16-byte pieces");
+};
+__device__ __forceinline__ void ef_publish_plan(const float *th, float fD, float fH, float fW, bool wanted, int *__restrict__ slot, int *s_tot, int tid)
+{
+    using C = ECfg;
+    static_assert(EfPlan::Threads == 1024, "16 waves");
+    const int lane = tid & 63, wave = tid >> 6;
+    const EfMap mp = ef_map(th, fD, fH, fW);
+    const EfDims dm = ef_dims(mp);
+    const int iy = tid & (C::NY - 1), iz = tid >> 5;
+    int cnt = 0, wlo = 0;
+    if (wanted && dm.ok && iy < dm.ny && iz < dm.nz) cnt = ef_row_window(mp, dm.dy0 + iy, dm.dz0 + iz, wlo);
+    const int p = wave_scan_incl(cnt);
+    if (lane == 63) s_tot[wave] = p;
+    __syncthreads();
+    int before = 0, G = 0;
+#pragma unroll
+    for (int c = 0; c < EfPlan::Threads / 64; c++) {
+        const int t = s_tot[c];
+        if (c < wave) before += t;
+        G += t;
+    }
+    const int pre = p - cnt + before;
+    const bool ok = wanted && dm.ok && G > 0 && G <= C::GCap;
+    if (tid == 0) { slot[EfPlan::Ok] = ok ? 1 : 0; slot[EfPlan::G] = G; }
+    if (tid < 12) slot[EfPlan::Theta + tid] = __float_as_int(th[tid]);
+    if (ok) {
+        slot[EfPlan::Tab + iz * C::TP + iy] = (pre * 4 - wlo) * 4;
+        for (int k = 0; k < cnt; k++) slot[EfPlan::Desc + pre + k] = (iz << 20) | (iy << 12) | ((wlo + 4 * k - dm.xmin) << 2);
+    }
+}
+
 struct EfPlanRegs {
     int G, ok;
     int geo[ECfg::K];
@@ -139,7 +157,8 @@
 };
 template <int MODE>
 __device__ __forceinline__ void eft_body(const trx_volumes &vol, const float *__restrict__ theta, const TileGeom &tg, float *__restrict__ partials,
-                                         float *lds, const int bx, const int by, const int rows_stride, const int wave_in, EfPlanRegs &pr, const bool replan)
+                                         float *lds, const int bx, const int by, const int rows_stride, const int wave_in, EfPlanRegs &pr, const bool replan,
+                                         const int *__restrict__ plans)
 {
     static_assert(MODE == 0 || MODE == 1 || MODE == 4, "step kernels and the moments pass");
     using C = ECfg;
@@ -187,8 +206,6 @@
     const EfDims dm = ef_dims(mp);
     int *ilds = reinterpret_cast<int *>(lds);
     int *tab = ilds + 2 * C::BufFloats;
-    int *desc = ilds + C::BufFloats;
-    int *wtot = ilds;
     const unsigned lds0 = (unsigned)(uintptr_t)lds;
 #if TRX_EF_STAMP
     unsigned long long ef_stamp[6] = {0, 0, 0, 0, 0, 0}, ef_issue[2] = {0, 0};
@@ -216,50 +233,14 @@
     };
     if (dm.ok) lane_origins(ty_begin);
     if (replan) {
-    int cnt_r[2], wlo_r[2], pre_r[2];
-#pragma unroll
-    for (int h = 0; h < 2; h++) {
-        const int r = tid + h * C::Threads, iy = r & (C::NY - 1), iz = r >> 5;
-        cnt_r[h] = 0; wlo_r[h] = 0;
-        if (dm.ok && iy < dm.ny && iz < dm.nz) cnt_r[h] = ef_row_window(mp, dm.dy0 + iy, dm.dz0 + iz, wlo_r[h]);
-        const int p = wave_scan_incl(cnt_r[h]);
-        pre_r[h] = p;
-        if (lane == 63) wtot[h * C::Waves + wave] = p;
-    }
-    TRX_EF_ST2(0);
-    __syncthreads();
-    TRX_EF_ST2(1);
-    int G = 0;
-    {
-        int before[2] = {0, 0};
-#pragma unroll
-        for (int c = 0; c < 2 * C::Waves; c++) {
-            const int t = wtot[c];
-            if (c < wave) before[0] += t;
-            if (c < C::Waves + wave) before[1] += t;
-            G += t;
-        }
-        pre_r[0] += before[0] - cnt_r[0];
-        pre_r[1] += before[1] - cnt_r[1];
-    }
-    G = __builtin_amdgcn_readfirstlane(G);
-    const bool plan_ok = dm.ok && G <= C::GCap && G > 0;
-    __syncthreads();
-    TRX_EF_ST2(2);
-    if (plan_ok) {
-#pragma unroll
-        for (int h = 0; h < 2; h++) {
-            const int r = tid + h * C::Threads, iy = r & (C::NY - 1), iz = r >> 5;
-            tab[iz * C::TP + iy] = (pre_r[h] * 4 - wlo_r[h]) * 4;
-            for (int k = 0; k < cnt_r[h]; k++) desc[pre_r[h] + k] = (iz << 20) | (iy << 12) | ((wlo_r[h] + 4 * k - dm.xmin) << 2);
-        }
-    }
-    __syncthreads();
-    TRX_EF_ST2(3);
+    const int *__restrict__ slot = uni_ptr(plans + (size_t)b * EfPlan::Ints);
+    const int G = slot[EfPlan::G];
+    const bool plan_ok = slot[EfPlan::Ok] != 0;
+    if (plan_ok && tid < C::TabInts / 4) reinterpret_cast<int4 *>(tab)[tid] = reinterpret_cast<const int4 *>(slot + EfPlan::Tab)[tid];
 #pragma unroll
     for (int k = 0; k < K; k++) {
         const int g = tid + k * C::Threads;
-        pr.geo[k] = (plan_ok && g < G) ? desc[g] : 0;
+        pr.geo[k] = (plan_ok && g < G) ? slot[EfPlan::Desc + g] : 0;
     }
     auto goff_of = [&](int pk) -> unsigned {
         unsigned t0, t1, t2;
@@ -273,7 +254,6 @@
 #pragma unroll
     for (int k = 0; k < K; k++) pr.goff[k] = goff_of(pr.geo[k]);
     pr.G = G; pr.ok = plan_ok ? 1 : 0;
-    __syncthreads();
     TRX_EF_ST2(4);
     }
     const int G = __builtin_amdgcn_readfirstlane(pr.G);
@@ -612,11 +592,12 @@
 }
 
 template <int MODE>
-__global__ __launch_bounds__(ECfg::Threads, 4) void affine_eft_kernel(trx_volumes vol, const float *__restrict__ theta, TileGeom tg, float *__restrict__ partials)
+__global__ __launch_bounds__(ECfg::Threads, 4) void affine_eft_kernel(trx_volumes vol, const float *__restrict__ theta, TileGeom tg, float *__restrict__ partials,
+                                                                      const int *__restrict__ plans)
 {
     __shared__ __attribute__((aligned(16))) float lds[ECfg::Alloc];
     if ((int)blockIdx.x >= tg.blocks_per_pair) return;
     EfPlanRegs pr;
-    eft_body<MODE>(vol, theta, tg, partials, lds, blockIdx.x, blockIdx.y, gridDim.x, trx_wave_index(), pr, true);
+    eft_body<MODE>(vol, theta, tg, partials, lds, blockIdx.x, blockIdx.y, gridDim.x, trx_wave_index(), pr, true, plans);
 }
 #pragma clang diagnostic pop
```

Result: no change. 26940 pair-iterations/s (-0.6%).
